# LLNL/Juqbox.jl

Hardware: AMD Instinct MI355X
Metric: traceobjgrad evals/sec (fwd+adjoint), cnot3 Hilbert dim (higher is better)
Workload: dtype f64

## Files before the change

### include/juqbox_hip.h

```cpp
#ifndef JUQBOX_HIP_H
#define JUQBOX_HIP_H

#include <stdint.h>

#ifdef __cplusplus
extern "C" {
#endif

#define JQ_ABI_VERSION 6

#define JQ_MAX_CONTROLS 16
#define JQ_MAX_WRANK 16

#define JQ_OK 0
#define JQ_EINVAL -1
#define JQ_EDIM -2
#define JQ_EUNSUPPORTED -3
#define JQ_EHIP -4
#define JQ_ENOMEM -5

typedef struct jq_handle jq_handle;

typedef struct jq_csc {
    int64_t m, n;
    const int64_t *colptr;
    const int64_t *rowval;
    const double *nzval;
} jq_csc;

typedef struct jq_problem {
    int32_t Ntot;
    int32_t N;
    int32_t Ncoupled;
    int32_t Nfreq;
    int32_t nsteps;
    int32_t neumann_terms;
    int32_t objFuncType;
    int32_t Nunc;
    double T;
    const double *Hconst;
    const double *Hsym_ops;
    const double *Hanti_ops;
    const double *Uinit;
    const double *Utarget_r;
    const double *Utarget_i;
    const double *wmat_real_diag;
    const double *Cfreq;
    const double *Hunc_ops;
    const double *Rfreq;
    const jq_csc *Hconst_csc;
    const jq_csc *Hsym_csc;
    const jq_csc *Hanti_csc;
} jq_problem;

typedef struct jq_timing {
    double ms_total;
    double ms_propagate;
    double ms_generate;
    double ms_forward;
    double ms_backward;
    int64_t n_forward_launches;
    int64_t n_backward_launches;
    int64_t mfma_executed;
    int64_t svts;
    int32_t kernel_family;
    int32_t kernel_size;
    int32_t kernel_band;
    int32_t kernel_variant;
    int64_t mfma_backward;
    double ms_allreduce;
    double ms_shard_min;
    double ms_shard_max;
} jq_timing;

int jq_device_count(void);
int jq_set_device(int device);
int jq_create(const jq_problem *problem, jq_handle **out);
int jq_create_opts(const jq_problem *problem, const char *options, jq_handle **out);
#define JQ_OPTION_DEFAULT INT64_MIN
int jq_set_option(jq_handle *h, const char *name, int64_t value);
int jq_get_option(const jq_handle *h, const char *name, int64_t *value);
void jq_destroy(jq_handle *h);
const char *jq_last_error(const jq_handle *h);

int jq_create_multi(const jq_problem *problem, const int32_t *devices, int32_t ndev, jq_handle **out);
int jq_create_multi_opts(const jq_problem *problem, const int32_t *devices, int32_t ndev, const char *options, jq_handle **out);
int jq_rccl_world_size(const jq_handle *h);
int jq_num_devices(const jq_handle *h);
int jq_num_compute_units(const jq_handle *h);
int jq_handle_device(const jq_handle *h);
int jq_shard_bounds(int32_t nquad, int32_t rank, int32_t world, int32_t *lo, int32_t *hi);

int jq_set_neumann_terms(jq_handle *h, int32_t m);
int jq_set_linear_solver(jq_handle *h, int32_t solver_id, int32_t max_iter, double tol);
int jq_set_integrator(jq_handle *h, int32_t integrator_id, int32_t max_iter, double tol);
int jq_update_target(jq_handle *h, const double *Utarget_r, const double *Utarget_i);
#define JQ_SV_TARGET 1
#define JQ_SV_TERM1 2
#define JQ_SV_TERM2 3
#define JQ_SV_BOTH 4
int jq_update_dvds(jq_handle *h, const double *dVds_r, const double *dVds_i);
int jq_set_sv_type(jq_handle *h, int32_t sv_type);
int jq_get_sv_type(const jq_handle *h);
int jq_update_hconst(jq_handle *h, const double *Hconst);
int jq_update_hconst_csc(jq_handle *h, const jq_csc *Hconst);
int jq_update_wmat_diag(jq_handle *h, const double *wmat_real_diag);
int jq_update_wmat(jq_handle *h, const double *wmat_real, const double *wmat_imag);

int jq_traceobjgrad(jq_handle *h, const double *pcof, int32_t ncoeff, int32_t evaladjoint, double *out4,
                    double *totalgrad, double *infidelgrad, double *leakgrad);

int jq_state_history(jq_handle *h, const double *pcof, int32_t ncoeff, double *ur, double *ui);
int jq_traceobj_verbose(jq_handle *h, const double *pcof, int32_t ncoeff, double *out4, double *ur, double *ui);

int jq_state_populations(jq_handle *h, const double *pcof, int32_t ncoeff, const int32_t *group_of_row, int32_t ngroups,
                         int32_t every, int32_t nout, double *pop, double *maxpop);

int jq_eval_f_g_grad(jq_handle *h, const double *pcof, int32_t ncoeff, const double *nodes, const double *weights,
                     int32_t nquad, const double *shift, int32_t compute_adjoint, double *out2, double *infid_grad,
                     double *leak_grad);

int jq_eval_f_g_grad_dev(jq_handle *h, const double *pcof, int32_t ncoeff, const double *nodes, const double *weights,
                         int32_t nquad, const double *shift, int32_t compute_adjoint, void *d_packed);

int jq_traceobj_sweep(jq_handle *h, const double *pcof, int32_t ncoeff, const double *nodes, int32_t nquad,
                      const double *shift, double *out);

int jq_plan_info(const jq_handle *h, char *buf, int32_t buflen);

int jq_last_timing(const jq_handle *h, jq_timing *t);
const char *jq_version(void);
int jq_abi_version(void);

#ifdef __cplusplus
}
#endif
#endif
```

### juqbox.jl_amd/_lib.py

```python
import ctypes
import os

_HERE = os.path.dirname(os.path.abspath(__file__))
LIB_PATH = os.environ.get("JQ_LIB") or os.path.join(_HERE, "libjuqbox_hip.so")

c_dp = ctypes.POINTER(ctypes.c_double)
c_i32 = ctypes.c_int32

JQ_OK, JQ_EINVAL, JQ_EDIM, JQ_EUNSUPPORTED, JQ_EHIP, JQ_ENOMEM = 0, -1, -2, -3, -4, -5
JQ_SV_TARGET, JQ_SV_TERM1, JQ_SV_TERM2, JQ_SV_BOTH = 1, 2, 3, 4
JQ_OPTION_DEFAULT = -2 ** 63


class jq_csc(ctypes.Structure):
    _fields_ = [("m", ctypes.c_int64), ("n", ctypes.c_int64), ("colptr", ctypes.POINTER(ctypes.c_int64)),
                ("rowval", ctypes.POINTER(ctypes.c_int64)), ("nzval", c_dp)]


class jq_problem(ctypes.Structure):
    _fields_ = [("Ntot", c_i32), ("N", c_i32), ("Ncoupled", c_i32), ("Nfreq", c_i32), ("nsteps", c_i32),
                ("neumann_terms", c_i32), ("objFuncType", c_i32), ("Nunc", c_i32), ("T", ctypes.c_double),
                ("Hconst", c_dp), ("Hsym_ops", c_dp), ("Hanti_ops", c_dp), ("Uinit", c_dp), ("Utarget_r", c_dp),
                ("Utarget_i", c_dp), ("wmat_real_diag", c_dp), ("Cfreq", c_dp), ("Hunc_ops", c_dp), ("Rfreq", c_dp),
                ("Hconst_csc", ctypes.POINTER(jq_csc)), ("Hsym_csc", ctypes.POINTER(jq_csc)), ("Hanti_csc", ctypes.POINTER(jq_csc))]


class jq_timing(ctypes.Structure):
    _fields_ = [("ms_total", ctypes.c_double), ("ms_propagate", ctypes.c_double), ("ms_generate", ctypes.c_double),
                ("ms_forward", ctypes.c_double), ("ms_backward", ctypes.c_double),
                ("n_forward_launches", ctypes.c_int64), ("n_backward_launches", ctypes.c_int64), ("mfma_executed", ctypes.c_int64), ("svts", ctypes.c_int64),
                ("kernel_family", ctypes.c_int32), ("kernel_size", ctypes.c_int32), ("kernel_band", ctypes.c_int32),
                ("kernel_variant", ctypes.c_int32), ("mfma_backward", ctypes.c_int64),
                ("ms_allreduce", ctypes.c_double), ("ms_shard_min", ctypes.c_double), ("ms_shard_max", ctypes.c_double)]


JQ_ABI_VERSION = 6


SYMBOLS = {
    "jq_device_count": (ctypes.c_int, []),
    "jq_set_device": (ctypes.c_int, [ctypes.c_int]),
    "jq_create": (ctypes.c_int, [ctypes.POINTER(jq_problem), ctypes.POINTER(ctypes.c_void_p)]),
    "jq_create_opts": (ctypes.c_int, [ctypes.POINTER(jq_problem), ctypes.c_char_p, ctypes.POINTER(ctypes.c_void_p)]),
    "jq_set_option": (ctypes.c_int, [ctypes.c_void_p, ctypes.c_char_p, ctypes.c_int64]),
    "jq_get_option": (ctypes.c_int, [ctypes.c_void_p, ctypes.c_char_p, ctypes.POINTER(ctypes.c_int64)]),
    "jq_destroy": (None, [ctypes.c_void_p]),
    "jq_last_error": (ctypes.c_char_p, [ctypes.c_void_p]),
    "jq_set_neumann_terms": (ctypes.c_int, [ctypes.c_void_p, c_i32]),
    "jq_set_linear_solver": (ctypes.c_int, [ctypes.c_void_p, c_i32, c_i32, ctypes.c_double]),
    "jq_set_integrator": (ctypes.c_int, [ctypes.c_void_p, c_i32, c_i32, ctypes.c_double]),
    "jq_update_target": (ctypes.c_int, [ctypes.c_void_p, c_dp, c_dp]),
    "jq_update_dvds": (ctypes.c_int, [ctypes.c_void_p, c_dp, c_dp]),
    "jq_set_sv_type": (ctypes.c_int, [ctypes.c_void_p, c_i32]),
    "jq_get_sv_type": (ctypes.c_int, [ctypes.c_void_p]),
    "jq_update_hconst": (ctypes.c_int, [ctypes.c_void_p, c_dp]),
    "jq_update_hconst_csc": (ctypes.c_int, [ctypes.c_void_p, ctypes.POINTER(jq_csc)]),
    "jq_update_wmat_diag": (ctypes.c_int, [ctypes.c_void_p, c_dp]),
    "jq_update_wmat": (ctypes.c_int, [ctypes.c_void_p, c_dp, c_dp]),
    "jq_traceobjgrad": (ctypes.c_int, [ctypes.c_void_p, c_dp, c_i32, c_i32, c_dp, c_dp, c_dp, c_dp]),
    "jq_state_history": (ctypes.c_int, [ctypes.c_void_p, c_dp, c_i32, c_dp, c_dp]),
    "jq_traceobj_verbose": (ctypes.c_int, [ctypes.c_void_p, c_dp, c_i32, c_dp, c_dp, c_dp]),
    "jq_state_populations": (ctypes.c_int, [ctypes.c_void_p, c_dp, c_i32, ctypes.POINTER(ctypes.c_int32), c_i32, c_i32, c_i32,
                                            c_dp, c_dp]),
    "jq_eval_f_g_grad": (ctypes.c_int, [ctypes.c_void_p, c_dp, c_i32, c_dp, c_dp, c_i32, c_dp, c_i32, c_dp, c_dp, c_dp]),
    "jq_eval_f_g_grad_dev": (ctypes.c_int, [ctypes.c_void_p, c_dp, c_i32, c_dp, c_dp, c_i32, c_dp, c_i32, ctypes.c_void_p]),
    "jq_create_multi": (ctypes.c_int, [ctypes.POINTER(jq_problem), ctypes.POINTER(ctypes.c_int32), c_i32,
                                       ctypes.POINTER(ctypes.c_void_p)]),
    "jq_create_multi_opts": (ctypes.c_int, [ctypes.POINTER(jq_problem), ctypes.POINTER(ctypes.c_int32), c_i32, ctypes.c_char_p,
                                            ctypes.POINTER(ctypes.c_void_p)]),
    "jq_rccl_world_size": (ctypes.c_int, [ctypes.c_void_p]),
    "jq_num_devices": (ctypes.c_int, [ctypes.c_void_p]),
    "jq_handle_device": (ctypes.c_int, [ctypes.c_void_p]),
    "jq_num_compute_units": (ctypes.c_int, [ctypes.c_void_p]),
    "jq_shard_bounds": (ctypes.c_int, [c_i32, c_i32, c_i32, ctypes.POINTER(ctypes.c_int32), ctypes.POINTER(ctypes.c_int32)]),
    "jq_traceobj_sweep": (ctypes.c_int, [ctypes.c_void_p, c_dp, c_i32, c_dp, c_i32, c_dp, c_dp]),
    "jq_plan_info": (ctypes.c_int, [ctypes.c_void_p, ctypes.c_char_p, c_i32]),
    "jq_last_timing": (ctypes.c_int, [ctypes.c_void_p, ctypes.POINTER(jq_timing)]),
    "jq_version": (ctypes.c_char_p, []),
    "jq_abi_version": (ctypes.c_int, []),
}

_lib = None


class JuqboxHipError(RuntimeError):
    def __init__(self, code, msg):
        super().__init__("libjuqbox_hip error %d: %s" % (code, msg))
        self.code = code


def load():
    global _lib
    if _lib is None:
        if not os.path.exists(LIB_PATH):
            raise ImportError("libjuqbox_hip.so not built: %s is missing (run `make -C juqbox.jl_amd/csrc`); "
                              "there is no CPU fallback for the hot path" % LIB_PATH)
        L = ctypes.CDLL(LIB_PATH)
        for name, (res, args) in SYMBOLS.items():
            fn = getattr(L, name)
            fn.restype = res
            fn.argtypes = args
        if L.jq_abi_version() != JQ_ABI_VERSION:
            raise ImportError("libjuqbox_hip.so has ABI version %d, this binding is written for %d (rebuild: make -C "
                              "juqbox.jl_amd/csrc)" % (L.jq_abi_version(), JQ_ABI_VERSION))
        _lib = L
    return _lib


def check(rc, handle=None):
    if rc != JQ_OK:
        msg = load().jq_last_error(handle)
        raise JuqboxHipError(rc, msg.decode() if msg else "?")
```

### juqbox.jl_amd/csrc/jq_host_create.h

```cpp
template <typename T>
static int dev_alloc(jq_handle* h, T** p, size_t count)
{
    if (*p) {
        (void)hipFree(*p);
        *p = nullptr;
    }
    if (hipMalloc((void**)p, std::max<size_t>(count, 1) * sizeof(T)) != hipSuccess) {
        *p = nullptr;
        (void)hipGetLastError();
        char buf[160];
        snprintf(buf, sizeof buf, "out of device memory (%zu bytes requested)", std::max<size_t>(count, 1) * sizeof(T));
        return fail(h, JQ_ENOMEM, buf);
    }
    return JQ_OK;
}
template <typename T>
static int dev_grow(jq_handle* h, T** p, size_t* cap, size_t need)
{
    if (need <= *cap && *p) return JQ_OK;
    *cap = 0;
    const int rc = dev_alloc(h, p, need);
    if (rc == JQ_OK) *cap = need;
    return rc;
}

static int upload_operators(jq_handle* h)
{
    const size_t nn = (size_t)h->Ntot * h->Ntot;
    std::vector<double> img((size_t)(1 + 2 * h->Nc) * h->mat_elems, 0.0);
    if (!h->big) {
        tile_image(h->Hconst.data(), h->Ntot, h->NT, h->BW, img.data());
        for (int q = 0; q < h->Nc; ++q) {
            tile_image(h->Hsym.data() + q * nn, h->Ntot, h->NT, h->BW, img.data() + (size_t)(1 + q) * h->mat_elems);
            tile_image(h->Hanti.data() + q * nn, h->Ntot, h->NT, h->BW, img.data() + (size_t)(1 + h->Nc + q) * h->mat_elems);
        }
    }
    HIPCHK(h, hipMemcpy(h->d_himg, img.data(), img.size() * sizeof(double), hipMemcpyHostToDevice));
    auto cslot = [&](int q, bool anti) {
        int g = 0;
        while (ctrl_gstart(h->Nc, g + 1) <= q) ++g;
        const int gs = ctrl_gstart(h->Nc, g), ng = ctrl_gstart(h->Nc, g + 1) - gs;
        return (size_t)(2 * gs + (anti ? ng : 0) + (q - gs));
    };
    std::vector<double> cimg((size_t)(2 * h->Nc) * h->mat_elems, 0.0);
    for (int q = 0; q < h->Nc && !h->big; ++q) {
        const int bwq = (h->BW == JQ_BW_T4) ? JQ_BW_T4 : (h->bw_trace[q] == 0) ? 0 : h->BW;
        const bool sd = (h->BW == JQ_BW_T4) ? false : (h->bw_trace[q] == 2);
        tile_image(h->Hsym.data() + q * nn, h->Ntot, h->NT, bwq, cimg.data() + cslot(q, false) * h->mat_elems, sd);
        tile_image(h->Hanti.data() + q * nn, h->Ntot, h->NT, bwq, cimg.data() + cslot(q, true) * h->mat_elems, sd);
    }
    HIPCHK(h, hipMemcpy(h->d_cimg, cimg.data(), cimg.size() * sizeof(double), hipMemcpyHostToDevice));
    if (h->mat_elems_c > 0) {
        std::vector<double> ic((size_t)(1 + 2 * h->Nc) * h->mat_elems_c, 0.0);
        tile_image_coop(h->Hconst.data(), h->Ntot, h->NT, h->BWc, ic.data());
        for (int q = 0; q < h->Nc; ++q) {
            tile_image_coop(h->Hsym.data() + q * nn, h->Ntot, h->NT, h->BWc, ic.data() + (size_t)(1 + q) * h->mat_elems_c);
            tile_image_coop(h->Hanti.data() + q * nn, h->Ntot, h->NT, h->BWc, ic.data() + (size_t)(1 + h->Nc + q) * h->mat_elems_c);
        }
        HIPCHK(h, hipMemcpy(h->d_himg_c, ic.data(), ic.size() * sizeof(double), hipMemcpyHostToDevice));
        std::vector<double> cc((size_t)2 * h->Nc * h->mat_elems_c);
        for (int q = 0; q < h->Nc; ++q) {
            std::copy_n(ic.data() + (size_t)(1 + q) * h->mat_elems_c, h->mat_elems_c, cc.data() + cslot(q, false) * h->mat_elems_c);
            std::copy_n(ic.data() + (size_t)(1 + h->Nc + q) * h->mat_elems_c, h->mat_elems_c, cc.data() + cslot(q, true) * h->mat_elems_c);
        }
        HIPCHK(h, hipMemcpy(h->d_cimg_c, cc.data(), cc.size() * sizeof(double), hipMemcpyHostToDevice));
    }
    if (h->lane_np > 0) {
        std::vector<double> il((size_t)(1 + 2 * h->Nc) * h->lane_stride, 0.0);
        plain_image(h->Hconst.data(), h->Ntot, h->lane_np, il.data());
        for (int q = 0; q < h->Nc; ++q) {
            plain_image(h->Hsym.data() + q * nn, h->Ntot, h->lane_np, il.data() + (size_t)(1 + q) * h->lane_stride);
            plain_image(h->Hanti.data() + q * nn, h->Ntot, h->lane_np, il.data() + (size_t)(1 + h->Nc + q) * h->lane_stride);
        }
        HIPCHK(h, hipMemcpy(h->d_himg_l, il.data(), il.size() * sizeof(double), hipMemcpyHostToDevice));
        std::vector<double> cl((size_t)2 * h->Nc * h->lane_stride);
        for (int q = 0; q < h->Nc; ++q) {
            std::copy_n(il.data() + (size_t)(1 + q) * h->lane_stride, h->lane_stride, cl.data() + cslot(q, false) * h->lane_stride);
            std::copy_n(il.data() + (size_t)(1 + h->Nc + q) * h->lane_stride, h->lane_stride, cl.data() + cslot(q, true) * h->lane_stride);
        }
        HIPCHK(h, hipMemcpy(h->d_cimg_l, cl.data(), cl.size() * sizeof(double), hipMemcpyHostToDevice));
    }
    if (h->dq_max_quads > 0) {
        std::vector<double> id((size_t)(1 + 2 * h->Nc) * JQ_DQ_ELEMS, 0.0);
        dq_image(h->Hconst.data(), h->Ntot, id.data());
        for (int q = 0; q < h->Nc; ++q) {
            dq_image(h->Hsym.data() + q * nn, h->Ntot, id.data() + (size_t)(1 + q) * JQ_DQ_ELEMS);
            dq_image(h->Hanti.data() + q * nn, h->Ntot, id.data() + (size_t)(1 + h->Nc + q) * JQ_DQ_ELEMS);
        }
        HIPCHK(h, hipMemcpy(h->d_himg_dq, id.data(), id.size() * sizeof(double), hipMemcpyHostToDevice));
        std::vector<double> cd((size_t)2 * h->Nc * JQ_DQ_ELEMS);
        for (int q = 0; q < h->Nc; ++q) {
            std::copy_n(id.data() + (size_t)(1 + q) * JQ_DQ_ELEMS, JQ_DQ_ELEMS, cd.data() + cslot(q, false) * JQ_DQ_ELEMS);
            std::copy_n(id.data() + (size_t)(1 + h->Nc + q) * JQ_DQ_ELEMS, JQ_DQ_ELEMS, cd.data() + cslot(q, true) * JQ_DQ_ELEMS);
        }
        HIPCHK(h, hipMemcpy(h->d_cimg_dq, cd.data(), cd.size() * sizeof(double), hipMemcpyHostToDevice));
    }
    if (h->rl_npj > 0) {
        std::vector<double> ir((size_t)(1 + 2 * h->Nc) * h->rl_stride, 0.0);
        rowlane_image(h->Hconst.data(), h->Ntot, h->rl_npj, ir.data());
        for (int q = 0; q < h->Nc; ++q) {
            rowlane_image(h->Hsym.data() + q * nn, h->Ntot, h->rl_npj, ir.data() + (size_t)(1 + q) * h->rl_stride);
            rowlane_image(h->Hanti.data() + q * nn, h->Ntot, h->rl_npj, ir.data() + (size_t)(1 + h->Nc + q) * h->rl_stride);
        }
        HIPCHK(h, hipMemcpy(h->d_himg_r, ir.data(), ir.size() * sizeof(double), hipMemcpyHostToDevice));
        std::vector<double> cr((size_t)2 * h->Nc * h->rl_stride);
        for (int q = 0; q < h->Nc; ++q) {
            std::copy_n(ir.data() + (size_t)(1 + q) * h->rl_stride, h->rl_stride, cr.data() + cslot(q, false) * h->rl_stride);
            std::copy_n(ir.data() + (size_t)(1 + h->Nc + q) * h->rl_stride, h->rl_stride, cr.data() + cslot(q, true) * h->rl_stride);
        }
        HIPCHK(h, hipMemcpy(h->d_cimg_r, cr.data(), cr.size() * sizeof(double), hipMemcpyHostToDevice));
    }
    return JQ_OK;
}

static int upload_terminal_images(jq_handle* h, const double* re, const double* im, double* d_r, double* d_i, double* d_r_l, double* d_i_l,
                                  double* d_r_r, double* d_i_r)
{
    std::vector<double> img((size_t)h->parts * h->KT * 64);
    slab_image(re, h->Ntot, h->N, h->sps, h->KT, img.data(), h->parts);
    HIPCHK(h, hipMemcpy(d_r, img.data(), img.size() * sizeof(double), hipMemcpyHostToDevice));
    slab_image(im, h->Ntot, h->N, h->sps, h->KT, img.data(), h->parts);
    HIPCHK(h, hipMemcpy(d_i, img.data(), img.size() * sizeof(double), hipMemcpyHostToDevice));
    if (h->lane_np > 0) {
        std::vector<double> cl((size_t)h->N * h->lane_np, 0.0);
        column_image(re, h->Ntot, h->N, h->lane_np, cl.data());
        HIPCHK(h, hipMemcpy(d_r_l, cl.data(), cl.size() * sizeof(double), hipMemcpyHostToDevice));
        std::fill(cl.begin(), cl.end(), 0.0);
        column_image(im, h->Ntot, h->N, h->lane_np, cl.data());
        HIPCHK(h, hipMemcpy(d_i_l, cl.data(), cl.size() * sizeof(double), hipMemcpyHostToDevice));
    }
    if (h->rl_npj > 0) {
        std::vector<double> cl((size_t)h->N * 16, 0.0);
        column_image(re, h->Ntot, h->N, 16, cl.data());
        HIPCHK(h, hipMemcpy(d_r_r, cl.data(), cl.size() * sizeof(double), hipMemcpyHostToDevice));
        std::fill(cl.begin(), cl.end(), 0.0);
        column_image(im, h->Ntot, h->N, 16, cl.data());
        HIPCHK(h, hipMemcpy(d_i_r, cl.data(), cl.size() * sizeof(double), hipMemcpyHostToDevice));
    }
    return JQ_OK;
}

static int upload_targets(jq_handle* h)
{
    return upload_terminal_images(h, h->Utr.data(), h->Uti.data(), h->d_vtr, h->d_vti, h->d_vtr_l, h->d_vti_l, h->d_vtr_r, h->d_vti_r);
}

static int upload_dvds(jq_handle* h)
{
    if (!h->dv_stale) return JQ_OK;
    HIPCHK(h, hipSetDevice(h->device));
    int rc;
    if (!h->dv_alloc) {
        if ((rc = dev_alloc(h, &h->d_dvr, (size_t)h->parts * h->KT * 64))) return rc;
        if ((rc = dev_alloc(h, &h->d_dvi, (size_t)h->parts * h->KT * 64))) return rc;
        if (h->lane_np > 0) {
            if ((rc = dev_alloc(h, &h->d_dvr_l, (size_t)h->N * h->lane_np))) return rc;
            if ((rc = dev_alloc(h, &h->d_dvi_l, (size_t)h->N * h->lane_np))) return rc;
        }
        if (h->rl_npj > 0) {
            if ((rc = dev_alloc(h, &h->d_dvr_r, (size_t)h->N * 16))) return rc;
            if ((rc = dev_alloc(h, &h->d_dvi_r, (size_t)h->N * 16))) return rc;
        }
        h->dv_alloc = true;
    }
    if ((rc = upload_terminal_images(h, h->dVr.data(), h->dVi.data(), h->d_dvr, h->d_dvi, h->d_dvr_l, h->d_dvi_l, h->d_dvr_r, h->d_dvi_r)))
        return rc;
    h->dv_stale = false;
    return JQ_OK;
}

extern "C" int jq_device_count(void)
{
    int n = 0;
    if (hipGetDeviceCount(&n) != hipSuccess) return 0;
    return n;
}

extern "C" int jq_set_device(int device) { return hipSetDevice(device) == hipSuccess ? JQ_OK : JQ_EHIP; }
// ... 70 lines not shown
        const int64_t b = A->colptr[j], e = A->colptr[j + 1];
        for (int64_t k = b - 1; k < e - 1; ++k) {
            const int64_t r = A->rowval[k];
            if (r < 1 || r > Ntot) {
                snprintf(buf, sizeof buf, "%s: rowval out of range (1 .. Ntot)", what);
                return fail(h, JQ_EINVAL, buf);
            }
            out[(r - 1) + (size_t)Ntot * j] += A->nzval[k];
        }
    }
    return JQ_OK;
}

static int create_dense(const jq_problem* p, jq_handle* h);

static int create_impl(const jq_problem* p, jq_handle* h)
{
    if (!p) return fail(h, JQ_EINVAL, "jq_create: problem is NULL");
    const bool sparse = (!p->Hconst && p->Hconst_csc) || (!p->Hsym_ops && p->Hsym_csc) || (!p->Hanti_ops && p->Hanti_csc);
    if (!sparse) return create_dense(p, h);
    if (p->Ntot < 1 || p->Ntot > 16384 || p->Ncoupled < 0 || p->Ncoupled > 4096) return create_dense(p, h);
    const size_t nn = (size_t)p->Ntot * p->Ntot;
    std::vector<double> H0, Hs, Ha;
    jq_problem q = *p;
    q.Hconst_csc = q.Hsym_csc = q.Hanti_csc = nullptr;
    int rc;
    if (!p->Hconst && p->Hconst_csc) {
        H0.resize(nn);
        if ((rc = csc_to_dense(h, p->Hconst_csc, p->Ntot, H0.data(), "jq_create: Hconst_csc"))) return rc;
        q.Hconst = H0.data();
    }
    if (!p->Hsym_ops && p->Hsym_csc) {
        Hs.resize(nn * std::max(p->Ncoupled, 1));
        for (int k = 0; k < p->Ncoupled; ++k)
            if ((rc = csc_to_dense(h, p->Hsym_csc + k, p->Ntot, Hs.data() + nn * k, "jq_create: Hsym_csc"))) return rc;
        q.Hsym_ops = Hs.data();
    }
    if (!p->Hanti_ops && p->Hanti_csc) {
        Ha.resize(nn * std::max(p->Ncoupled, 1));
        for (int k = 0; k < p->Ncoupled; ++k)
            if ((rc = csc_to_dense(h, p->Hanti_csc + k, p->Ntot, Ha.data() + nn * k, "jq_create: Hanti_csc"))) return rc;
        q.Hanti_ops = Ha.data();
    }
    return create_dense(&q, h);
}

static int create_dense(const jq_problem* p, jq_handle* h)
{
    if (!p) return fail(h, JQ_EINVAL, "jq_create: problem is NULL");
    if (p->Ntot < 1 || p->N < 1 || p->N > p->Ntot) return fail(h, JQ_EINVAL, "jq_create: need 1 <= N <= Ntot");
    if (p->nsteps < 1 || !(p->T > 0.0)) return fail(h, JQ_EINVAL, "jq_create: need nsteps >= 1 and T > 0");
    if (p->Nfreq < 1) return fail(h, JQ_EINVAL, "jq_create: need Nfreq >= 1");
    if (p->neumann_terms < 0) return fail(h, JQ_EINVAL, "jq_create: neumann_terms must be >= 0");
    if (p->Nunc < 0) return fail(h, JQ_EINVAL, "jq_create: Nunc must be >= 0");
    if (p->Nunc > 0 && p->Ncoupled != 0)
        return fail(h, JQ_EINVAL, "jq_create: coupled and uncoupled controls cannot be combined (Ncoupled == 0 || Nunc == 0)");
    if (!p->Hconst || !p->Uinit || !p->Utarget_r || !p->Utarget_i || !p->wmat_real_diag || !p->Cfreq ||
        (p->Nunc == 0 && (!p->Hsym_ops || !p->Hanti_ops)) || (p->Nunc > 0 && (!p->Hunc_ops || !p->Rfreq)))
        return fail(h, JQ_EINVAL, "jq_create: NULL array in problem description");
    const int nctrl = p->Nunc > 0 ? p->Nunc : p->Ncoupled;
    if (nctrl < 1) return fail(h, JQ_EUNSUPPORTED, "jq_create: at least one control Hamiltonian is required");
    if (nctrl > 4096) return fail(h, JQ_EINVAL, "jq_create: more than 4096 control Hamiltonians");
    if (p->Ntot > 16384) return fail(h, JQ_EINVAL, "jq_create: Ntot > 16384");
    if (p->objFuncType < 1 || p->objFuncType > 3) return fail(h, JQ_EINVAL, "jq_create: objFuncType must be 1, 2 or 3");

    HIPCHK(h, hipGetDevice(&h->device));
    hipDeviceProp_t prop;
    HIPCHK(h, hipGetDeviceProperties(&prop, h->device));
    if (strncmp(prop.gcnArchName, "gfx950", 6) != 0) {
        char buf[256];
        snprintf(buf, sizeof buf, "jq_create: device arch '%s' is not gfx950 (this library is MI355X-only)", prop.gcnArchName);
        return fail(h, JQ_EUNSUPPORTED, buf);
    }
    HIPCHK(h, hipStreamCreate(&h->stream));

    h->Ntot = p->Ntot; h->N = p->N; h->Nc = nctrl; h->NcK = std::min(nctrl, JQ_MAXNC); h->Nfreq = p->Nfreq; h->nsteps = p->nsteps;
    h->m = p->neumann_terms; h->objFuncType = p->objFuncType; h->T = p->T;
    h->NT = (p->Ntot + 15) / 16;
    h->big = h->NT > 6;
    h->huge = h->NT > 16;
    h->bw_trace.assign(nctrl, 0);
    h->KT = 4 * h->NT;
    h->NP = 16 * h->NT;
    h->parts = p->N > 16 ? (p->N + 15) / 16 : 1;
    h->sps = p->N > 16 ? 1 : 16 / p->N;
    h->state_stride = (long long)(JQ_STATE_ARRAYS * h->KT + JQ_STATE_EXTRA) * 64;
    const size_t nn = (size_t)p->Ntot * p->Ntot, nc = (size_t)p->Ntot * p->N;
    h->Hconst.assign(p->Hconst, p->Hconst + nn);
    if (p->Nunc > 0) {
        h->Hsym.assign(nn * nctrl, 0.0);
        h->Hanti.assign(nn * nctrl, 0.0);
        h->rfreq.assign(p->Rfreq, p->Rfreq + nctrl);
        for (int q = 0; q < nctrl; ++q) {
            const double* M = p->Hunc_ops + nn * q;
            bool sym = true;
            double nrm2 = 0.0;
            for (int c = 0; c < p->Ntot; ++c)
                for (int r = 0; r < p->Ntot; ++r) {
                    const double a = M[r + (size_t)p->Ntot * c], b = M[c + (size_t)p->Ntot * r];
                    if (a != b) sym = false;
                    nrm2 += (a + b) * (a + b);
                }
            if (!sym && !(std::sqrt(nrm2) < 1e-15))
                return fail(h, JQ_EINVAL, "jq_create: Uncoupled Hamiltonian is not symmetric or anti-symmetric. This functionality is "
                                          "not currently supported.");
            std::copy(M, M + nn, (sym ? h->Hsym.begin() : h->Hanti.begin()) + nn * q);
        }
    } else {
        h->Hsym.assign(p->Hsym_ops, p->Hsym_ops + nn * p->Ncoupled);
        h->Hanti.assign(p->Hanti_ops, p->Hanti_ops + nn * p->Ncoupled);
    }
    h->Uinit.assign(p->Uinit, p->Uinit + nc);
    h->Utr.assign(p->Utarget_r, p->Utarget_r + nc);
    h->Uti.assign(p->Utarget_i, p->Utarget_i + nc);
    h->dVr = h->Utr;
    h->dVi = h->Uti;
    h->wd.assign(p->wmat_real_diag, p->wmat_real_diag + p->Ntot);
    h->cfreq.assign(p->Cfreq, p->Cfreq + (size_t)nctrl * p->Nfreq);

    if (h->big && h->NT <= 8 && !h->force_plain) {
        bool t4 = block_band(h->Hconst.data(), h->Ntot) <= 1 && t4_structure(h->Hconst.data(), h->Ntot);
        for (int q = 0; q < h->Nc && t4; ++q)
            t4 = block_band(h->Hsym.data() + q * nn, h->Ntot) <= 1 && block_band(h->Hanti.data() + q * nn, h->Ntot) <= 1 &&
                 t4_structure(h->Hsym.data() + q * nn, h->Ntot) && t4_structure(h->Hanti.data() + q * nn, h->Ntot);
        if (!h->opt.on(O_T4) || !h->opt.on(O_OD) || !h->opt.on(O_T4BIG) || h->opt.on(O_FORCE_DENSE)) t4 = false;
        if (t4) h->big = false;
    }

    {
        int bw = block_band(h->Hconst.data(), h->Ntot);
        for (int q = 0; q < h->Nc; ++q) {
            const int bq = std::max(block_band(h->Hsym.data() + q * nn, h->Ntot), block_band(h->Hanti.data() + q * nn, h->Ntot));
            h->bw_trace[q] = bq;
            bw = std::max(bw, bq);
        }
        if (h->opt.on(O_FORCE_DENSE)) bw = h->NT - 1;
        h->BW = (bw <= 2 && bw < h->NT - 1) ? bw : h->NT - 1;
        if (h->big && h->BW == 0) h->BW = 1;
        if (h->big && h->BW > 2) h->BW = 15;
        if (h->huge) h->BW = 15;
        h->BWc = h->BW;
        bool od = (!h->big && bw == 1 && h->NT >= 2 && offdiag_blocks_diagonal(h->Hconst.data(), h->Ntot));
        for (int q = 0; q < h->Nc && od; ++q)
            od = offdiag_blocks_diagonal(h->Hsym.data() + q * nn, h->Ntot) && offdiag_blocks_diagonal(h->Hanti.data() + q * nn, h->Ntot);
        if (!h->opt.on(O_OD) || h->opt.on(O_FORCE_DENSE)) od = false;
        if (od) h->BW = h->BWc = JQ_BW_OD;
        bool t4 = !h->big && (bw <= 1) && t4_structure(h->Hconst.data(), h->Ntot);
        for (int q = 0; q < h->Nc && t4; ++q)
            t4 = t4_structure(h->Hsym.data() + q * nn, h->Ntot) && t4_structure(h->Hanti.data() + q * nn, h->Ntot);
        if (!h->opt.on(O_T4) || !h->opt.on(O_OD) || h->opt.on(O_FORCE_DENSE) || h->force_plain) t4 = false;
        if (t4) h->BW = JQ_BW_T4;
        for (int q = 0; q < h->Nc && h->BW == JQ_BW_T4; ++q)
            h->bw_trace[q] = t4_mode(h->Hsym.data() + q * nn, h->Ntot) | t4_mode(h->Hanti.data() + q * nn, h->Ntot);
        for (int q = 0; q < h->Nc && h->BW != JQ_BW_T4; ++q) {
            if (h->bw_trace[q] == 0 || h->BW == 0)
                h->bw_trace[q] = (h->BW == 0) ? 1 : 0;
            else
                h->bw_trace[q] = (h->NT > 1 && diag_blocks_zero(h->Hsym.data() + q * nn, h->Ntot) &&
                                  diag_blocks_zero(h->Hanti.data() + q * nn, h->Ntot)) ? 2 : 1;
        }
        h->mat_elems = (((h->BW == JQ_BW_T4 ? (long long)JQ_T4_ELEMS(h->NT)
                                             : 64LL * band_tiles(h->NT, h->BW) + (h->BW == JQ_BW_OD ? JQ_OD_COEFS(h->NT) : 0)) + 127) / 128) * 128;
        const long long slot = h->mat_elems * 8;
        const long long lds_fwd_fixed = (long long)32 * h->NT * 8;
        const long long lds_bwd_fixed = bwd_lds_tail(h->NT, h->NcK, JQ_WAVES, 0);
        const long long park_bytes = (long long)JQ_WAVES * h->KT * 64 * 8;
        if (h->big) {
            h->mat_elems = 128;
            h->BW = -1;
        } else if (2 * slot + lds_fwd_fixed > JQ_LDS_MAX)
            return fail(h, JQ_EUNSUPPORTED, "jq_create: operator images do not fit the LDS double buffer");
        h->nslots = 2;
        h->nslots_bwd = 2;
        h->park_lds = (2 * slot + lds_bwd_fixed + park_bytes <= JQ_LDS_MAX) ? 1 : 0;
        h->mat_elems_c = 0;
        if (h->NT > 6) {
            if (h->BWc == 0) h->BWc = 1;
            if (h->BWc > 2) h->BWc = 15;
        }
        if (h->NT >= 2 || h->N > 4) {
            const long long ec = (((long long)h->NT * coop_row_elems(h->NT, h->BWc) + 127) / 128) * 128;
            const long long lds_c = (coop_hbm(h->NT, h->BWc) ? 0 : 2 * ec * 8) + lds_fwd_fixed + 2LL * h->KT * 64 * 8 + 16LL * h->NT * 8;
            h->mat_elems_c = ec;
            h->coop_ok = lds_c <= JQ_LDS_MAX && (h->NT <= 6 || h->big);
            if (h->huge) h->coop_ok = true;
        }
        h->coop_max_slabs = prop.multiProcessorCount;
        if (h->opt.has(O_COOP_MAX)) h->coop_max_slabs = (int)h->opt.get(O_COOP_MAX);
        if (h->big) h->coop_max_slabs = 1 << 30;
        h->batch = 0;
        {
            const long long budget = (h->NT <= JQ_MINW_MAXNT) ? JQ_LDS_MAX / 2 : JQ_LDS_MAX;
            if (!h->big && (long long)win_lds(h, h->mat_elems) + lds_bwd_fixed + park_bytes <= budget && h->opt.on(O_WINDOW)) {
                h->batch = -1;
                h->park_lds = 1;
            }
        }
        h->quad_max_slabs = (h->BW == JQ_BW_T4 && quad_bwd_lds(h, 1) <= JQ_LDS_MAX && h->opt.on(O_WINDOW)) ? (1 << 30) : 0;
        h->num_cu = prop.multiProcessorCount;
        if (h->opt.has(O_QUAD) && h->quad_max_slabs > 0) h->quad_max_slabs = (int)h->opt.get(O_QUAD);
        h->cq_max_quads = (h->BW == JQ_BW_T4 && h->NT >= 2 && h->NT <= 7 && h->quad_max_slabs > 0 && cq_lds(h, win_lds(h, h->mat_elems)) <= JQ_LDS_MAX) ? 2 * prop.multiProcessorCount : 0;
        if (h->opt.has(O_CQ) && h->cq_max_quads > 0) h->cq_max_quads = (int)h->opt.get(O_CQ);
        h->dq_max_quads = (h->NT == 2 && h->BW != JQ_BW_T4 && !h->big && !h->huge && !h->is_emb && cq_lds(h, win_lds(h, JQ_DQ_ELEMS)) <= JQ_LDS_MAX && h->opt.on(O_DQ)) ? 3 * prop.multiProcessorCount : 0;
        if (h->opt.has(O_BATCH)) {
            const int v = (int)h->opt.get(O_BATCH);
            if (v >= 2 && slot <= 8192) {
                const long long fixed = lds_bwd_fixed + park_bytes + 2LL * h->NcK * slot;
                const long long per_buf = (JQ_LDS_MAX - fixed) / 2;
                long long B = (per_buf / (2 * slot) - 1) / 2;
                if (B > v) B = v;
                if (B >= 2) {
                    h->batch = (int)B;
                    h->park_lds = 1;
                }
            }
        }
    }

    h->lane_np = 0;
    {
        static const int nps[] = {2, 4, 6, 8};
        for (int v : nps)
            if (h->Ntot <= v) {
                h->lane_np = v;
                break;
            }
        if (!h->opt.on(O_LANE)) h->lane_np = 0;
        h->lane_stride = ((long long)h->lane_np * h->lane_np + 15) / 16 * 16;
        h->lane_min_cols = 1;
        h->lane_max_cols = 1 << 30;
        h->rl_npj = h->Ntot <= 8 ? (h->Ntot + 1) / 2 * 2 : (h->Ntot <= 12 ? 12 : (h->Ntot <= 16 ? 16 : 0));
        if (!h->opt.on(O_LANE)) h->rl_npj = 0;
        if (h->is_emb) h->rl_npj = 0, h->lane_np = 0;
        h->rl_stride = 16LL * h->rl_npj;
        h->rl_max_cols = 2 * 4 * 4 * prop.multiProcessorCount;
        if (h->opt.has(O_ROWLANE_MAX)) h->rl_max_cols = (int)h->opt.get(O_ROWLANE_MAX);
        if (h->opt.has(O_LANE_MIN)) h->lane_min_cols = (int)h->opt.get(O_LANE_MIN);
        if (h->opt.has(O_LANE_MAX)) h->lane_max_cols = (int)h->opt.get(O_LANE_MAX);
    }

    const double dt = h->T / h->nsteps;
    h->tf.resize(h->nsteps + 1);
    h->tb.resize(h->nsteps + 1);
    double t = 0.0;
    for (int n = 0; n <= h->nsteps; ++n) {
        h->tf[n] = t;
        t = t + dt;
    }
    t = h->T;
    for (int n = 0; n <= h->nsteps; ++n) {
        h->tb[n] = t;
        t = t + (-dt);
    }

    int rc;
    if ((rc = dev_alloc(h, &h->d_himg, (size_t)(1 + 2 * h->Nc) * h->mat_elems))) return rc;
    if ((rc = dev_alloc(h, &h->d_cimg, (size_t)(2 * h->Nc) * h->mat_elems))) return rc;
    if (h->mat_elems_c > 0) {
        if ((rc = dev_alloc(h, &h->d_himg_c, (size_t)(1 + 2 * h->Nc) * h->mat_elems_c))) return rc;
        if ((rc = dev_alloc(h, &h->d_cimg_c, (size_t)(2 * h->Nc) * h->mat_elems_c))) return rc;
    }
    if (h->lane_np > 0) {
        if ((rc = dev_alloc(h, &h->d_himg_l, (size_t)(1 + 2 * h->Nc) * h->lane_stride))) return rc;
        if ((rc = dev_alloc(h, &h->d_cimg_l, (size_t)(2 * h->Nc) * h->lane_stride))) return rc;
        if ((rc = dev_alloc(h, &h->d_uinit_l, (size_t)h->N * h->lane_np))) return rc;
        if ((rc = dev_alloc(h, &h->d_vtr_l, (size_t)h->N * h->lane_np))) return rc;
        if ((rc = dev_alloc(h, &h->d_vti_l, (size_t)h->N * h->lane_np))) return rc;
        std::vector<double> cl((size_t)h->N * h->lane_np, 0.0);
        column_image(h->Uinit.data(), h->Ntot, h->N, h->lane_np, cl.data());
        HIPCHK(h, hipMemcpy(h->d_uinit_l, cl.data(), cl.size() * sizeof(double), hipMemcpyHostToDevice));
    }
    if (h->dq_max_quads > 0) {
        if ((rc = dev_alloc(h, &h->d_himg_dq, (size_t)(1 + 2 * h->Nc) * JQ_DQ_ELEMS))) return rc;
        if ((rc = dev_alloc(h, &h->d_cimg_dq, (size_t)(2 * h->Nc) * JQ_DQ_ELEMS))) return rc;
    }
    if (h->rl_npj > 0) {
        if ((rc = dev_alloc(h, &h->d_himg_r, (size_t)(1 + 2 * h->Nc) * h->rl_stride))) return rc;
        if ((rc = dev_alloc(h, &h->d_cimg_r, (size_t)(2 * h->Nc) * h->rl_stride))) return rc;
        if ((rc = dev_alloc(h, &h->d_uinit_r, (size_t)h->N * 16))) return rc;
        if ((rc = dev_alloc(h, &h->d_vtr_r, (size_t)h->N * 16))) return rc;
        if ((rc = dev_alloc(h, &h->d_vti_r, (size_t)h->N * 16))) return rc;
        std::vector<double> cl((size_t)h->N * 16, 0.0);
        column_image(h->Uinit.data(), h->Ntot, h->N, 16, cl.data());
        HIPCHK(h, hipMemcpy(h->d_uinit_r, cl.data(), cl.size() * sizeof(double), hipMemcpyHostToDevice));
    }
    if ((rc = dev_alloc(h, &h->d_uimg, (size_t)h->parts * h->KT * 64))) return rc;
    if ((rc = dev_alloc(h, &h->d_vtr, (size_t)h->parts * h->KT * 64))) return rc;
    if ((rc = dev_alloc(h, &h->d_vti, (size_t)h->parts * h->KT * 64))) return rc;
    if ((rc = dev_alloc(h, &h->d_tabs, (size_t)32 * h->NT))) return rc;
    if ((rc = dev_alloc(h, &h->d_tf, (size_t)h->nsteps + 1))) return rc;
    if ((rc = dev_alloc(h, &h->d_tb, (size_t)h->nsteps + 1))) return rc;
    if ((rc = dev_alloc(h, &h->d_cfreq, h->cfreq.size()))) return rc;
    HIPCHK(h, hipMemcpy(h->d_tf, h->tf.data(), h->tf.size() * sizeof(double), hipMemcpyHostToDevice));
    HIPCHK(h, hipMemcpy(h->d_tb, h->tb.data(), h->tb.size() * sizeof(double), hipMemcpyHostToDevice));
    HIPCHK(h, hipMemcpy(h->d_cfreq, h->cfreq.data(), h->cfreq.size() * sizeof(double), hipMemcpyHostToDevice));
    if (!h->rfreq.empty()) {
        if ((rc = dev_alloc(h, &h->d_rfreq, h->rfreq.size()))) return rc;
        HIPCHK(h, hipMemcpy(h->d_rfreq, h->rfreq.data(), h->rfreq.size() * sizeof(double), hipMemcpyHostToDevice));
    }
    if ((rc = upload_operators(h))) return rc;
    if ((rc = upload_targets(h))) return rc;
    {
        std::vector<double> img((size_t)h->parts * h->KT * 64);
        slab_image(h->Uinit.data(), h->Ntot, h->N, h->sps, h->KT, img.data(), h->parts);
        HIPCHK(h, hipMemcpy(h->d_uimg, img.data(), img.size() * sizeof(double), hipMemcpyHostToDevice));
    }
// ... 151 lines not shown
```

### juqbox.jl_amd/csrc/jq_host_info.h

```cpp
extern "C" int jq_set_option(jq_handle* h, const char* name, int64_t value)
{
    if (!h) return JQ_EINVAL;
    if (!name) return fail(h, JQ_EINVAL, "jq_set_option: NULL name");
    const int o = JqOptions::find(name, strlen(name));
    if (o < 0) return fail(h, JQ_EINVAL, (std::string("jq_set_option: unknown option '") + name + "'").c_str());
    const long long v = (value == JQ_OPTION_DEFAULT) ? JQ_OPT_UNSET : (long long)value;
    if (!h->subs.empty()) {
        std::string err;
        if (!h->opt.set(o, v, &err)) return fail(h, JQ_EUNSUPPORTED, ("jq_set_option: " + err).c_str());
        if (o == O_MULTI_SAME_DEVICE) return fail(h, JQ_EINVAL, "jq_set_option: multi_same_device is an option of jq_create_multi_opts");
        return multi_forall(h, [&](jq_handle* sub) { return jq_set_option(sub, name, value); });
    }
    const long long old = h->opt.v[o];
    if (old == v) return JQ_OK;
    std::string err;
    if (!h->opt.set(o, v, &err)) return fail(h, JQ_EUNSUPPORTED, ("jq_set_option: " + err).c_str());
    if (g_jq_opt[o].flags & JQ_OPT_PLAN) {
        HIPCHK(h, hipSetDevice(h->device));
        const std::vector<double> H0 = h->Hconst;
        const int rc = replan(h, H0.data());
        if (rc != JQ_OK) {
            h->opt.v[o] = old;
            return rc;
        }
        h->replanned = false;
        return JQ_OK;
    }
    if (h->emb) h->emb->opt = h->opt;
    return JQ_OK;
}

extern "C" int jq_get_option(const jq_handle* h, const char* name, int64_t* value)
{
    if (!h || !name || !value) return JQ_EINVAL;
    const int o = JqOptions::find(name, strlen(name));
    if (o < 0) return JQ_EINVAL;
    const long long v = h->opt.get(o);
    *value = (v == JQ_OPT_UNSET) ? JQ_OPTION_DEFAULT : (int64_t)v;
    return JQ_OK;
}

extern "C" int jq_rccl_world_size(const jq_handle* h)
{
    if (!h || h->comms.empty() || !h->comms[0] || !g_rccl.CommCount) return 0;
    int n = 0;
    if (g_rccl.CommCount(h->comms[0], &n) != ncclSuccess) return -1;
    return n;
}

extern "C" int jq_plan_info(const jq_handle* hh, char* buf, int32_t buflen)
{
    if (!hh || (!buf && buflen > 0) || buflen < 0) return JQ_EINVAL;
    const jq_handle* h = hh->subs.empty() ? hh : hh->subs[0];
    std::string o = "{";
    auto kv = [&](const char* k, const std::string& v, bool quote = false) {
        if (o.size() > 1) o += ", ";
        o += std::string("\"") + k + "\": " + (quote ? "\"" + v + "\"" : v);
    };
    auto num = [](long long v) { return std::to_string(v); };
    kv("devices", num(hh->subs.empty() ? 1 : (long long)hh->subs.size()));
    kv("Ntot", num(h->Ntot));
    kv("N", num(h->N));
    kv("controls", num(h->Nc));
    kv("control_groups", num(ctrl_ngroups(h->Nc)));
    kv("tile_rows", num(h->NT));
    kv("compute_units", num(h->num_cu));
    const char* structure = h->big ? (h->BWc == 15 ? "dense" : "band") : h->BW == JQ_BW_T4 ? "t4" : h->BW == JQ_BW_OD ? "od" : h->BW == h->NT - 1 ? "dense" : "band";
    kv("structure", structure, true);
    kv("block_band", num(h->big ? h->BWc : h->BW));
    kv("embedded_twin_Ntot", num(h->emb ? h->emb->Ntot : 0));
    kv("integrator", h->integrator == 2 ? "implicit_midpoint" : "stormer_verlet", true);
    kv("linear_solver", h->solver_id == 2 ? "jacobi" : "neumann", true);
    kv("sv_type", num(h->sv_type));
    kv("neumann_terms_or_max_iter", num(h->integrator == 2 ? h->imr_max_iter : h->m));
    kv("chunk_steps", num(h->chunk_steps));
    kv("replanned", h->replanned ? "true" : "false");
    std::string fam = "[";
    auto add = [&](int id, const char* name, const char* unit, long long mx) {
        if (fam.size() > 1) fam += ", ";
        fam += std::string("{\"family\": ") + std::to_string(id) + ", \"name\": \"" + name + "\", \"max_" + unit + "\": " + std::to_string(mx) + "}";
    };
    const jq_handle* t = h->emb ? h->emb : h;
    if (h->rl_npj > 0) add(3, "row-lane (VALU, lane per (row, column); backward sweep on three or four waves, implicit midpoint: two)", "columns", h->rl_max_cols);
    if (h->lane_np > 0) add(2, "lane (VALU, lane per column)", "columns", h->lane_max_cols);
    if (t->cq_max_quads > 0) add(8, "cooperative quad (one 16-row block per wave)", "quads", t->cq_max_quads);
    if (t->dq_max_quads > 0) add(8, "cooperative quad, dense blocks (17 .. 32 levels without the 4 x 4 x n structure; Neumann, Diagonal weights)", "quads", t->dq_max_quads);
    if (t->quad_max_slabs > 0) add(6, "quad layout (four columns per wave; 1 / 2 / 3 slabs per workgroup by round count)", "slabs", t->quad_max_slabs);
    if (t->coop_ok && t->NT >= 2) add(1, "cooperative (tile row per wave)", "slabs", t->coop_max_slabs);
    if (!t->big) add(0, "slab (wave per 16-column slab)", "slabs", 1LL << 30);
    fam += "]";
    kv("families", fam);
    {
        const std::string man(jq_build_manifest);
        std::vector<std::string> tags;
        auto tag = [&](const char* prefix, int a, int b) {
            char buf[32];
            if (b >= 0) snprintf(buf, sizeof buf, "%s_%d_%d", prefix, a, b);
            else snprintf(buf, sizeof buf, "%s_%d", prefix, a);
            tags.push_back(buf);
        };
        for (const jq_handle* x : {h, (const jq_handle*)h->emb}) {
            if (!x) continue;
            if (x->BW == JQ_BW_T4) {
                for (const char* pre : {"k", "s", "p", "u", "w", "q", "v"}) tag(pre, x->NT, JQ_BW_T4Q);
                tag("k", x->NT, JQ_BW_T4);
            } else if (!x->big) {
                tag("k", x->NT, x->BW);
                tag("j", x->NT, x->BW);
            }
            if (x->mat_elems_c > 0) tag("c", x->NT, x->BWc), tag("i", x->NT, x->BWc);
            if (x->rl_npj > 0) tag("r", x->rl_npj, -1), tag("m", x->rl_npj, -1);
            if (x->lane_np > 0) tag("l", x->lane_np, -1);
        }
        std::string objs = "{";
        for (const std::string& t : tags) {
            const std::string key = "\"" + t + "\": {";
            const size_t at = man.find(key);
            if (at == std::string::npos) continue;
            const size_t end = man.find('}', at);
            if (end == std::string::npos) continue;
            if (objs.size() > 1) objs += ", ";
            objs += man.substr(at, end - at + 1);
        }
        objs += "}";
        std::string hipcc = "null";
        {
            const size_t at = man.find("\"hipcc\": {");
            const size_t end = at == std::string::npos ? at : man.find('}', at);
            if (end != std::string::npos) hipcc = man.substr(at + 9, end - at - 8);
        }
        kv("build", std::string("{\"manifest\": ") + (man.size() > 2 ? "true" : "false") + ", \"hipcc\": " + hipcc + ", \"objects\": " + objs + "}");
    }
    kv("full_weight_rank", num(h->wrank));
    kv("options", hh->opt.str(), true);
    kv("rccl_selfchecks", num(hh->rccl_checks));
    {
        const jq_handle* t2 = h->emb ? h->emb : h;
        const std::string d = t2->cq3_last.empty() ? "no batch of the cooperative-quad families yet" : t2->cq3_last;
        kv("latency_split", std::string("{\"last_decision\": \"") + d + "\", \"faults\": " + num(t2->cq3_faults) + ", \"faults_xcd\": " + num(t2->cq3_faults_xcd) + ", \"abandoned_at_rendezvous\": " + num(t2->cq3_busy) + ", \"cooling_down\": " + num(t2->cq3_skip) +
                                ", \"off\": " + (t2->cq3_off ? "true" : "false") + "}");
    }
    o += "}";
    if (buflen > 0) {
        const size_t n = std::min(o.size(), (size_t)buflen - 1);
        memcpy(buf, o.data(), n);
        buf[n] = 0;
    }
    return (int)o.size();
}

extern "C" int jq_last_timing(const jq_handle* h, jq_timing* t)
{
    if (!h || !t) return JQ_EINVAL;
    *t = h->timing;
    return JQ_OK;
}
```

### juqbox.jl_amd/csrc/jq_host_select.h

```cpp
typedef void (*prop_kernel_t)(PropArgs);

#define JQ_FOR_EACH_INST(X)                                                                       \
    X(1, 0) X(2, 0) X(2, 1) X(3, 0) X(3, 1) X(3, 2) X(4, 0) X(4, 1) X(4, 2) X(4, 3) X(5, 0) X(5, 1) \
    X(5, 2) X(5, 4) X(6, 0) X(6, 1) X(6, 2) X(6, 5) X(2, 9) X(3, 9) X(4, 9) X(5, 9) X(6, 9) X(1, 8) X(2, 8) X(3, 8)       \
    X(4, 8) X(5, 8) X(6, 8) X(7, 8) X(8, 8)
#define JQ_MINW_OF(nt) (((nt) <= JQ_MINW_MAXNT) ? 2 : 1)
#define JQ_DECL(nt, bw)                                                                      \
    extern template __global__ void k_forward<nt, bw, JQ_MINW_OF(nt), false>(PropArgs);      \
    extern template __global__ void k_backward<nt, bw, JQ_MINW_OF(nt), false>(PropArgs);     \
    extern template __global__ void k_forward<nt, bw, JQ_MINW_OF(nt), true>(PropArgs);       \
    extern template __global__ void k_backward<nt, bw, JQ_MINW_OF(nt), true>(PropArgs);
JQ_FOR_EACH_INST(JQ_DECL)
#undef JQ_DECL

extern template __global__ void k_forward<1, 0, JQ_MINW_OF(1), false, true>(PropArgs);
extern template __global__ void k_backward<1, 0, JQ_MINW_OF(1), false, true>(PropArgs);
extern template __global__ void k_forward<6, 5, JQ_MINW_OF(6), false, true>(PropArgs);
extern template __global__ void k_backward<6, 5, JQ_MINW_OF(6), false, true>(PropArgs);
extern template __global__ void k_forward<1, 0, JQ_MINW_OF(1), true, true>(PropArgs);
extern template __global__ void k_backward<1, 0, JQ_MINW_OF(1), true, true>(PropArgs);
extern template __global__ void k_forward<6, 5, JQ_MINW_OF(6), true, true>(PropArgs);
extern template __global__ void k_backward<6, 5, JQ_MINW_OF(6), true, true>(PropArgs);

static int select_kernels(jq_handle* h, prop_kernel_t* fwd, prop_kernel_t* bwd)
{
    const bool jac = (h->solver_id == 2);
    if (h->wrank > 0) {
        if (h->NT == 1 && h->BW == 0) {
            *fwd = jac ? k_forward<1, 0, JQ_MINW_OF(1), true, true> : k_forward<1, 0, JQ_MINW_OF(1), false, true>;
            *bwd = jac ? k_backward<1, 0, JQ_MINW_OF(1), true, true> : k_backward<1, 0, JQ_MINW_OF(1), false, true>;
            return JQ_OK;
        }
        if (h->NT == 6 && h->BW == 5) {
            *fwd = jac ? k_forward<6, 5, JQ_MINW_OF(6), true, true> : k_forward<6, 5, JQ_MINW_OF(6), false, true>;
            *bwd = jac ? k_backward<6, 5, JQ_MINW_OF(6), true, true> : k_backward<6, 5, JQ_MINW_OF(6), false, true>;
            return JQ_OK;
        }
        return fail(h, JQ_EUNSUPPORTED, "full leakage weights (jq_update_wmat): no kernels with the low-rank terms for this plan (row-lane kernels "
                                        "disabled, or cooperative kernels that do not fit the LDS)");
    }
#define JQ_PICK(nt, bw)                                                                                  \
    if (h->NT == nt && h->BW == bw) {                                                                    \
        *fwd = jac ? k_forward<nt, bw, JQ_MINW_OF(nt), true> : k_forward<nt, bw, JQ_MINW_OF(nt), false>; \
        *bwd = jac ? k_backward<nt, bw, JQ_MINW_OF(nt), true> : k_backward<nt, bw, JQ_MINW_OF(nt), false>; \
        return JQ_OK;                                                                                    \
    }
    JQ_FOR_EACH_INST(JQ_PICK)
#undef JQ_PICK
    return fail(h, JQ_EUNSUPPORTED, "unsupported Hilbert dimension / band width");
}

#define JQ_DECLQ(nt)                                                            \
    extern template __global__ void k_forward<nt, JQ_BW_T4Q, 1, false>(PropArgs);    \
    extern template __global__ void k_backward<nt, JQ_BW_T4Q, 1, false>(PropArgs);   \
    extern template __global__ void k_forward<nt, JQ_BW_T4Q, 2, false>(PropArgs);    \
    extern template __global__ void k_backward<nt, JQ_BW_T4Q, 2, false>(PropArgs);   \
    extern template __global__ void k_forward<nt, JQ_BW_T4Q, 3, false>(PropArgs);    \
    extern template __global__ void k_backward<nt, JQ_BW_T4Q, 3, false>(PropArgs);   \
    extern template __global__ void k_backward<nt, JQ_BW_T4Q, 3, false, false, true>(PropArgs);   \
    extern template __global__ void k_backward<nt, JQ_BW_T4Q, 3, false, false, true, true>(PropArgs);
JQ_DECLQ(1) JQ_DECLQ(2) JQ_DECLQ(3) JQ_DECLQ(4) JQ_DECLQ(5) JQ_DECLQ(6) JQ_DECLQ(7) JQ_DECLQ(8)
#undef JQ_DECLQ
template <int NT, bool MODD, int NS, bool WLR = false, bool DN = false> __global__ void k_forward_cq(PropArgs);
template <int NT, bool MODD, bool ORD, bool WLR = false, bool DN = false> __global__ void k_backward_cq(PropArgs);
template <int NT, bool MODD, bool ORD, int NR = 3, bool WLR = false, bool DN = false> __global__ void k_backward_cq3(PropArgs);
#define JQ_DECLCQ(nt)                                                      \
    extern template __global__ void k_forward_cq<nt, false, 1>(PropArgs);  \
    extern template __global__ void k_forward_cq<nt, false, 2>(PropArgs);  \
    extern template __global__ void k_backward_cq<nt, false, false>(PropArgs);    \
    extern template __global__ void k_backward_cq<nt, false, true>(PropArgs);     \
    extern template __global__ void k_forward_cq<nt, true, 1>(PropArgs);   \
    extern template __global__ void k_forward_cq<nt, true, 2>(PropArgs);   \
    extern template __global__ void k_backward_cq<nt, true, false>(PropArgs);     \
    extern template __global__ void k_backward_cq<nt, true, true>(PropArgs);      \
    extern template __global__ void k_forward_cq<nt, false, 1, true>(PropArgs);          \
    extern template __global__ void k_forward_cq<nt, true, 1, true>(PropArgs);           \
    extern template __global__ void k_backward_cq<nt, false, false, true>(PropArgs);     \
    extern template __global__ void k_backward_cq<nt, false, true, true>(PropArgs);      \
    extern template __global__ void k_backward_cq<nt, true, false, true>(PropArgs);      \
    extern template __global__ void k_backward_cq<nt, true, true, true>(PropArgs);       \
    extern template __global__ void k_backward_cq3<nt, false, false, 3, true>(PropArgs);   \
    extern template __global__ void k_backward_cq3<nt, false, true, 3, true>(PropArgs);    \
    extern template __global__ void k_backward_cq3<nt, true, false, 3, true>(PropArgs);    \
    extern template __global__ void k_backward_cq3<nt, true, true, 3, true>(PropArgs);     \
    extern template __global__ void k_backward_cq3<nt, false, false, 2, true>(PropArgs);   \
    extern template __global__ void k_backward_cq3<nt, false, true, 2, true>(PropArgs);    \
    extern template __global__ void k_backward_cq3<nt, true, false, 2, true>(PropArgs);    \
    extern template __global__ void k_backward_cq3<nt, true, true, 2, true>(PropArgs);     \
    extern template __global__ void k_backward_cq3<nt, false, false>(PropArgs);   \
    extern template __global__ void k_backward_cq3<nt, false, true>(PropArgs);    \
    extern template __global__ void k_backward_cq3<nt, true, false>(PropArgs);    \
    extern template __global__ void k_backward_cq3<nt, true, true>(PropArgs);     \
    extern template __global__ void k_backward_cq3<nt, false, false, 2>(PropArgs);   \
    extern template __global__ void k_backward_cq3<nt, false, true, 2>(PropArgs);    \
    extern template __global__ void k_backward_cq3<nt, true, false, 2>(PropArgs);    \
    extern template __global__ void k_backward_cq3<nt, true, true, 2>(PropArgs);
JQ_DECLCQ(1) JQ_DECLCQ(2) JQ_DECLCQ(3) JQ_DECLCQ(4) JQ_DECLCQ(5) JQ_DECLCQ(6) JQ_DECLCQ(7)
#undef JQ_DECLCQ
extern template __global__ void k_forward_cq<2, false, 1, false, true>(PropArgs);
extern template __global__ void k_forward_cq<2, true, 1, false, true>(PropArgs);
extern template __global__ void k_backward_cq<2, false, false, false, true>(PropArgs);
extern template __global__ void k_backward_cq<2, true, false, false, true>(PropArgs);
extern template __global__ void k_backward_cq3<2, false, false, 3, false, true>(PropArgs);
extern template __global__ void k_backward_cq3<2, true, false, 3, false, true>(PropArgs);
extern template __global__ void k_backward_cq3<2, false, false, 2, false, true>(PropArgs);
extern template __global__ void k_backward_cq3<2, true, false, 2, false, true>(PropArgs);
static bool ctrl_per_subsystem(const jq_handle* h)
{
    for (int q = 0; q < h->Nc; ++q)
        if (h->bw_trace[q] != (1 << q)) return false;
    return true;
}
static int select_cq_kernels(jq_handle* h, bool fwd2, int bwd_nr, bool wlr, bool dense, prop_kernel_t* fwd, prop_kernel_t* bwd)
{
    const bool bwd3 = bwd_nr == 3, bwd2 = bwd_nr == 2;
    const bool modd = (h->m > 0 ? h->m : 0) & 1;
    if (dense) {
        if (h->NT != 2 || wlr || fwd2) return fail(h, JQ_EHIP, "internal error: dense cooperative-quad kernels selected for a plan they do not exist for");
        *fwd = modd ? k_forward_cq<2, true, 1, false, true> : k_forward_cq<2, false, 1, false, true>;
        *bwd = bwd3 ? (modd ? k_backward_cq3<2, true, false, 3, false, true> : k_backward_cq3<2, false, false, 3, false, true>)
             : bwd2 ? (modd ? k_backward_cq3<2, true, false, 2, false, true> : k_backward_cq3<2, false, false, 2, false, true>)
                    : (modd ? k_backward_cq<2, true, false, false, true> : k_backward_cq<2, false, false, false, true>);
        return JQ_OK;
    }
    const bool ord = h->Nc <= 3 && !h->opt.on(O_CQ_GENERIC_TRACES) && ctrl_per_subsystem(h);
#define JQ_PICKCQ(nt)                                                              \
    if (h->NT == nt && wlr) {                                                      \
        *fwd = modd ? k_forward_cq<nt, true, 1, true> : k_forward_cq<nt, false, 1, true>;                        \
        *bwd = bwd3 ? (modd ? (ord ? k_backward_cq3<nt, true, true, 3, true> : k_backward_cq3<nt, true, false, 3, true>)          \
                            : (ord ? k_backward_cq3<nt, false, true, 3, true> : k_backward_cq3<nt, false, false, 3, true>))       \
             : bwd2 ? (modd ? (ord ? k_backward_cq3<nt, true, true, 2, true> : k_backward_cq3<nt, true, false, 2, true>)          \
                            : (ord ? k_backward_cq3<nt, false, true, 2, true> : k_backward_cq3<nt, false, false, 2, true>))       \
                    : modd ? (ord ? k_backward_cq<nt, true, true, true> : k_backward_cq<nt, true, false, true>)         \
                           : (ord ? k_backward_cq<nt, false, true, true> : k_backward_cq<nt, false, false, true>);      \
        return JQ_OK;                                                              \
    }                                                                              \
    if (h->NT == nt) {                                                             \
        *fwd = fwd2 ? (modd ? k_forward_cq<nt, true, 2> : k_forward_cq<nt, false, 2>) : (modd ? k_forward_cq<nt, true, 1> : k_forward_cq<nt, false, 1>);            \
        *bwd = bwd3 ? (modd ? (ord ? k_backward_cq3<nt, true, true> : k_backward_cq3<nt, true, false>)          \
                            : (ord ? k_backward_cq3<nt, false, true> : k_backward_cq3<nt, false, false>))       \
             : bwd2 ? (modd ? (ord ? k_backward_cq3<nt, true, true, 2> : k_backward_cq3<nt, true, false, 2>)    \
                            : (ord ? k_backward_cq3<nt, false, true, 2> : k_backward_cq3<nt, false, false, 2>)) \
                    : modd ? (ord ? k_backward_cq<nt, true, true> : k_backward_cq<nt, true, false>)          \
                           : (ord ? k_backward_cq<nt, false, true> : k_backward_cq<nt, false, false>);       \
        return JQ_OK;                                                              \
    }
    JQ_PICKCQ(1) JQ_PICKCQ(2) JQ_PICKCQ(3) JQ_PICKCQ(4) JQ_PICKCQ(5) JQ_PICKCQ(6) JQ_PICKCQ(7)
#undef JQ_PICKCQ
    return fail(h, JQ_EUNSUPPORTED, "unsupported Hilbert dimension");
}
template <int NT, int SPW> __global__ void k_forward_quad_imr(PropArgs);
template <int NT, int SPW> __global__ void k_backward_quad_imr(PropArgs);
#define JQ_DECLQI(nt)                                                         \
    extern template __global__ void k_forward_quad_imr<nt, 1>(PropArgs);      \
    extern template __global__ void k_backward_quad_imr<nt, 1>(PropArgs);
JQ_DECLQI(1) JQ_DECLQI(2) JQ_DECLQI(3) JQ_DECLQI(4) JQ_DECLQI(5) JQ_DECLQI(6) JQ_DECLQI(7) JQ_DECLQI(8)
#undef JQ_DECLQI
static int select_quad_imr_kernels(jq_handle* h, prop_kernel_t* fwd, prop_kernel_t* bwd)
{
#define JQ_PICKQI(nt)                                 \
    if (h->NT == nt) {                                \
        *fwd = k_forward_quad_imr<nt, 1>;             \
        *bwd = k_backward_quad_imr<nt, 1>;            \
        return JQ_OK;                                 \
    }
    JQ_PICKQI(1) JQ_PICKQI(2) JQ_PICKQI(3) JQ_PICKQI(4) JQ_PICKQI(5) JQ_PICKQI(6) JQ_PICKQI(7) JQ_PICKQI(8)
#undef JQ_PICKQI
    return fail(h, JQ_EUNSUPPORTED, "unsupported Hilbert dimension");
}
template <int NT, bool DN = false> __global__ void k_forward_cq_imr(PropArgs);
template <int NT, bool DN = false> __global__ void k_backward_cq_imr(PropArgs);
template <int NT> __global__ void k_backward_cq_imr2(PropArgs);
#define JQ_DECLCI(nt)                                                    \
    extern template __global__ void k_forward_cq_imr<nt>(PropArgs);      \
    extern template __global__ void k_backward_cq_imr<nt>(PropArgs);
JQ_DECLCI(1) JQ_DECLCI(2) JQ_DECLCI(3) JQ_DECLCI(4) JQ_DECLCI(5) JQ_DECLCI(6) JQ_DECLCI(7)
#undef JQ_DECLCI
template <int NT, bool DN = false> __global__ void k_backward_cq_imr3(PropArgs);
#define JQ_DECLCI(nt) extern template __global__ void k_backward_cq_imr3<nt>(PropArgs);
JQ_DECLCI(1) JQ_DECLCI(2) JQ_DECLCI(3) JQ_DECLCI(4) JQ_DECLCI(5) JQ_DECLCI(6) JQ_DECLCI(7)
#undef JQ_DECLCI
#define JQ_DECLCI(nt) extern template __global__ void k_backward_cq_imr2<nt>(PropArgs);
JQ_DECLCI(1) JQ_DECLCI(2) JQ_DECLCI(3) JQ_DECLCI(4) JQ_DECLCI(5) JQ_DECLCI(6)
#undef JQ_DECLCI
extern template __global__ void k_forward_cq_imr<2, true>(PropArgs);
extern template __global__ void k_backward_cq_imr<2, true>(PropArgs);
extern template __global__ void k_backward_cq_imr3<2, true>(PropArgs);
static int select_cq_imr_kernels(jq_handle* h, bool two, bool three, bool dense, prop_kernel_t* fwd, prop_kernel_t* bwd)
{
    if (dense) {
        if (h->NT != 2 || two) return fail(h, JQ_EHIP, "internal error: dense implicit-midpoint cooperative-quad kernels selected for a plan they do not exist for");
        *fwd = k_forward_cq_imr<2, true>;
        *bwd = three ? k_backward_cq_imr3<2, true> : k_backward_cq_imr<2, true>;
        return JQ_OK;
    }
#define JQ_PICKCI(nt)                            \
    if (h->NT == nt && three) {                  \
        *fwd = k_forward_cq_imr<nt>;             \
        *bwd = k_backward_cq_imr3<nt>;           \
        return JQ_OK;                            \
    }
    JQ_PICKCI(1) JQ_PICKCI(2) JQ_PICKCI(3) JQ_PICKCI(4) JQ_PICKCI(5) JQ_PICKCI(6) JQ_PICKCI(7)
#undef JQ_PICKCI
#define JQ_PICKCI(nt)                            \
    if (h->NT == nt && two) {                    \
        *fwd = k_forward_cq_imr<nt>;             \
        *bwd = k_backward_cq_imr2<nt>;           \
        return JQ_OK;                            \
    }
    JQ_PICKCI(1) JQ_PICKCI(2) JQ_PICKCI(3) JQ_PICKCI(4) JQ_PICKCI(5) JQ_PICKCI(6)
#undef JQ_PICKCI
#define JQ_PICKCI(nt)                            \
    if (h->NT == nt) {                           \
        *fwd = k_forward_cq_imr<nt>;             \
        *bwd = k_backward_cq_imr<nt>;            \
        return JQ_OK;                            \
    }
    JQ_PICKCI(1) JQ_PICKCI(2) JQ_PICKCI(3) JQ_PICKCI(4) JQ_PICKCI(5) JQ_PICKCI(6) JQ_PICKCI(7)
#undef JQ_PICKCI
    return fail(h, JQ_EUNSUPPORTED, "unsupported Hilbert dimension");
}
static int select_quad_kernels(jq_handle* h, int spw, prop_kernel_t* fwd, prop_kernel_t* bwd)
{
    const bool uni = (h->N % 4 == 0 || h->parts > 1) && !h->opt.on(O_NO_UNI);
    const bool ord = uni && h->Nc >= 2 && h->Nc <= 3 && !h->opt.on(O_NO_ORD) && ctrl_per_subsystem(h);
#define JQ_PICKQ(nt)                                                                                                                             \
    if (h->NT == nt) {                                                                                                                           \
        *fwd = spw == 3 ? k_forward<nt, JQ_BW_T4Q, 3, false> : spw == 2 ? k_forward<nt, JQ_BW_T4Q, 2, false> : k_forward<nt, JQ_BW_T4Q, 1, false>;     \
        *bwd = spw == 3 ? (ord ? k_backward<nt, JQ_BW_T4Q, 3, false, false, true, true>                                                       \
                                : uni ? k_backward<nt, JQ_BW_T4Q, 3, false, false, true> : k_backward<nt, JQ_BW_T4Q, 3, false>)                 \
                        : spw == 2 ? k_backward<nt, JQ_BW_T4Q, 2, false> : k_backward<nt, JQ_BW_T4Q, 1, false>;  \
        return JQ_OK;                                                                                                                            \
    }
    JQ_PICKQ(1) JQ_PICKQ(2) JQ_PICKQ(3) JQ_PICKQ(4) JQ_PICKQ(5) JQ_PICKQ(6) JQ_PICKQ(7) JQ_PICKQ(8)
#undef JQ_PICKQ
    return fail(h, JQ_EUNSUPPORTED, "unsupported Hilbert dimension");
}

template <int NT, bool ORD, int QW, bool RIDE = false> __global__ void k_backward_qsplit(PropArgs);
#define JQ_DECLQS(nt)                                                            \
    extern template __global__ void k_backward_qsplit<nt, false, 4>(PropArgs);   \
    extern template __global__ void k_backward_qsplit<nt, true, 4>(PropArgs);    \
    extern template __global__ void k_backward_qsplit<nt, false, 2>(PropArgs);   \
    extern template __global__ void k_backward_qsplit<nt, true, 2>(PropArgs);    \
    extern template __global__ void k_backward_qsplit<nt, true, 4, true>(PropArgs);    \
    extern template __global__ void k_backward_qsplit<nt, true, 2, true>(PropArgs);
JQ_DECLQS(1) JQ_DECLQS(2) JQ_DECLQS(3) JQ_DECLQS(4) JQ_DECLQS(5) JQ_DECLQS(6)
#undef JQ_DECLQS
static int select_qsplit_kernel(jq_handle* h, int qw, prop_kernel_t* bwd)
{
    const bool ord = h->Nc >= 2 && h->Nc <= 3 && !h->opt.on(O_NO_ORD) && ctrl_per_subsystem(h);
    const bool ride_set = h->opt.has(O_QS_RIDE);
    const long long ride_v = h->opt.get(O_QS_RIDE);
    const bool ride = ord && h->Nc == 3 && !(ride_set && ride_v == 0) && (qw == 2 || (ride_set && ride_v == 1));
#define JQ_PICKQS(nt)                                                                                         \
    if (h->NT == nt) {                                                                                        \
        *bwd = qw == 4 ? (ride ? k_backward_qsplit<nt, true, 4, true> : ord ? k_backward_qsplit<nt, true, 4> : k_backward_qsplit<nt, false, 4>)             \
                       : (ride ? k_backward_qsplit<nt, true, 2, true> : ord ? k_backward_qsplit<nt, true, 2> : k_backward_qsplit<nt, false, 2>);            \
        return JQ_OK;                                                                                         \
    }
    JQ_PICKQS(1) JQ_PICKQS(2) JQ_PICKQS(3) JQ_PICKQS(4) JQ_PICKQS(5) JQ_PICKQS(6)
#undef JQ_PICKQS
    return fail(h, JQ_EUNSUPPORTED, "unsupported Hilbert dimension");
}

#define JQ_DECLQW(nt)                                                                  \
    extern template __global__ void k_forward<nt, JQ_BW_T4Q, 1, false, true>(PropArgs);    \
    extern template __global__ void k_backward<nt, JQ_BW_T4Q, 1, false, true>(PropArgs);
JQ_DECLQW(1) JQ_DECLQW(2) JQ_DECLQW(3) JQ_DECLQW(4) JQ_DECLQW(5) JQ_DECLQW(6) JQ_DECLQW(7) JQ_DECLQW(8)
#undef JQ_DECLQW
static int select_quad_w_kernels(jq_handle* h, prop_kernel_t* fwd, prop_kernel_t* bwd)
{
#define JQ_PICKQW(nt)                                          \
    if (h->NT == nt) {                                         \
        *fwd = k_forward<nt, JQ_BW_T4Q, 1, false, true>;       \
        *bwd = k_backward<nt, JQ_BW_T4Q, 1, false, true>;      \
        return JQ_OK;                                          \
    }
    JQ_PICKQW(1) JQ_PICKQW(2) JQ_PICKQW(3) JQ_PICKQW(4) JQ_PICKQW(5) JQ_PICKQW(6) JQ_PICKQW(7) JQ_PICKQW(8)
#undef JQ_PICKQW
    return fail(h, JQ_EUNSUPPORTED, "unsupported Hilbert dimension");
}

#define JQ_DECLC(nt, bw)                                                   \
    extern template __global__ void k_forward_coop<nt, bw>(PropArgs);       \
    extern template __global__ void k_backward_coop<nt, bw>(PropArgs);
#define JQ_FOR_EACH_COOP(X)                                                                               \
    X(2, 0) X(2, 1) X(3, 0) X(3, 1) X(3, 2) X(4, 0) X(4, 1) X(4, 2) X(4, 3) X(5, 0) X(5, 1) X(5, 2) X(5, 4) \
    X(6, 0) X(6, 1) X(6, 2) X(6, 5) X(2, 9) X(3, 9) X(4, 9) X(5, 9) X(6, 9)
JQ_FOR_EACH_COOP(JQ_DECLC)
#define JQ_FOR_EACH_BIG(X)                                                                                   \
    X(7, 1) X(7, 2) X(7, 15) X(8, 1) X(8, 2) X(8, 15) X(9, 1) X(9, 2) X(9, 15) X(10, 1) X(10, 2) X(10, 15)  \
    X(11, 1) X(11, 2) X(11, 15) X(12, 1) X(12, 2) X(12, 15) X(13, 1) X(13, 2) X(13, 15) X(14, 1) X(14, 2)   \
    X(14, 15) X(15, 1) X(15, 2) X(15, 15) X(16, 1) X(16, 2) X(16, 15)
JQ_FOR_EACH_BIG(JQ_DECLC)
#undef JQ_DECLC

static int select_coop_kernels(jq_handle* h, prop_kernel_t* fwd, prop_kernel_t* bwd)
{
    if (h->huge) {
        *fwd = k_forward_huge, *bwd = k_backward_huge;
        return JQ_OK;
    }
#define JQ_PICKC(nt, bw)                      \
    if (h->NT == nt && h->BWc == bw) {        \
        *fwd = k_forward_coop<nt, bw>;        \
        *bwd = k_backward_coop<nt, bw>;       \
        return JQ_OK;                         \
    }
    JQ_FOR_EACH_COOP(JQ_PICKC)
    JQ_FOR_EACH_BIG(JQ_PICKC)
#undef JQ_PICKC
    return fail(h, JQ_EUNSUPPORTED, "no cooperative kernel for this Hilbert dimension / band width");
}

typedef void (*lane_init_t)(double*, long long, const double*, int, long long);
typedef void (*lane_term_t)(double*, long long, const double*, const double*, int, int, double, double*, const double*, const double*, int);
#define JQ_FOR_EACH_LANE(X) X(2) X(4) X(6) X(8)
#define JQ_DECLL(np)                                                                                  \
    extern template __global__ void k_forward_lane<np>(PropArgs);                                     \
    extern template __global__ void k_backward_lane<np>(PropArgs);                                    \
    extern template __global__ void k_init_state_lane<np>(double*, long long, const double*, int, long long); \
    extern template __global__ void k_terminal_lane<np>(double*, long long, const double*, const double*, int, int, double, double*, const double*, const double*, int);
JQ_FOR_EACH_LANE(JQ_DECLL)
#undef JQ_DECLL

static int select_lane_kernels(jq_handle* h, prop_kernel_t* fwd, prop_kernel_t* bwd, lane_init_t* init, lane_term_t* term)
{
#define JQ_PICKL(np)                     \
    if (h->lane_np == np) {              \
        *fwd = k_forward_lane<np>;       \
        *bwd = k_backward_lane<np>;      \
        *init = k_init_state_lane<np>;   \
        *term = k_terminal_lane<np>;     \
        return JQ_OK;                    \
    }
    JQ_FOR_EACH_LANE(JQ_PICKL)
#undef JQ_PICKL
    return fail(h, JQ_EUNSUPPORTED, "no lane kernel for this Hilbert dimension");
}

#define JQ_FOR_EACH_ROWLANE(X) X(2) X(4) X(6) X(8) X(12) X(16)
#define JQ_DECLR(npj)                                                     \
    extern template __global__ void k_forward_rowlane<npj>(PropArgs);     \
    extern template __global__ void k_backward_rowlane<npj>(PropArgs);    \
    extern template __global__ void k_forward_rowlane<npj, false, true>(PropArgs);     \
    extern template __global__ void k_forward_rowlane<npj, true, true>(PropArgs);     \
    extern template __global__ void k_backward_rowlane<npj, true>(PropArgs);    \
    extern template __global__ void k_backward_rowlane2<npj>(PropArgs);   \
    extern template __global__ void k_backward_rowlane3<npj>(PropArgs);
JQ_FOR_EACH_ROWLANE(JQ_DECLR)
#undef JQ_DECLR

static int select_rowlane_kernels(jq_handle* h, int split, bool hist, prop_kernel_t* fwd, prop_kernel_t* bwd)
{
#define JQ_PICKR(npj)                                                          \
    if (h->rl_npj == npj) {                                                    \
        *fwd = h->wrank > 0 ? k_forward_rowlane<npj, true, true> : hist ? k_forward_rowlane<npj, false, true> : k_forward_rowlane<npj>;     \
        *bwd = h->wrank > 0 ? k_backward_rowlane<npj, true> : split == 3 ? k_backward_rowlane3<npj> : split == 2 ? k_backward_rowlane2<npj> : k_backward_rowlane<npj>;     \
        return JQ_OK;                                                          \
    }
    JQ_FOR_EACH_ROWLANE(JQ_PICKR)
#undef JQ_PICKR
    return fail(h, JQ_EUNSUPPORTED, "no row-lane kernel for this Hilbert dimension");
}

#define JQ_DECLM(npj)                                                        \
    extern template __global__ void k_forward_rowlane_imr<npj>(PropArgs);    \
    extern template __global__ void k_backward_rowlane_imr<npj>(PropArgs);   \
    extern template __global__ void k_backward_rowlane_imr2<npj>(PropArgs);
JQ_FOR_EACH_ROWLANE(JQ_DECLM)
#undef JQ_DECLM

static int select_rowlane_imr_kernels(jq_handle* h, bool split, prop_kernel_t* fwd, prop_kernel_t* bwd)
{
#define JQ_PICKM(npj)                                                                  \
    if (h->rl_npj == npj) {                                                            \
        *fwd = k_forward_rowlane_imr<npj>;                                             \
        *bwd = split ? k_backward_rowlane_imr2<npj> : k_backward_rowlane_imr<npj>;     \
        return JQ_OK;                                                                  \
    }
    JQ_FOR_EACH_ROWLANE(JQ_PICKM)
// ... 66 lines not shown
```

### juqbox.jl_amd/csrc/jq_kernel_inst.hip

```cpp
#if !defined(JQ_NT) || !defined(JQ_BW) || !defined(JQ_VARIANT)
#error "compile with -DJQ_NT=<tiles> -DJQ_BW=<band> -DJQ_VARIANT=<0..12>"
#endif
#if JQ_VARIANT == 9
#include "jq_cq_split_kernels.h"
template __global__ void k_forward_cq<JQ_NT, false>(PropArgs);
template __global__ void k_backward_cq<JQ_NT, false, false>(PropArgs);
template __global__ void k_backward_cq<JQ_NT, false, true>(PropArgs);
template __global__ void k_forward_cq<JQ_NT, true>(PropArgs);
template __global__ void k_forward_cq<JQ_NT, false, 2>(PropArgs);
template __global__ void k_forward_cq<JQ_NT, true, 2>(PropArgs);
template __global__ void k_backward_cq<JQ_NT, true, false>(PropArgs);
template __global__ void k_backward_cq<JQ_NT, true, true>(PropArgs);
template __global__ void k_forward_cq<JQ_NT, false, 1, true>(PropArgs);
template __global__ void k_forward_cq<JQ_NT, true, 1, true>(PropArgs);
template __global__ void k_backward_cq<JQ_NT, false, false, true>(PropArgs);
template __global__ void k_backward_cq<JQ_NT, false, true, true>(PropArgs);
template __global__ void k_backward_cq<JQ_NT, true, false, true>(PropArgs);
template __global__ void k_backward_cq<JQ_NT, true, true, true>(PropArgs);
template __global__ void k_backward_cq3<JQ_NT, false, false>(PropArgs);
template __global__ void k_backward_cq3<JQ_NT, false, true>(PropArgs);
template __global__ void k_backward_cq3<JQ_NT, true, false>(PropArgs);
template __global__ void k_backward_cq3<JQ_NT, true, true>(PropArgs);
template __global__ void k_backward_cq3<JQ_NT, false, false, 2>(PropArgs);
template __global__ void k_backward_cq3<JQ_NT, false, true, 2>(PropArgs);
template __global__ void k_backward_cq3<JQ_NT, true, false, 2>(PropArgs);
template __global__ void k_backward_cq3<JQ_NT, true, true, 2>(PropArgs);
template __global__ void k_backward_cq3<JQ_NT, false, false, 3, true>(PropArgs);
template __global__ void k_backward_cq3<JQ_NT, false, true, 3, true>(PropArgs);
template __global__ void k_backward_cq3<JQ_NT, true, false, 3, true>(PropArgs);
template __global__ void k_backward_cq3<JQ_NT, true, true, 3, true>(PropArgs);
template __global__ void k_backward_cq3<JQ_NT, false, false, 2, true>(PropArgs);
template __global__ void k_backward_cq3<JQ_NT, false, true, 2, true>(PropArgs);
template __global__ void k_backward_cq3<JQ_NT, true, false, 2, true>(PropArgs);
template __global__ void k_backward_cq3<JQ_NT, true, true, 2, true>(PropArgs);
#if JQ_NT == 2
template __global__ void k_forward_cq<2, false, 1, false, true>(PropArgs);
template __global__ void k_forward_cq<2, true, 1, false, true>(PropArgs);
template __global__ void k_backward_cq<2, false, false, false, true>(PropArgs);
template __global__ void k_backward_cq<2, true, false, false, true>(PropArgs);
template __global__ void k_backward_cq3<2, false, false, 3, false, true>(PropArgs);
template __global__ void k_backward_cq3<2, true, false, 3, false, true>(PropArgs);
template __global__ void k_backward_cq3<2, false, false, 2, false, true>(PropArgs);
template __global__ void k_backward_cq3<2, true, false, 2, false, true>(PropArgs);
#endif
#elif JQ_VARIANT == 12
#include "jq_quad_split_kernels.h"
template __global__ void k_backward_qsplit<JQ_NT, false, 4>(PropArgs);
template __global__ void k_backward_qsplit<JQ_NT, true, 4>(PropArgs);
template __global__ void k_backward_qsplit<JQ_NT, false, 2>(PropArgs);
template __global__ void k_backward_qsplit<JQ_NT, true, 2>(PropArgs);
template __global__ void k_backward_qsplit<JQ_NT, true, 4, true>(PropArgs);
template __global__ void k_backward_qsplit<JQ_NT, true, 2, true>(PropArgs);
#elif JQ_VARIANT == 10
#include "jq_cq_imr_kernels.h"
template __global__ void k_forward_cq_imr<JQ_NT>(PropArgs);
template __global__ void k_backward_cq_imr<JQ_NT>(PropArgs);
template __global__ void k_backward_cq_imr3<JQ_NT>(PropArgs);
#if JQ_NT <= 6
template __global__ void k_backward_cq_imr2<JQ_NT>(PropArgs);
#endif
#if JQ_NT == 2
template __global__ void k_forward_cq_imr<2, true>(PropArgs);
template __global__ void k_backward_cq_imr<2, true>(PropArgs);
template __global__ void k_backward_cq_imr3<2, true>(PropArgs);
#endif
#elif JQ_VARIANT == 7
#include "jq_quad_imr_kernels.h"
template __global__ void k_forward_quad_imr<JQ_NT, 1>(PropArgs);
template __global__ void k_backward_quad_imr<JQ_NT, 1>(PropArgs);
#elif JQ_VARIANT == 6
#include "jq_coop_imr_kernels.h"
template __global__ void k_forward_coop_imr<JQ_NT, JQ_BW, (JQ_NT > 6)>(PropArgs);
template __global__ void k_backward_coop_imr<JQ_NT, JQ_BW, (JQ_NT > 6)>(PropArgs);
#if JQ_NT >= 2
template __global__ void k_forward_coop_imr_parts<JQ_NT, JQ_BW, (JQ_NT > 6)>(PropArgs);
template __global__ void k_backward_coop_imr_parts<JQ_NT, JQ_BW, (JQ_NT > 6)>(PropArgs);
#endif
#if JQ_NT == 6 && JQ_BW == 5
template __global__ void k_forward_coop_imr<6, 5, true>(PropArgs);
template __global__ void k_backward_coop_imr<6, 5, true>(PropArgs);
template __global__ void k_forward_coop_imr_parts<6, 5, true>(PropArgs);
template __global__ void k_backward_coop_imr_parts<6, 5, true>(PropArgs);
#endif
#elif JQ_VARIANT == 5
#include "jq_rowlane_imr_kernels.h"
template __global__ void k_forward_rowlane_imr<JQ_NT>(PropArgs);
template __global__ void k_backward_rowlane_imr<JQ_NT>(PropArgs);
template __global__ void k_backward_rowlane_imr2<JQ_NT>(PropArgs);
#elif JQ_VARIANT == 4
#include "jq_rowlane_kernels.h"
template __global__ void k_forward_rowlane<JQ_NT>(PropArgs);
template __global__ void k_forward_rowlane<JQ_NT, false, true>(PropArgs);
template __global__ void k_backward_rowlane<JQ_NT>(PropArgs);
template __global__ void k_backward_rowlane2<JQ_NT>(PropArgs);
template __global__ void k_backward_rowlane3<JQ_NT>(PropArgs);
template __global__ void k_forward_rowlane<JQ_NT, true, true>(PropArgs);
template __global__ void k_backward_rowlane<JQ_NT, true>(PropArgs);
#elif JQ_VARIANT == 3
#include "jq_lane_kernels.h"
template __global__ void k_forward_lane<JQ_NT>(PropArgs);
template __global__ void k_backward_lane<JQ_NT>(PropArgs);
template __global__ void k_init_state_lane<JQ_NT>(double*, long long, const double*, int, long long);
template __global__ void k_terminal_lane<JQ_NT>(double*, long long, const double*, const double*, int, int, double, double*, const double*, const double*, int);
#elif JQ_VARIANT == 2
#include "jq_coop_kernels.h"
template __global__ void k_forward_coop<JQ_NT, JQ_BW>(PropArgs);
template __global__ void k_backward_coop<JQ_NT, JQ_BW>(PropArgs);
#else
#include "jq_kernels.h"
#ifndef JQ_MINW_MAXNT
#define JQ_MINW_MAXNT 2
#endif
#define JQ_MINW ((JQ_NT <= JQ_MINW_MAXNT) ? 2 : 1)
#if JQ_BW == 7 && JQ_VARIANT == 11
template __global__ void k_forward<JQ_NT, JQ_BW, 1, false, true>(PropArgs);
template __global__ void k_backward<JQ_NT, JQ_BW, 1, false, true>(PropArgs);
#elif JQ_VARIANT == 11
template __global__ void k_forward<JQ_NT, JQ_BW, JQ_MINW, false, true>(PropArgs);
template __global__ void k_backward<JQ_NT, JQ_BW, JQ_MINW, false, true>(PropArgs);
#elif JQ_VARIANT == 13
template __global__ void k_forward<JQ_NT, JQ_BW, JQ_MINW, true, true>(PropArgs);
template __global__ void k_backward<JQ_NT, JQ_BW, JQ_MINW, true, true>(PropArgs);
#elif JQ_BW == 7 && JQ_VARIANT == 8
template __global__ void k_forward<JQ_NT, JQ_BW, 1, false>(PropArgs);
template __global__ void k_backward<JQ_NT, JQ_BW, 1, false>(PropArgs);
template __global__ void k_forward<JQ_NT, JQ_BW, 2, false>(PropArgs);
template __global__ void k_backward<JQ_NT, JQ_BW, 2, false>(PropArgs);
#elif JQ_BW == 7
template __global__ void k_forward<JQ_NT, JQ_BW, 3, false>(PropArgs);
template __global__ void k_backward<JQ_NT, JQ_BW, 3, false>(PropArgs);
template __global__ void k_backward<JQ_NT, JQ_BW, 3, false, false, true>(PropArgs);
template __global__ void k_backward<JQ_NT, JQ_BW, 3, false, false, true, true>(PropArgs);
#else
template __global__ void k_forward<JQ_NT, JQ_BW, JQ_MINW, (JQ_VARIANT == 1)>(PropArgs);
template __global__ void k_backward<JQ_NT, JQ_BW, JQ_MINW, (JQ_VARIANT == 1)>(PropArgs);
#endif
#endif
```

### juqbox.jl_amd/csrc/jq_kernels.h

```cpp
#pragma once
#include <hip/hip_runtime.h>
#include <stdint.h>
#include <type_traits>

typedef double d4 __attribute__((ext_vector_type(4)));

#define JQ_WAVES 4
#define JQ_MAXNC 4
#define JQ_NTR 5
#define JQ_STATE_ARRAYS 4
#define JQ_STATE_EXTRA 8
#define JQ_MAXSLOTS 2
#define JQ_MAXSCHED 30

#define JQ_BW_OD 9
#define JQ_OD_COEFS(NT) (32 * (NT))

#define JQ_BW_T4 8
#define JQ_BW_T4Q 7
#define JQ_T4_AIDX(rho, k, i) (((rho) >> 2) * 64 + 16 * (k) + 4 * ((rho) & 3) + (i))
#define JQ_T4_TILE 16
#define JQ_T4_COEFS(NT) (64 * (NT))
#define JQ_T4_CIDX(g, r, t) ((g) * 16 + (r) * 4 + (t))
#define JQ_T4_CPOS(r, t) (4 * (r) + (t))
// ... 281 lines not shown
    constexpr auto cnt = [on](int r) constexpr { return on(r, 0) + on(r, 1) + on(r, 2) + on(r, 3); };
    constexpr auto act = [on](int r, int k) constexpr {
        for (int t = 0; t < 4; ++t)
            if (on(r, t) && k-- == 0) return t;
        return 0;
    };
    constexpr int NA = cnt(R), NB = cnt(R + 1);
    static_assert((NA == 0) == (NB == 0), "");
    if constexpr (NA > 0) {
#define JQ_XA(k) (k < NA ? xa[act(R, k)] : c)
#define JQ_XB(k) (k < NB ? xb[act(R + 1, k)] : c)
        fma_rowbcast_pair<G, NA, NB, JQ_T4_CPOS(R, act(R, 0)), JQ_T4_CPOS(R, act(R, 1)), JQ_T4_CPOS(R, act(R, 2)), JQ_T4_CPOS(R, act(R, 3)),
                          JQ_T4_CPOS(R + 1, act(R + 1, 0)), JQ_T4_CPOS(R + 1, act(R + 1, 1)), JQ_T4_CPOS(R + 1, act(R + 1, 2)),
                          JQ_T4_CPOS(R + 1, act(R + 1, 3))>(
            accA, accB, c, JQ_XA(0), JQ_XA(1), JQ_XA(2), JQ_XA(3), JQ_XB(0), JQ_XB(1), JQ_XB(2), JQ_XB(3));
#undef JQ_XA
#undef JQ_XB
    }
}
template <int R, bool RT, bool MTM, int G>
__device__ __forceinline__ void t4_couple_pair(double& accA, double& accB, double c, const double (&xa)[4], const double (&xb)[4], bool lo,
                                               bool hi)
{
    if (lo && hi) t4_couple_pair<R, RT, MTM, true, true, G>(accA, accB, c, xa, xb);
    else if (lo) t4_couple_pair<R, RT, MTM, true, false, G>(accA, accB, c, xa, xb);
    else if (hi) t4_couple_pair<R, RT, MTM, false, true, G>(accA, accB, c, xa, xb);
    else t4_couple_pair<R, RT, MTM, false, false, G>(accA, accB, c, xa, xb);
}

template <int NT, bool ZEROC, int MODE>
__device__ __forceinline__ void mm_t4(Arr<NT>& D, const Arr<NT>& C, const double* mat, const Arr<NT>& x)
{
    constexpr int NR = 4 * NT;
    constexpr bool diag = MODE & JQ_T4_DIAG, rt = MODE & JQ_T4_RTERMS, mtm = MODE & JQ_T4_MTERMS;
    const int lane = threadIdx.x & 63;
    const double* cf = mat + NR * JQ_T4_TILE;
    const double* ma = mat - lane + ((lane >> 4) * 16 + (lane & 3));
    double f[JQ_PF];
    double cq[2];
    if constexpr (diag) {
#pragma unroll
        for (int i = 0; i < JQ_PF; ++i)
            if (i < NR) f[i] = ma[JQ_T4_AIDX(i, 0, 0)];
    }
    if constexpr (rt || mtm) {
        cq[0] = cf[0];
        if (NT > 1) cq[1] = cf[64];
    }
    double xo[4] = {0.0, 0.0, 0.0, 0.0};
    double pend[2];
#pragma unroll
    for (int i = 0; i < 2; ++i) {
        pend[i] = ZEROC ? 0.0 : C.t[0][i];
        if constexpr (diag) {
            pend[i] = __builtin_amdgcn_mfma_f64_4x4x4f64(f[i % JQ_PF], x.t[0][i], pend[i], 0, 0, 0);
            if (i + JQ_PF < NR) f[i % JQ_PF] = ma[JQ_T4_AIDX(i + JQ_PF, 0, 0)];
        }
    }
    __builtin_amdgcn_sched_barrier(0);
#pragma unroll
    for (int mt = 0; mt < NT; ++mt) {
        double c = 0.0;
        if constexpr (rt || mtm) {
            c = cq[mt & 1];
            if (mt + 2 < NT) cq[mt & 1] = cf[(mt + 2) * 64];
        }
#pragma unroll
        for (int pr = 0; pr < 2; ++pr) {
            const int r = 2 * pr, rho = 4 * mt + r;
            double curA = pend[0], curB = pend[1];
#pragma unroll
            for (int i = 0; i < 2; ++i) {
                const int nx = rho + 2 + i;
                if (nx < NR) {
                    double nxt = ZEROC ? 0.0 : C.t[nx >> 2][nx & 3];
                    if constexpr (diag) {
                        nxt = __builtin_amdgcn_mfma_f64_4x4x4f64(f[nx % JQ_PF], x.t[nx >> 2][nx & 3], nxt, 0, 0, 0);
                        if (nx + JQ_PF < NR) f[nx % JQ_PF] = ma[JQ_T4_AIDX(nx + JQ_PF, 0, 0)];
                    }
                    pend[i] = nxt;
                }
            }
            __builtin_amdgcn_sched_barrier(0);
            const double xA = x.t[mt][r], xB = x.t[mt][r + 1];
            if constexpr (rt || mtm) {
                const bool hi = mt + 1 < NT;
                const int mu = hi ? mt + 1 : mt;
                const double xa[4] = {xo[(rho + 3) & 3], xB, xo[rho & 3], hi ? x.t[mu][r] : 0.0};
                const double xb[4] = {xA, r + 2 < 4 ? x.t[mt][(r + 2) & 3] : 0.0, xo[(rho + 1) & 3], hi ? x.t[mu][r + 1] : 0.0};
                constexpr int G = diag ? 6 : 2;
                if (rho == 0)
                    t4_couple_pair<0, rt, mtm, G>(curA, curB, c, xa, xb, false, hi);
                else if (pr == 0)
                    t4_couple_pair<0, rt, mtm, 2>(curA, curB, c, xa, xb, mt > 0, hi);
                else
                    t4_couple_pair<2, rt, mtm, 2>(curA, curB, c, xa, xb, mt > 0, hi);
            }
            D.t[mt][r] = curA;
            D.t[mt][r + 1] = curB;
            xo[rho & 3] = xA;
            xo[(rho + 1) & 3] = xB;
            __builtin_amdgcn_sched_barrier(0);
        }
    }
}

template <int CTRL>
__device__ __forceinline__ double row_shift4(double x)
{
    union {
        double d;
        int i[2];
    } a, b;
    a.d = x;
#ifdef JQ_EXP_NOSHIFT
    return x;
#endif
#ifdef JQ_EXP_BPERM
    if (CTRL == 0x114) {
        const int addr = (((int)(threadIdx.x & 63) - 4) & 63) * 4;
        b.i[0] = __builtin_amdgcn_ds_bpermute(addr, a.i[0]);
        b.i[1] = __builtin_amdgcn_ds_bpermute(addr, a.i[1]);
        return b.d;
    }
#endif
#ifdef JQ_EXP_BPERM2
    {
        const int addr = (((int)(threadIdx.x & 63) + (CTRL == 0x114 ? -4 : 4)) & 63) * 4;
        b.i[0] = __builtin_amdgcn_ds_bpermute(addr, a.i[0]);
        b.i[1] = __builtin_amdgcn_ds_bpermute(addr, a.i[1]);
        return b.d;
    }
#endif
    b.i[0] = __builtin_amdgcn_update_dpp(0, a.i[0], CTRL, 0xf, 0xf, true);
    b.i[1] = __builtin_amdgcn_update_dpp(0, a.i[1], CTRL, 0xf, 0xf, true);
    return b.d;
}
typedef double d2 __attribute__((ext_vector_type(2)));
template <int NT>
struct OpQ {
    double a[NT];
    d4 c[NT];
};
__device__ __forceinline__ const double* t4q_a(const double* mat, int lane)
{
    return mat;
}
template <int NT>
__device__ __forceinline__ const d4* t4q_c(const double* mat, int lane)
{
    return (const d4*)(mat - lane + 4 * NT * JQ_T4_TILE + JQ_T4_CIDX(lane >> 4, (lane >> 2) & 3, 0));
}
__device__ __forceinline__ d4 t4q_cload(const d4* cf, int mt) { return cf[mt * 16]; }
template <int NT, bool ZEROC, int MODE>
__device__ __forceinline__ void t4q_block(Arr<NT>& D, const Arr<NT>& C, const Arr<NT>& x, int mt, double a, const d4& c, double& xold)
{
    constexpr bool diag = MODE & JQ_T4_DIAG, rt = MODE & JQ_T4_RTERMS, mtm = MODE & JQ_T4_MTERMS;
    const double xc = x.t[mt][0];
    double acc = ZEROC ? 0.0 : C.t[mt][0];
#ifdef JQ_EXP_MFMA_LAST
    const double xnext = x.t[mt + 1 < NT ? mt + 1 : mt][0];
    if constexpr (rt) {
        acc = fma(c[0], row_shift4<0x114>(xc), acc);
        acc = fma(c[1], row_shift4<0x104>(xc), acc);
    }
    if constexpr (mtm) {
        if (mt > 0) acc = fma(c[2], xold, acc);
        if (mt + 1 < NT) acc = fma(c[3], xnext, acc);
    }
    if constexpr (diag) acc = __builtin_amdgcn_mfma_f64_4x4x4f64(a, xc, acc, 0, 0, 0);
#else
    if constexpr (diag) acc = __builtin_amdgcn_mfma_f64_4x4x4f64(a, xc, acc, 0, 0, 0);
    if constexpr (rt) {
        acc = fma(c[0], row_shift4<0x114>(xc), acc);
        acc = fma(c[1], row_shift4<0x104>(xc), acc);
    }
    if constexpr (mtm) {
        if (mt > 0) acc = fma(c[2], xold, acc);
        if (mt + 1 < NT) acc = fma(c[3], x.t[mt + 1 < NT ? mt + 1 : mt][0], acc);
    }
#endif
    xold = xc;
    D.t[mt][0] = acc;
}
template <int NT, bool ZEROC, int MODE, bool SH = false>
__device__ __forceinline__ void mm_t4q(Arr<NT>& D, const Arr<NT>& C, const double* mat, const Arr<NT>& x, double shd = 0.0,
                                       const double* wsr = nullptr)
{
    constexpr bool diag = MODE & JQ_T4_DIAG, coef = (MODE & (JQ_T4_RTERMS | JQ_T4_MTERMS)) != 0;
    const int lane = threadIdx.x & 63;
    const double* ma = t4q_a(mat, lane);
    const d4* cf = t4q_c<NT>(mat, lane);
    double a_cur = 0.0;
    d4 c_cur = {0.0, 0.0, 0.0, 0.0};
    if constexpr (diag) a_cur = ma[0];
    if constexpr (diag && SH) a_cur = fma(shd, wsr[0], a_cur);
    if constexpr (coef) c_cur = t4q_cload(cf, 0);
    double xold = 0.0;
#ifdef JQ_EXP_NOPF
#pragma unroll
    for (int mt = 0; mt < NT; ++mt) {
        double a = 0.0;
        d4 c = {0.0, 0.0, 0.0, 0.0};
        if constexpr (diag) a = ma[mt * 64];
        if constexpr (coef) c = t4q_cload(cf, mt);
        t4q_block<NT, ZEROC, MODE>(D, C, x, mt, a, c, xold);
        __builtin_amdgcn_sched_barrier(0);
    }
    return;
#endif
#pragma unroll
    for (int mt = 0; mt < NT; ++mt) {
        const double a = a_cur;
        const d4 c = c_cur;
        if (mt + 1 < NT) {
            if constexpr (diag) a_cur = ma[(mt + 1) * 64];
            if constexpr (diag && SH) a_cur = fma(shd, wsr[16 * (mt + 1)], a_cur);
            if constexpr (coef) c_cur = t4q_cload(cf, mt + 1);
        }
        t4q_block<NT, ZEROC, MODE>(D, C, x, mt, a, c, xold);
    }
}
struct T4qNoHook {
    __device__ __forceinline__ void operator()(int, double, double) const {}
};
template <int NT, int NP, bool Z0, bool Z1, bool Z2, int SH = 0, typename HOOK = T4qNoHook>
__device__ __forceinline__ void mm_t4q_multi(Arr<NT>& D0, const Arr<NT>& C0, const double* m0, Arr<NT>& D1, const Arr<NT>& C1,
                                             const double* m1, Arr<NT>& D2, const Arr<NT>& C2, const double* m2, const Arr<NT>& x,
                                             double sh0 = 0.0, double sh1 = 0.0, double sh2 = 0.0, const double* wsr = nullptr,
                                             HOOK hook = HOOK())
{
    const int lane = threadIdx.x & 63;
    const double* ma[3] = {t4q_a(m0, lane), t4q_a(m1, lane), t4q_a(NP > 2 ? m2 : m1, lane)};
    const d4* cf[3] = {t4q_c<NT>(m0, lane), t4q_c<NT>(m1, lane), t4q_c<NT>(NP > 2 ? m2 : m1, lane)};
    double xold = 0.0;
#pragma unroll
    for (int mt = 0; mt < NT; ++mt) {
        double a[3];
        d4 c[3];
#pragma unroll
        for (int k = 0; k < NP; ++k) {
            a[k] = ma[k][mt * 64];
            c[k] = t4q_cload(cf[k], mt);
        }
        if constexpr (SH != 0) {
            const double w = wsr[16 * mt];
            if constexpr (SH & 1) a[0] = fma(sh0, w, a[0]);
            if constexpr (NP > 1 && (SH & 2)) a[1] = fma(sh1, w, a[1]);
            if constexpr (NP > 2 && (SH & 4)) a[2] = fma(sh2, w, a[2]);
        }
        const double xc = x.t[mt][0], xn = x.t[mt + 1 < NT ? mt + 1 : mt][0];
        const double su = row_shift4<0x114>(xc), sd = row_shift4<0x104>(xc);
        hook(mt, su, sd);
        double acc[3] = {Z0 ? 0.0 : C0.t[mt][0], (NP > 1 && !Z1) ? C1.t[mt][0] : 0.0, (NP > 2 && !Z2) ? C2.t[mt][0] : 0.0};
#ifndef JQ_EXP_MFMA_LAST
#pragma unroll
        for (int k = 0; k < NP; ++k) acc[k] = __builtin_amdgcn_mfma_f64_4x4x4f64(a[k], xc, acc[k], 0, 0, 0);
#endif
#pragma unroll
        for (int k = 0; k < NP; ++k) acc[k] = fma(c[k][0], su, acc[k]);
#pragma unroll
        for (int k = 0; k < NP; ++k) acc[k] = fma(c[k][1], sd, acc[k]);
        if (mt > 0) {
#pragma unroll
            for (int k = 0; k < NP; ++k) acc[k] = fma(c[k][2], xold, acc[k]);
        }
        if (mt + 1 < NT) {
#pragma unroll
            for (int k = 0; k < NP; ++k) acc[k] = fma(c[k][3], xn, acc[k]);
        }
#ifdef JQ_EXP_MFMA_LAST
#pragma unroll
        for (int k = 0; k < NP; ++k) acc[k] = __builtin_amdgcn_mfma_f64_4x4x4f64(a[k], xc, acc[k], 0, 0, 0);
#endif
        xold = xc;
        D0.t[mt][0] = acc[0];
        if constexpr (NP > 1) D1.t[mt][0] = acc[1];
        if constexpr (NP > 2) D2.t[mt][0] = acc[2];
        __builtin_amdgcn_sched_barrier(0);
    }
}
template <int NT, bool Z0, bool Z1, int SH = 0>
__device__ __forceinline__ void mm_t4q2(Arr<NT>& D0, const Arr<NT>& C0, const double* m0, Arr<NT>& D1, const Arr<NT>& C1,
                                        const double* m1, const Arr<NT>& x, double sh0 = 0.0, double sh1 = 0.0, const double* wsr = nullptr)
{
    mm_t4q_multi<NT, 2, Z0, Z1, true, SH>(D0, C0, m0, D1, C1, m1, D1, C1, m1, x, sh0, sh1, 0.0, wsr);
}
template <int NT, bool Z0, bool Z1, bool Z2, int SH = 0>
__device__ __forceinline__ void mm_t4q3(Arr<NT>& D0, const Arr<NT>& C0, const double* m0, Arr<NT>& D1, const Arr<NT>& C1,
                                        const double* m1, Arr<NT>& D2, const Arr<NT>& C2, const double* m2, const Arr<NT>& x,
                                        double sh0 = 0.0, double sh1 = 0.0, double sh2 = 0.0, const double* wsr = nullptr)
{
    mm_t4q_multi<NT, 3, Z0, Z1, Z2, SH>(D0, C0, m0, D1, C1, m1, D2, C2, m2, x, sh0, sh1, sh2, wsr);
}
template <int NT>
__device__ __forceinline__ void t4q_load(OpQ<NT>& op, const double* mat)
{
    const int lane = threadIdx.x & 63;
    const double* ma = t4q_a(mat, lane);
    const d4* cf = t4q_c<NT>(mat, lane);
#pragma unroll
    for (int mt = 0; mt < NT; ++mt) {
        op.a[mt] = ma[mt * 64];
#ifdef JQ_EXP_OPQ_EDGE
        const double* cd = (const double*)(cf + mt * 16);
        op.c[mt][0] = cd[0], op.c[mt][1] = cd[1];
        op.c[mt][2] = mt > 0 ? cd[2] : 0.0;
        op.c[mt][3] = mt + 1 < NT ? cd[3] : 0.0;
#else
        op.c[mt] = t4q_cload(cf, mt);
#endif
    }
}
template <int NT>
__device__ __forceinline__ void mm_t4q_regs(Arr<NT>& D, const Arr<NT>& C, const OpQ<NT>& op, const Arr<NT>& x)
{
    double xold = 0.0;
#pragma unroll
    for (int mt = 0; mt < NT; ++mt) t4q_block<NT, false, JQ_T4_DIAG | JQ_T4_RTERMS | JQ_T4_MTERMS>(D, C, x, mt, op.a[mt], op.c[mt], xold);
}

template <int NT, int BW, bool ZEROC, bool SD = false>
__device__ __forceinline__ void mm_band(Arr<NT>& D, const Arr<NT>& C, const double* mat, const Arr<NT>& x);
template <int NT, int BW, bool ZEROC, bool SD = false>
__device__ __forceinline__ void mm_any(Arr<NT>& D, const Arr<NT>& C, const double* mat, const Arr<NT>& x)
{
    if constexpr (BW == JQ_BW_T4)
        mm_t4<NT, ZEROC, JQ_T4_DIAG | JQ_T4_RTERMS | JQ_T4_MTERMS>(D, C, mat, x);
    else if constexpr (BW == JQ_BW_T4Q)
        mm_t4q<NT, ZEROC, JQ_T4_DIAG | JQ_T4_RTERMS | JQ_T4_MTERMS>(D, C, mat, x);
    else if constexpr (BW == JQ_BW_OD)
        mm_od<NT, ZEROC, SD>(D, C, mat, x);
    else
        mm_band<NT, BW, ZEROC, SD>(D, C, mat, x);
}
template <int NT, int BW, bool ZEROC, bool SD>
__device__ __forceinline__ void mm_band(Arr<NT>& D, const Arr<NT>& C, const double* mat, const Arr<NT>& x)
{
    constexpr int NTILES = band_tiles(NT, BW, SD);
    double f[JQ_PF];
#pragma unroll
    for (int i = 0; i < JQ_PF; ++i)
        if (i < NTILES) f[i] = mat[i * 64];
    int idx = 0;
#pragma unroll
    for (int kk = 0; kk < 4 * NT; ++kk) {
#pragma unroll
        for (int mt = 0; mt < NT; ++mt) {
            if (block_on(BW, SD, mt, kk >> 2)) {
                const double a = f[idx % JQ_PF];
                if (idx + JQ_PF < NTILES) f[idx % JQ_PF] = mat[(idx + JQ_PF) * 64];
                const bool first = (kk == 4 * first_kb(NT, BW, SD, mt));
                const d4 zero = {0.0, 0.0, 0.0, 0.0};
                const d4 cin = first ? (ZEROC ? zero : C.t[mt]) : D.t[mt];
                D.t[mt] = __builtin_amdgcn_mfma_f64_16x16x4f64(a, x.t[kk >> 2][kk & 3], cin, 0, 0, 0);
                __builtin_amdgcn_sched_barrier(0);
                ++idx;
            }
        }
    }
    if (ZEROC) {
#pragma unroll
        for (int mt = 0; mt < NT; ++mt)
            if (first_kb(NT, BW, SD, mt) >= NT) D.t[mt] = (d4){0.0, 0.0, 0.0, 0.0};
    }
}
template <int NT, int BW>
__device__ __forceinline__ void mm_c(Arr<NT>& D, const Arr<NT>& C, const double* mat, const Arr<NT>& x)
{
    mm_any<NT, BW, false>(D, C, mat, x);
}
template <int NT, int BW>
__device__ __forceinline__ void mm_z(Arr<NT>& D, const double* mat, const Arr<NT>& x)
{
    mm_any<NT, BW, true>(D, D, mat, x);
}
template <int NT, int BW>
__device__ __forceinline__ void mm_z_bw(Arr<NT>& D, const double* mat, const Arr<NT>& x, int mode)
{
    if constexpr (BW == JQ_BW_T4) {
        switch (mode) {
        case JQ_T4_DIAG: mm_t4<NT, true, JQ_T4_DIAG>(D, D, mat, x); break;
        case JQ_T4_RTERMS: mm_t4<NT, true, JQ_T4_RTERMS>(D, D, mat, x); break;
        case JQ_T4_MTERMS: mm_t4<NT, true, JQ_T4_MTERMS>(D, D, mat, x); break;
        default: mm_t4<NT, true, JQ_T4_DIAG | JQ_T4_RTERMS | JQ_T4_MTERMS>(D, D, mat, x); break;
        }
    } else if constexpr (BW == JQ_BW_T4Q) {
        switch (mode) {
        case JQ_T4_DIAG: mm_t4q<NT, true, JQ_T4_DIAG>(D, D, mat, x); break;
        case JQ_T4_RTERMS: mm_t4q<NT, true, JQ_T4_RTERMS>(D, D, mat, x); break;
        case JQ_T4_MTERMS: mm_t4q<NT, true, JQ_T4_MTERMS>(D, D, mat, x); break;
        default: mm_t4q<NT, true, JQ_T4_DIAG | JQ_T4_RTERMS | JQ_T4_MTERMS>(D, D, mat, x); break;
        }
    } else {
        if (BW > 0 && mode == 0)
            mm_any<NT, 0, true>(D, D, mat, x);
        else if (BW > 0 && NT > 1 && mode == 2)
            mm_any<NT, BW, true, true>(D, D, mat, x);
        else
            mm_any<NT, BW, true>(D, D, mat, x);
    }
}

template <int N>
__device__ __forceinline__ double row_ror_add(double x)
{
    union {
        double d;
        int i[2];
    } a, b;
    a.d = x;
    b.i[0] = __builtin_amdgcn_update_dpp(0, a.i[0], 0x120 + N, 0xf, 0xf, false);
    b.i[1] = __builtin_amdgcn_update_dpp(0, a.i[1], 0x120 + N, 0xf, 0xf, false);
    return x + b.d;
}
__device__ __forceinline__ double lane_bcast(double x, int l)
{
    union {
        double d;
        int i[2];
    } a, b;
    a.d = x;
    b.i[0] = __builtin_amdgcn_readlane(a.i[0], l);
    b.i[1] = __builtin_amdgcn_readlane(a.i[1], l);
    return b.d;
}
__device__ __forceinline__ double wave_sum(double x)
{
    x = row_ror_add<8>(x);
    x = row_ror_add<4>(x);
    x = row_ror_add<2>(x);
    x = row_ror_add<1>(x);
    return (lane_bcast(x, 0) + lane_bcast(x, 16)) + (lane_bcast(x, 32) + lane_bcast(x, 48));
}

__device__ __forceinline__ double wave_sum_hi(double x)
{
    x = row_ror_add<8>(x);
    x = row_ror_add<4>(x);
    x = row_ror_add<2>(x);
    x = row_ror_add<1>(x);
    union {
        double d;
        int i[2];
    } a, b;
    a.d = x;
    b.i[0] = __builtin_amdgcn_update_dpp(0, a.i[0], 0x142, 0xa, 0xf, false);
    b.i[1] = __builtin_amdgcn_update_dpp(0, a.i[1], 0x142, 0xa, 0xf, false);
    x += b.d;
    a.d = x;
    b.i[0] = __builtin_amdgcn_update_dpp(0, a.i[0], 0x143, 0xc, 0xf, false);
    b.i[1] = __builtin_amdgcn_update_dpp(0, a.i[1], 0x143, 0xc, 0xf, false);
    return x + b.d;
}

typedef unsigned jq_u2 __attribute__((ext_vector_type(2)));
__device__ __forceinline__ void row_swap32(double& a, double& b)
{
    union { double d; unsigned u[2]; } x, y;
    x.d = a, y.d = b;
    const jq_u2 lo = __builtin_amdgcn_permlane32_swap(x.u[0], y.u[0], false, false);
    const jq_u2 hi = __builtin_amdgcn_permlane32_swap(x.u[1], y.u[1], false, false);
    x.u[0] = lo[0], y.u[0] = lo[1], x.u[1] = hi[0], y.u[1] = hi[1];
    a = x.d, b = y.d;
}
__device__ __forceinline__ void row_swap16(double& a, double& b)
{
    union { double d; unsigned u[2]; } x, y;
    x.d = a, y.d = b;
    const jq_u2 lo = __builtin_amdgcn_permlane16_swap(x.u[0], y.u[0], false, false);
    const jq_u2 hi = __builtin_amdgcn_permlane16_swap(x.u[1], y.u[1], false, false);
    x.u[0] = lo[0], y.u[0] = lo[1], x.u[1] = hi[0], y.u[1] = hi[1];
// ... 393 lines not shown
                if (sl >= TPS) sl -= TPS;
                off = sl * (unsigned)slot_bytes + kind * stride_b;
            }
            qword >>= 6;
            if (Q >= npro) {
                ++iq;
                if (iq == 10) qword = sb1;
                if (iq == 20) qword = sb2;
                if (iq == period) {
                    iq = 0;
                    qword = sb0;
                }
            } else if (Q + 1 == npro) {
                qword = sb0;
            }
            ++Q;
            return (const double*)(smem + off) + lane;
        }
        if (batch > 0) {
            int kind, tp;
            entry_at(Q, ip, kind, tp);
            const int n = (Q < npro) ? 0 : np;
            if (kind == 2) {
                M = (const double*)(smem + 2 * (size_t)slot_bytes) + (size_t)tp * stride;
            } else {
                const int b = n / batch, nl = n - b * batch;
                M = (const double*)(smem + (size_t)(b & 1) * slot_bytes) + (size_t)(2 * (2 * nl + tp) + kind) * stride;
            }
            advance(Q, np, ip);
            return M + lane;
        }
        if (!(debug & 8)) {
            asm volatile("s_waitcnt vmcnt(0) lgkmcnt(0)" ::: "memory");
            __builtin_amdgcn_s_barrier();
            asm volatile("" ::: "memory");
            issue_prefetch<KPER>();
        }
        M = (const double*)(smem + (size_t)(Q & 1) * slot_bytes) + lane;
        ++Q;
        return M;
    }
    template <int KIND, int TP>
    __device__ __forceinline__ const double* next_ks()
    {
        if constexpr (WIN) __builtin_amdgcn_sched_barrier(0);
        if (WIN || batch < 0) return (const double*)(smem + ((TP == 0 ? wb0 : TP == 1 ? wb1 : wb2) + KIND * stride_b)) + lane;
        return next();
    }
    __device__ __forceinline__ const double* next_c(int idx)
    {
        if constexpr (WIN) __builtin_amdgcn_sched_barrier(0);
        if (WIN || batch < 0) return (const double*)(smem + ((unsigned)(TPS * slot_bytes) + (unsigned)idx * stride_b)) + lane;
        return next();
    }
    __device__ __forceinline__ void drain()
    {
        asm volatile("s_waitcnt vmcnt(0) lgkmcnt(0)" ::: "memory");
        __builtin_amdgcn_s_barrier();
        asm volatile("" ::: "memory");
    }
};
typedef RingT<false> Ring;


template <int NT>
__device__ __forceinline__ double a_diff2(const Arr<NT>& x, const Arr<NT>& y)
{
    double s = 0.0;
#pragma unroll
    for (int i = 0; i < NT; ++i) {
        const auto d = x.t[i] - y.t[i];
        s += row_sum(d * d);
    }
    return s;
}

__device__ __forceinline__ double sample_sum(double x, int N)
{
    x += __shfl_xor(x, 16);
    x += __shfl_xor(x, 32);
    const int lane = threadIdx.x & 63, col = lane & 15;
    const int n = N < 16 ? N : 16, c0 = col - col % n;
    double s = 0.0;
    for (int k = 0; k < n; ++k) {
        const double v = __shfl(x, (lane & 48) | ((c0 + k) & 15));
        s += (c0 + k < 16) ? v : 0.0;
    }
    return s;
}

__device__ __forceinline__ double jacobi_wg_sum(double r, int jac_wg, int it)
{
    extern __shared__ __attribute__((aligned(16))) char jq_smem_[];
    double* ex = (double*)(jq_smem_ + jac_wg) + (it & 1) * JQ_WAVES;
    const int wave = threadIdx.x >> 6, nw = blockDim.x >> 6;
    if ((threadIdx.x & 63) == 0) ex[wave] = r;
    asm volatile("s_waitcnt lgkmcnt(0)" ::: "memory");
    __builtin_amdgcn_s_barrier();
    asm volatile("" ::: "memory");
    double s = 0.0;
    for (int w = 0; w < nw; ++w) s += ex[w];
    return s;
}
template <int NT, int BW>
__device__ __forceinline__ void jacobi_add(Arr<NT>& out, const Arr<NT>& bpa, const Arr<NT>& A, const double* S, int max_iter,
                                           double tol2, Arr<NT>& Ya, Arr<NT>& Yb, int ncol, int jac_wg = -1)
{
    if (max_iter <= 0) {
        out = bpa;
        return;
    }
    if (jac_wg >= 0) {
        __builtin_amdgcn_s_barrier();
        mm_c<NT, BW>(Ya, A, S, A);
        bool in_a = true;
        bool done = jacobi_wg_sum(sample_sum(a_diff2(Ya, A), ncol), jac_wg, 1) < tol2;
        for (int j = 2; j <= max_iter && !done; ++j) {
            if (in_a) {
                mm_c<NT, BW>(Yb, A, S, Ya);
                done = jacobi_wg_sum(sample_sum(a_diff2(Yb, Ya), ncol), jac_wg, j) < tol2;
            } else {
                mm_c<NT, BW>(Ya, A, S, Yb);
                done = jacobi_wg_sum(sample_sum(a_diff2(Ya, Yb), ncol), jac_wg, j) < tol2;
            }
            in_a = !in_a;
        }
#pragma unroll
        for (int i = 0; i < NT; ++i) out.t[i] = (bpa.t[i] - A.t[i]) + (in_a ? Ya.t[i] : Yb.t[i]);
        return;
    }
    mm_c<NT, BW>(Ya, A, S, A);
    bool in_a = true;
    bool done = sample_sum(a_diff2(Ya, A), ncol) < tol2;
    for (int j = 2; j <= max_iter && !__all(done); ++j) {
        if (in_a) {
            mm_c<NT, BW>(Yb, A, S, Ya);
            const bool conv = sample_sum(a_diff2(Yb, Ya), ncol) < tol2;
#pragma unroll
            for (int i = 0; i < NT; ++i) Yb.t[i] = done ? Ya.t[i] : Yb.t[i];
            done = done || conv;
        } else {
            mm_c<NT, BW>(Ya, A, S, Yb);
            const bool conv = sample_sum(a_diff2(Ya, Yb), ncol) < tol2;
#pragma unroll
            for (int i = 0; i < NT; ++i) Ya.t[i] = done ? Yb.t[i] : Ya.t[i];
            done = done || conv;
        }
        in_a = !in_a;
    }
#pragma unroll
    for (int i = 0; i < NT; ++i) out.t[i] = (bpa.t[i] - A.t[i]) + (in_a ? Ya.t[i] : Yb.t[i]);
}

template <int NT, int BW, bool JAC, bool REGOP = true>
__device__ __forceinline__ void horner_add(Arr<NT>& out, const Arr<NT>& bpa, const Arr<NT>& A, const double* S, int m,
                                           Arr<NT>& Ya, Arr<NT>& Yb, double jacobi_tol2, int ncol, int jac_wg = -1)
{
    if (JAC) {
        jacobi_add<NT, BW>(out, bpa, A, S, m, jacobi_tol2, Ya, Yb, ncol, jac_wg);
        return;
    }
    if (m <= 0) {
        out = bpa;
        return;
    }
    int rem = m - 1;
    if (rem == 0) {
        mm_c<NT, BW>(out, bpa, S, A);
        return;
    }
#ifdef JQ_EXP_NOOPQ
    if constexpr (false) {
#else
    if constexpr (BW == JQ_BW_T4Q && REGOP) {
#endif
        OpQ<NT> op;
        t4q_load(op, S);
        mm_t4q_regs(Ya, A, op, A);
        for (--rem; rem >= 2; rem -= 2) {
            mm_t4q_regs(Ya, A, op, Ya);
            mm_t4q_regs(Ya, A, op, Ya);
        }
        if (rem > 0) mm_t4q_regs(Ya, A, op, Ya);
        mm_t4q_regs(out, bpa, op, Ya);
        return;
    }
    mm_c<NT, BW>(Ya, A, S, A);
    --rem;
    if constexpr (BW == JQ_BW_OD || BW == JQ_BW_T4 || BW == JQ_BW_T4Q) {
        for (; rem > 0; --rem) mm_c<NT, BW>(Ya, A, S, Ya);
        mm_c<NT, BW>(out, bpa, S, Ya);
        return;
    }
    while (rem >= 2) {
        mm_c<NT, BW>(Yb, A, S, Ya);
        mm_c<NT, BW>(Ya, A, S, Yb);
        rem -= 2;
    }
    if (rem == 1) {
        mm_c<NT, BW>(Yb, A, S, Ya);
        mm_c<NT, BW>(out, bpa, S, Yb);
    } else {
        mm_c<NT, BW>(out, bpa, S, Ya);
    }
}

#ifndef JQ_BWD_TERMS
#define JQ_BWD_TERMS 1
#endif
constexpr bool jq_bwd_terms(int NT, int BW, bool JAC) { return JQ_BWD_TERMS && !JAC && NT >= 6 && BW != JQ_BW_OD && BW != JQ_BW_T4 && BW != JQ_BW_T4Q; }
template <int NT, int BW>
__device__ __forceinline__ void neumann_terms_add(Arr<NT>& out, Arr<NT>& A, const double* S, int m, Arr<NT>& Ya)
{
    for (int j = 0; j < m; j += 2) {
        mm_z<NT, BW>(Ya, S, A);
        a_add(out, Ya);
        if (j + 1 < m) {
            mm_z<NT, BW>(A, S, Ya);
            a_add(out, A);
        }
    }
}

template <int NT>
__device__ __forceinline__ void a_park(const Arr<NT>& a, __attribute__((address_space(3))) double* park)
{
#pragma unroll
    for (int i = 0; i < NT; ++i)
#pragma unroll
        for (int r = 0; r < JQ_RL; ++r) park[(JQ_RL * i + r) * 64] = a.t[i][r];
}
template <int NT>
__device__ __forceinline__ void a_unpark(Arr<NT>& a, const __attribute__((address_space(3))) double* park)
{
#pragma unroll
    for (int i = 0; i < NT; ++i)
#pragma unroll
        for (int r = 0; r < JQ_RL; ++r) a.t[i][r] = park[(JQ_RL * i + r) * 64];
}
template <int NT>
__device__ __forceinline__ void a_park(const Arr<NT>& a, double* park)
{
#pragma unroll
    for (int i = 0; i < NT; ++i)
#pragma unroll
        for (int r = 0; r < JQ_RL; ++r) park[(JQ_RL * i + r) * 64] = a.t[i][r];
}
template <int NT>
__device__ __forceinline__ void a_unpark(Arr<NT>& a, const double* park)
{
#pragma unroll
    for (int i = 0; i < NT; ++i)
#pragma unroll
        for (int r = 0; r < JQ_RL; ++r) a.t[i][r] = park[(JQ_RL * i + r) * 64];
}

#ifndef JQ_FWD_FUSE
#define JQ_FWD_FUSE 3
#endif
#ifndef JQ_BWD_FUSE
#define JQ_BWD_FUSE 3
#endif
#ifndef JQ_BWD_FUSE3
#define JQ_BWD_FUSE3 0
#endif
#ifndef JQ_BWD_ADJ_FUSE
#define JQ_BWD_ADJ_FUSE 1
#endif
#ifndef JQ_BWD3_NOOPQ
#define JQ_BWD3_NOOPQ 0
#endif
#ifndef JQ_BWD3_NOOPQ_STATE
#define JQ_BWD3_NOOPQ_STATE 0
#endif
template <int NT, int BW, bool JAC, int FUSE = 0, bool FOLD = false, bool REGOP = true, bool TERMS = false, typename RING = RingT<BW == JQ_BW_T4Q>>
__device__ __forceinline__ void sv_state(RING& p, const PropArgs& a, bool active, double ceps, const double* ws, int g,
                                         const Arr<NT>& u, Arr<NT>& v, Arr<NT>& unew, Arr<NT>& vN, Arr<NT>& A, Arr<NT>& Ya,
                                         Arr<NT>& Yb)
{
    if constexpr (BW == JQ_BW_T4Q && !JAC && FUSE != 0) {
        const double* M0 = p.template next_ks<0, 1>();
        const double* M1 = p.template next_ks<1, 0>();
        if (active) {
            if constexpr (FOLD) {
                static_assert(!FOLD || (FUSE & 3) == 3 || FUSE == 0, "FOLD: fused or generic path");
                mm_t4q2<NT, true, false, 1>(A, A, M0, unew, u, M1, u, ceps, 0.0, ws + g);
            } else {
            if constexpr (FUSE & 1) {
                mm_t4q2<NT, true, false>(A, A, M0, unew, u, M1, u);
            } else {
                mm_z<NT, BW>(A, M0, u);
                mm_c<NT, BW>(unew, u, M1, u);
            }
            if (a.use_shift) a_axpy_rows(A, ceps, ws, g, u);
            }
        }
        M0 = p.template next_ks<1, 1>();
        if (active) {
            mm_c<NT, BW>(A, A, M0, v);
            a_add(v, A);
            horner_add<NT, BW, JAC, REGOP>(v, v, A, M0, a.m, Ya, Yb, a.jacobi_tol2, a.N, a.jac_wg_lds);
        }
        M1 = p.template next_ks<0, 0>();
        const double* M2 = p.template next_ks<0, 2>();
        if (active) {
            if constexpr (FOLD) {
                mm_t4q3<NT, false, false, true, 6>(vN, v, M0, unew, unew, M1, A, A, M2, v, 0.0, -ceps, -ceps, ws + g);
            } else {
            if constexpr (FUSE & 2) {
                mm_t4q3<NT, false, false, true>(vN, v, M0, unew, unew, M1, A, A, M2, v);
            } else {
                mm_c<NT, BW>(vN, v, M0, v);
                mm_c<NT, BW>(unew, unew, M1, v);
                mm_z<NT, BW>(A, M2, v);
            }
            if (a.use_shift) {
                a_axpy_rows(unew, -ceps, ws, g, v);
                a_axpy_rows(A, -ceps, ws, g, v);
            }
            }
        }
        M0 = p.template next_ks<1, 2>();
        if (active) {
            mm_c<NT, BW>(A, A, M0, unew);
            a_add(unew, A);
            horner_add<NT, BW, JAC, REGOP>(unew, unew, A, M0, a.m, Ya, Yb, a.jacobi_tol2, a.N, a.jac_wg_lds);
        }
        return;
    }
    constexpr int FULLQ = JQ_T4_DIAG | JQ_T4_RTERMS | JQ_T4_MTERMS;
    const double* M = p.template next_ks<0, 1>();
    if (active) {
        if constexpr (FOLD) {
            mm_t4q<NT, true, FULLQ, true>(A, A, M, u, ceps, ws + g);
        } else {
            mm_z<NT, BW>(A, M, u);
            if (a.use_shift) a_axpy_rows(A, ceps, ws, g, u);
        }
    }
    M = p.template next_ks<1, 1>();
    if (active) {
        mm_c<NT, BW>(A, A, M, v);
        a_add(v, A);
        if constexpr (TERMS) neumann_terms_add<NT, BW>(v, A, M, a.m, Ya);
        else horner_add<NT, BW, JAC, REGOP>(v, v, A, M, a.m, Ya, Yb, a.jacobi_tol2, a.N, a.jac_wg_lds);
        mm_c<NT, BW>(vN, v, M, v);
    }
    M = p.template next_ks<0, 0>();
    if (active) {
        if constexpr (FOLD) {
            mm_t4q<NT, false, FULLQ, true>(unew, u, M, v, -ceps, ws + g);
        } else {
            mm_c<NT, BW>(unew, u, M, v);
            if (a.use_shift) a_axpy_rows(unew, -ceps, ws, g, v);
        }
    }
    M = p.template next_ks<1, 0>();
    if (active) mm_c<NT, BW>(unew, unew, M, u);
    M = p.template next_ks<0, 2>();
    if (active) {
        if constexpr (FOLD) {
            mm_t4q<NT, true, FULLQ, true>(A, A, M, v, -ceps, ws + g);
        } else {
            mm_z<NT, BW>(A, M, v);
            if (a.use_shift) a_axpy_rows(A, -ceps, ws, g, v);
        }
    }
    M = p.template next_ks<1, 2>();
    if (active) {
        mm_c<NT, BW>(A, A, M, unew);
        a_add(unew, A);
        if constexpr (TERMS) neumann_terms_add<NT, BW>(unew, A, M, a.m, Ya);
        else horner_add<NT, BW, JAC, REGOP>(unew, unew, A, M, a.m, Ya, Yb, a.jacobi_tol2, a.N, a.jac_wg_lds);
    }
}

template <int BW, bool JAC, bool WLRT>
constexpr bool jq_wlr_on() { return WLRT; }
template <int NT, int BW, int MINW, bool JAC, bool WLRT = false, bool UNI = false>
__global__ __launch_bounds__((BW == JQ_BW_T4Q) ? 256 * MINW : 256, (BW == JQ_BW_T4Q) ? 1 : MINW) void k_forward(PropArgs a)
{
    extern __shared__ __attribute__((aligned(16))) char smem[];
    constexpr int KT = 4 * NT;
    const int lane_ = threadIdx.x & 63;
    const int wave = __builtin_amdgcn_readfirstlane(threadIdx.x >> 6);
    constexpr bool QUAD = (BW == JQ_BW_T4Q);
    constexpr int NWAVES = QUAD ? JQ_WAVES * MINW : JQ_WAVES;
    const int col = QUAD ? 4 * (wave & 3) + (lane_ & 3) : (lane_ & 15);
    const int lane = QUAD ? ((lane_ >> 2) & 3) * 64 + 16 * (lane_ >> 4) + col : lane_;
    const int g = QUAD ? 4 * (lane_ >> 4) + ((lane_ >> 2) & 3) : lane_ >> 4;
    const int wpw = (JAC && !QUAD) ? (int)(blockDim.x >> 6) : JQ_WAVES;
    const int slab = QUAD ? (int)blockIdx.x * (NWAVES / 4) + (wave >> 2) : blockIdx.x * wpw + wave;
    const bool active = slab < a.nslabs;

    double* tab = (double*)(smem + a.lds_tab_off);
    const double* wd = tab;
    const double* ws = tab + 16 * NT;
    for (int i = threadIdx.x; i < 32 * NT; i += blockDim.x) tab[(i & ~15) + 4 * (i & 3) + ((i >> 2) & 3)] = a.tabs[i];

    Arr<NT> ua, va, ub, vb, A, Ya, Yb;
    double leak = 0.0, ceps = 0.0;
    double* st = a.state + (size_t)(active ? slab : 0) * a.state_stride;
    if (active) {
        a_load(ua, st, lane);
        a_load(va, st + KT * 64, lane);
        leak = (!QUAD || ((lane_ >> 2) & 3) == 0) ? st[(JQ_STATE_ARRAYS * KT + JQ_MAXNC) * 64 + (QUAD ? 16 * (lane_ >> 4) + col : lane)] : 0.0;
        ceps = 0.5 * a.h * a.colinfo[(size_t)slab * 32 + col];
        if constexpr (UNI) ceps = (a.use_shift && (lane_ >> 4) == (lane_ & 3)) ? lane_bcast(ceps, 0) : 0.0;
    } else {
        a_zero(ua);
        a_zero(va);
    }
    RingT<QUAD> p;
    p.init(smem, a, wave, lane_, QUAD ? NWAVES : wpw);
    constexpr bool WLR = jq_wlr_on<BW, JAC, WLRT>();
    WLow<NT, QUAD> wl;
    if constexpr (WLR) wl.init(a, lane_, smem);

#define JQ_FWD_STEP(U, V, UN, VN, NSTEP)                                                                         \
    {                                                                                                            \
        p.begin_step(NSTEP);                                                                                     \
        if (active) leak += a_wsq(wd, g, U);                   \
        sv_state<NT, BW, JAC, JQ_FWD_FUSE, UNI>(p, a, active, ceps, ws, g, U, V, UN, VN, A, Ya, Yb);                  \
                                                \
        const double* M6 = p.template next_ks<0, 1>();                                                                             \
        if (active) {                                                                                            \
            if constexpr (UNI) {                                                                                 \
                mm_t4q<NT, false, JQ_T4_DIAG | JQ_T4_RTERMS | JQ_T4_MTERMS, true>(VN, VN, M6, UN, ceps, ws + g);   \
            } else {                                                                                             \
                mm_c<NT, BW>(VN, VN, M6, UN);                                                                    \
                if (a.use_shift) a_axpy_rows(VN, ceps, ws, g, UN);                                               \
            }                                                                                                    \
                   \
            leak += a_wsq(wd, g, UN) + 2.0 * a_wsq(wd, g, V);                                                    \
            if constexpr (WLR)                                                                                   \
                if (wl.r > 0) {    \
                    double lk = 0.0;                                                                             \
                    for (int k = 0; k < wl.r; ++k) {                                                             \
                        double p0, q0, p1, q1, rr, ss;                                                           \
                        if (wl.has_sc) p0 = wl.get(k, 0), q0 = wl.get(k, 1);       \
                        else wl.dots(k, U, p0, q0);                                                              \
                        wl.dots(k, UN, p1, q1);                                                                  \
                        if (wl.has_sc) wl.put(k, 0, p1), wl.put(k, 1, q1);                                       \
                        wl.dots(k, V, rr, ss);                                                                   \
                        lk += wl.lam(k) * ((p0 * p0 + q0 * q0) + (p1 * p1 + q1 * q1) + 2.0 * (rr * rr + ss * ss) - 2.0 * (ss * p0 - rr * q0)); \
                    }                                                                                            \
                    if (wl.lead) leak += lk;                                                                     \
                }                                                                                                \
            if (a.hist_r) hist_store<NT>(a, slab, col, QUAD ? 4 * ((lane_ >> 2) & 3) + (lane_ >> 4) : g, NSTEP, UN, VN); \
        }                                                                                                        \
    }
    if constexpr (WLR)
        if (wl.has_sc && active)
            for (int k = 0; k < wl.r; ++k) {
                double p0, q0;
                wl.dots(k, ua, p0, q0);
                wl.put(k, 0, p0), wl.put(k, 1, q0);
            }
    int n = 0;
    for (; n + 1 < a.nsteps_chunk; n += 2) {
        JQ_FWD_STEP(ua, va, ub, vb, n)
        JQ_FWD_STEP(ub, vb, ua, va, n + 1)
    }
    if (n < a.nsteps_chunk) {
        JQ_FWD_STEP(ua, va, ub, vb, n)
        if (active) {
            ua = ub;
            va = vb;
        }
    }
#undef JQ_FWD_STEP
    p.drain();
    if (active) {
        a_store(ua, st, lane);
        a_store(va, st + KT * 64, lane);
        if constexpr (QUAD) {
            leak = row_ror_add<8>(row_ror_add<4>(leak));
            if (((lane_ >> 2) & 3) == 0) st[(JQ_STATE_ARRAYS * KT + JQ_MAXNC) * 64 + 16 * (lane_ >> 4) + col] = leak;
        } else {
            st[(JQ_STATE_ARRAYS * KT + JQ_MAXNC) * 64 + lane] = leak;
        }
    }
}

template <int NT, int BW, int MINW, bool JAC, bool WLRT = false, bool UNI = false, bool ORD = false>
__global__ __launch_bounds__((BW == JQ_BW_T4Q) ? 256 * MINW : 256, (BW == JQ_BW_T4Q) ? 1 : MINW) void k_backward(PropArgs a)
{
    static_assert(!ORD || (UNI && BW == JQ_BW_T4Q && !JAC), "ORD: a variant of the UNI quad-layout kernel");
    extern __shared__ __attribute__((aligned(16))) char smem[];
    constexpr int KT = 4 * NT;
    const int lane_ = threadIdx.x & 63;
    const int wave = __builtin_amdgcn_readfirstlane(threadIdx.x >> 6);
    constexpr bool QUAD = (BW == JQ_BW_T4Q);
    constexpr int NWAVES = QUAD ? JQ_WAVES * MINW : JQ_WAVES;
    constexpr int NTHREADS = 64 * NWAVES;
    const int col = QUAD ? 4 * (wave & 3) + (lane_ & 3) : (lane_ & 15);
    const int lane = QUAD ? ((lane_ >> 2) & 3) * 64 + 16 * (lane_ >> 4) + col : lane_;
    const int g = QUAD ? 4 * (lane_ >> 4) + ((lane_ >> 2) & 3) : lane_ >> 4;
    const int wpw = (JAC && !QUAD) ? (int)(blockDim.x >> 6) : JQ_WAVES;
    const int slab = QUAD ? (int)blockIdx.x * (NWAVES / 4) + (wave >> 2) : blockIdx.x * wpw + wave;
    const bool active = slab < a.nslabs;
    const int Nc = a.Ncoupled;
    const bool cslot = !QUAD || ((lane_ >> 2) & 3) == 0;
    const int clane = QUAD ? 16 * (lane_ >> 4) + col : lane_;

    double* tab = (double*)(smem + a.lds_tab_off);
    const double* wd = tab;
    const double* ws = tab + 16 * NT;
    double* carry = tab + 32 * NT;
    const double cfw = a.forced ? 0.5 * a.h * a.tinv : 0.0;
    for (int i = threadIdx.x; i < 32 * NT; i += blockDim.x)
        tab[(i & ~15) + 4 * (i & 3) + ((i >> 2) & 3)] = (i < 16 * NT) ? cfw * a.tabs[i] : a.tabs[i];
    double* st = a.state + (size_t)(active ? slab : 0) * a.state_stride;
    typedef __attribute__((address_space(3))) double lds_double;
    typedef typename std::conditional<QUAD, lds_double*, double*>::type park_ptr;
    park_ptr P0;
    if constexpr (QUAD)
        P0 = (lds_double*)(carry + Nc * NTHREADS + (size_t)wave * (JQ_RL * NT) * 64 + lane_);
    else
        P0 = a.park_lds ? (carry + Nc * NTHREADS + (size_t)wave * (JQ_RL * NT) * 64 + lane_)
                        : (a.park + (size_t)(active ? slab : 0) * KT * 64 + lane);
    const int ntr = Nc * JQ_NTR;
    double* rec = carry + Nc * NTHREADS + (a.park_lds ? (size_t)NWAVES * (JQ_RL * NT) * 64 : 0);
    const int rslots = 8 * Nc;
    for (int i = threadIdx.x; i < 2 * NWAVES * rslots; i += blockDim.x) rec[i] = 0.0;
    auto flush_traces = [&](int k) {
        if (!QUAD && a.batch > 0) {
            asm volatile("s_waitcnt lgkmcnt(0)" ::: "memory");
            __builtin_amdgcn_s_barrier();
            asm volatile("" ::: "memory");
        }
        if (wave == 0 && lane_ < ntr) {
            const int q = lane_ / JQ_NTR, kk = lane_ - q * JQ_NTR;
            const int slot = (kk == 0 ? 0 : kk == 2 ? 2 : 4 * Nc + (kk == 1 ? 0 : kk == 3 ? 2 : 1)) + 4 * q;
            const double* r = rec + (size_t)(k & 1) * NWAVES * rslots + slot;
            double s = r[0];
#pragma unroll
            for (int w = 1; w < NWAVES; ++w) s += r[w * rslots];
            a.traces[((size_t)blockIdx.x * a.nsteps_chunk + k) * ntr + lane_] = s;
        }
    };

    Arr<NT> u, v, mu, nb, un, vN, L, Ya, Yb;
    double ceps = 0.0, wgt = 0.0;
    if (active) {
        a_load(u, st, lane);
        a_load(v, st + KT * 64, lane);
        a_load(mu, st + 2 * KT * 64, lane);
        a_load(nb, st + 3 * KT * 64, lane);
        ceps = 0.5 * a.h * a.colinfo[(size_t)slab * 32 + col];
        wgt = a.colinfo[(size_t)slab * 32 + 16 + col];
        if constexpr (UNI) {
            wgt = lane_bcast(wgt, 0);
            ceps = (a.use_shift && (lane_ >> 4) == (lane_ & 3)) ? lane_bcast(ceps, 0) : 0.0;
        }
        for (int q = 0; q < Nc; ++q) carry[q * NTHREADS + threadIdx.x] = cslot ? st[(JQ_STATE_ARRAYS * KT + q) * 64 + clane] : 0.0;
    } else {
        a_zero(u);
        a_zero(v);
        a_zero(mu);
        a_zero(nb);
    }
    RingT<QUAD> p;
    p.init(smem, a, wave, lane_, QUAD ? NWAVES : wpw);
    constexpr bool WLR = jq_wlr_on<BW, JAC, WLRT>();
    WLow<NT, QUAD> wl;
    if constexpr (WLR) wl.init(a, lane_, smem);
    const bool wforce = WLR && a.wrank > 0 && a.forced;
    constexpr bool BREG = !(QUAD && MINW >= 3 && JQ_BWD3_NOOPQ);

    if (a.first_chunk) {
        for (int q = 0; q < Nc; ++q) {
            const double* M = p.next_c(q);
            if (active) {
                mm_z_bw<NT, BW>(Ya, M, nb, a.bw_trace[q]);
                carry[q * NTHREADS + threadIdx.x] = -a_dot(u, Ya);
            }
        }
    }

    if constexpr (WLR)
        if (wforce && wl.has_sc && active)
            for (int k = 0; k < wl.r; ++k) {
                double pu, qu;
                wl.dots(k, u, pu, qu);
                wl.put(k, 0, pu), wl.put(k, 1, qu);
            }
    for (int n = 0; n < a.nsteps_chunk; ++n) {
        p.begin_step(n);
        if (active) a_park(mu, P0);
        sv_state<NT, BW, JAC, (MINW >= 3 ? (UNI ? 3 : JQ_BWD_FUSE3) : JQ_BWD_FUSE), UNI, !(QUAD && MINW >= 3 && JQ_BWD3_NOOPQ_STATE), jq_bwd_terms(NT, BW, JAC)>(p, a, active, ceps, ws, g, u, v, un, vN, mu, Ya, Yb);
        if (n > 0) flush_traces(n - 1);
        const double* M = p.template next_ks<0, 1>();
        if (active) {
            if constexpr (UNI) {
                constexpr int FULLQ = JQ_T4_DIAG | JQ_T4_RTERMS | JQ_T4_MTERMS;
                mm_t4q<NT, false, FULLQ, true>(vN, vN, M, un, ceps, ws + g);
                mm_t4q<NT, true, FULLQ, true>(L, L, M, nb, ceps, ws + g);
            } else {
                mm_c<NT, BW>(vN, vN, M, un);
                if (a.use_shift) a_axpy_rows(vN, ceps, ws, g, un);
                mm_z<NT, BW>(L, M, nb);
                if (a.use_shift) a_axpy_rows(L, ceps, ws, g, nb);
            }
            a_unpark(mu, P0);
            a_park(vN, P0);
        }
        M = p.template next_ks<1, 0>();
        if (active) {
            mm_c<NT, BW>(L, L, M, mu);
            a_axpy_rows1<NT, false>(L, wd, g, u);
            if constexpr (WLR)
                if (wforce)
                    for (int k = 0; k < wl.r; ++k) {
                        double pu, qu;
                        if (wl.has_sc) pu = wl.get(k, 0), qu = wl.get(k, 1);
                        else wl.dots(k, u, pu, qu);
                        const double cl = cfw * wl.lam(k);
                        wl.axpy2(k, L, cl * pu, cl * qu);
                    }
            a_add(mu, L);
            if constexpr (jq_bwd_terms(NT, BW, JAC)) neumann_terms_add<NT, BW>(mu, L, M, a.m, Ya);
            else horner_add<NT, BW, JAC, BREG>(mu, mu, L, M, a.m, Ya, Yb, a.jacobi_tol2, a.N, a.jac_wg_lds);
        }
        double o_p4 = 0.0;
        for (int q = 0; q < Nc; ++q) {
            M = p.next_c(Nc + q);
            if (active) {
                if constexpr (ORD) {
                    if (q == 0) mm_t4q<NT, true, JQ_T4_DIAG>(Ya, Ya, M, mu);
                    else if (q == 1) mm_t4q<NT, true, JQ_T4_RTERMS>(Ya, Ya, M, mu);
                    else mm_t4q<NT, true, JQ_T4_MTERMS>(Ya, Ya, M, mu);
                } else {
                    mm_z_bw<NT, BW>(Ya, M, mu, a.bw_trace[q]);
                }
                const double ts = UNI ? wave_sum4(a_dot(u, Ya), a_dot(un, Ya), 0.0, 0.0) * wgt
                                      : wave_sum4(a_dot(u, Ya) * wgt, a_dot(un, Ya) * wgt, 0.0, 0.0);
                if ((lane_ & 15) == 0) rec[((size_t)(n & 1) * NWAVES + wave) * rslots + 4 * q + (lane_ >> 4)] = ts;
            }
        }
        if constexpr (QUAD && !JAC && (JQ_BWD_ADJ_FUSE & 1)) {
            M = p.template next_ks<0, 0>();
            const double* M9 = p.template next_ks<0, 2>();
            if (active) {
                if constexpr (UNI) {
                    mm_t4q2<NT, true, true, 3>(L, L, M, vN, vN, M9, mu, -ceps, -ceps, ws + g);
                } else {
                    mm_t4q2<NT, true, true>(L, L, M, vN, vN, M9, mu);
                    if (a.use_shift) {
                        a_axpy_rows(L, -ceps, ws, g, mu);
                        a_axpy_rows(vN, -ceps, ws, g, mu);
                    }
                }
            }
        } else {
        M = p.template next_ks<0, 0>();
        if (active) {
            mm_z<NT, BW>(L, M, mu);
            if (a.use_shift) a_axpy_rows(L, -ceps, ws, g, mu);
        }
        M = p.template next_ks<0, 2>();
        if (active) {
            mm_z<NT, BW>(vN, M, mu);
            if (a.use_shift) a_axpy_rows(vN, -ceps, ws, g, mu);
        }
        }
        M = p.template next_ks<1, 1>();
        if (active) {
            mm_z<NT, BW>(Ya, M, nb);
            a_axpy_rows1<NT, true>(Ya, wd, g, v);
            if constexpr (WLR)
                if (wforce)
                    for (int k = 0; k < wl.r; ++k) {
                        double pn, qn, rr, ss;
                        wl.dots(k, un, pn, qn);
                        wl.dots(k, v, rr, ss);
                        if (wl.has_sc) wl.put(k, 2, pn), wl.put(k, 3, qn), wl.put(k, 4, rr), wl.put(k, 5, ss);
                        const double cl = cfw * wl.lam(k);
                        wl.axpy2(k, Ya, -cl * rr, -cl * ss);
                        wl.axpy2(k, vN, -cl * qn, cl * pn);
                    }
            a_add(L, Ya);
            a_add(vN, Ya);
            mm_c<NT, BW>(vN, vN, M, L);
            a_add(L, nb);
            a_add(L, vN);
            if constexpr (jq_bwd_terms(NT, BW, JAC)) neumann_terms_add<NT, BW>(L, vN, M, a.m, Ya);
            else horner_add<NT, BW, JAC, BREG>(L, L, vN, M, a.m, Ya, Yb, a.jacobi_tol2, a.N, a.jac_wg_lds);
            a_add(nb, L);
        }
        M = p.template next_ks<0, 1>();
        if (active) {
            if constexpr (ORD) {
                const d4* cfs = t4q_c<NT>(p.next_c(1), lane_);
                mm_t4q_multi<NT, 1, false, true, true, 1>(vN, mu, M, vN, mu, M, vN, mu, M, L, ceps, 0.0, 0.0, ws + g,
                                                          [&](int mt, double su, double sd) {
                                                              const d4 cs = t4q_cload(cfs, mt);
                                                              o_p4 = fma(-un.t[mt][0], fma(cs[1], sd, cs[0] * su), o_p4);
                                                          });
            } else if constexpr (UNI) {
                mm_t4q<NT, false, JQ_T4_DIAG | JQ_T4_RTERMS | JQ_T4_MTERMS, true>(vN, mu, M, L, ceps, ws + g);
            } else {
                mm_c<NT, BW>(vN, mu, M, L);
                if (a.use_shift) a_axpy_rows(vN, ceps, ws, g, L);
            }
        }
        M = p.template next_ks<1, 2>();
        if (active) {
            mm_c<NT, BW>(vN, vN, M, mu);
            a_axpy_rows1<NT, false>(vN, wd, g, un);
            if constexpr (WLR)
                if (wforce)
                    for (int k = 0; k < wl.r; ++k) {
                        double pn, qn, rr, ss;
                        if (wl.has_sc) {
                            pn = wl.get(k, 2), qn = wl.get(k, 3), rr = wl.get(k, 4), ss = wl.get(k, 5);
                            wl.put(k, 0, pn), wl.put(k, 1, qn);
                        } else {
                            wl.dots(k, un, pn, qn);
                            wl.dots(k, v, rr, ss);
                        }
                        const double cl = cfw * wl.lam(k);
                        wl.axpy2(k, vN, cl * (pn - ss), cl * (qn + rr));
                    }
        }
        for (int q = 0; q < Nc; ++q) {
            double t2 = 0, t4 = 0, t5 = 0;
            const int bwq = a.bw_trace[q];
            M = p.next_c(Nc + q);
            if (active) {
                if constexpr (ORD) {
                    if (q == 0) mm_t4q<NT, true, JQ_T4_DIAG>(Ya, Ya, M, nb);
                    else if (q == 1) mm_t4q<NT, true, JQ_T4_RTERMS>(Ya, Ya, M, nb);
                    else mm_t4q<NT, true, JQ_T4_MTERMS>(Ya, Ya, M, nb);
                } else {
                    mm_z_bw<NT, BW>(Ya, M, nb, bwq);
                }
                t5 = -a_dot(v, Ya);
            }
            M = p.next_c(q);
            if (active) {
                double p4;
                if constexpr (ORD) {
                    if (q == 1) {
                        mm_t4q<NT, true, JQ_T4_RTERMS>(Ya, Ya, M, mu);
                        t2 = a_dot(v, Ya);
                        p4 = o_p4;
                    } else {
                        if (q == 0) mm_t4q<NT, true, JQ_T4_DIAG>(Ya, Ya, M, mu);
                        else mm_t4q<NT, true, JQ_T4_MTERMS>(Ya, Ya, M, mu);
                        t2 = a_dot(v, Ya);
                        if (q == 0) mm_t4q<NT, true, JQ_T4_DIAG>(Ya, Ya, M, L);
                        else mm_t4q<NT, true, JQ_T4_MTERMS>(Ya, Ya, M, L);
                        p4 = -a_dot(un, Ya);
                    }
                } else {
                    mm_z_bw<NT, BW>(Ya, M, mu, bwq);
                    t2 = a_dot(v, Ya);
                    mm_z_bw<NT, BW>(Ya, M, L, bwq);
                    p4 = -a_dot(un, Ya);
                }
                t4 = p4 + carry[q * NTHREADS + threadIdx.x];
                carry[q * NTHREADS + threadIdx.x] = p4;
                const double ts = UNI ? wave_sum4(t2, t4, t5, 0.0) * wgt : wave_sum4(t2 * wgt, t4 * wgt, t5 * wgt, 0.0);
                if ((lane_ & 15) == 0) rec[((size_t)(n & 1) * NWAVES + wave) * rslots + 4 * (Nc + q) + (lane_ >> 4)] = ts;
            }
        }
        if (active) {
            u = un;
            mu = vN;
            nb = L;
            a_unpark(v, P0);
        }
    }
    p.drain();
    flush_traces(a.nsteps_chunk - 1);
    if (active) {
        a_store(u, st, lane);
        a_store(v, st + KT * 64, lane);
        a_store(mu, st + 2 * KT * 64, lane);
        a_store(nb, st + 3 * KT * 64, lane);
        for (int q = 0; q < Nc; ++q) {
            double cv = carry[q * NTHREADS + threadIdx.x];
            if constexpr (QUAD) cv = row_ror_add<8>(row_ror_add<4>(cv));
            if (cslot) st[(JQ_STATE_ARRAYS * KT + q) * 64 + clane] = cv;
        }
    }
}
```

### juqbox.jl_amd/csrc/jq_options.h

```cpp
#pragma once
#include <climits>
#include <cstdlib>
#include <cstring>
#include <string>

enum JqOpt {
    O_T4, O_OD, O_T4BIG, O_FORCE_DENSE, O_WINDOW, O_LANE, O_LANE_MIN, O_LANE_MAX, O_ROWLANE_MAX, O_COOP_MAX, O_QUAD, O_CQ, O_EMBED,
    O_STREAM_BYTES, O_CHUNK_STEPS, O_BATCH,
    O_DQ, O_NOSPLIT, O_QUAD8, O_CQ_W, O_IMR_CQ, O_IMR_CQ2, O_CQ_FWD2, O_CQ3, O_QSPLIT, O_RL_SPLIT, O_JAC_WG, O_TRACE_BYTES, O_NO_UNI, O_NO_ORD,
    O_QS_RIDE, O_CQ_GENERIC_TRACES, O_WLR_SC, O_RCCL_SELFCHECK, O_MULTI_SAME_DEVICE, O_CQ3_RDV_US, O_CQ3_WAIT_MS,
    O_DEBUG, O_CQ3_FAULT,
    O_COUNT
};

#define JQ_OPT_UNSET LLONG_MIN
#define JQ_OPT_PLAN 1u
#define JQ_OPT_HOOK 2u
#define JQ_OPT_EXP 4u

struct JqOptDesc {
    const char* name;
    long long dflt;
    unsigned flags;
    const char* doc;
};

static const JqOptDesc g_jq_opt[O_COUNT] = {
    {"t4", 1, JQ_OPT_PLAN, "0: no 4 x 4 x n variant (4x4 diagonal blocks on v_mfma_f64_4x4x4); falls back to diagonal off-diagonal blocks"},
    {"od", 1, JQ_OPT_PLAN, "0: no diagonal-off-diagonal-block and no 4 x 4 x n variant (plain block-band tiles)"},
    {"t4big", 1, JQ_OPT_PLAN, "0: 4 x 4 x 7 / 4 x 4 x 8 structures (Ntot 97 .. 128) on the general Ntot > 96 cooperative kernels"},
    {"force_dense", 0, JQ_OPT_PLAN, "1: no structure exploitation at all (all 16x16 tiles)"},
    {"window", 1, JQ_OPT_PLAN, "0: per-operator LDS ring instead of the window staging"},
    {"lane", 1, JQ_OPT_PLAN, "0: no lane / row-lane kernels (Ntot <= 16 on the MFMA kernels)"},
    {"lane_min", JQ_OPT_UNSET, JQ_OPT_PLAN, "smallest column count routed to the lane kernels"},
    {"lane_max", JQ_OPT_UNSET, JQ_OPT_PLAN, "largest column count routed to the lane kernels"},
    {"rowlane_max", JQ_OPT_UNSET, JQ_OPT_PLAN, "largest column count routed to the row-lane kernels (0: never)"},
    {"coop_max", JQ_OPT_UNSET, JQ_OPT_PLAN, "cooperative kernels for batches of at most n slabs (default #CU; 0: never)"},
    {"quad", JQ_OPT_UNSET, JQ_OPT_PLAN, "quad-layout kernels for batches of at most n slabs (0: never; default: whenever the round count favours them)"},
    {"cq", JQ_OPT_UNSET, JQ_OPT_PLAN, "cooperative-quad (latency) kernels for batches of at most n column quads (0: never; default 2 #CU)"},
    {"embed", 1, JQ_OPT_PLAN, "structure embedding (d1 x d2 x d3 zero-padded to 4 x 4 x n): 0 off, 1 for batches of the MFMA families, 2 for every batch"},
    {"stream_bytes", JQ_OPT_UNSET, JQ_OPT_PLAN, "bytes of the operator tile stream of one chunk (default 1 GiB)"},
    {"chunk_steps", JQ_OPT_UNSET, JQ_OPT_PLAN, "time steps per chunk (default: what the tile stream holds)"},
    {"batch", JQ_OPT_UNSET, JQ_OPT_PLAN | JQ_OPT_EXP, "batched staging of B time steps per DMA burst (measured: no gain)"},
    {"dq", 1, JQ_OPT_PLAN, "0: no dense cooperative-quad kernels (17 .. 32 levels without the 4 x 4 x n structure: small batches on the cooperative kernels)"},
    {"nosplit", 0, 0, "1: evaluate an ensemble as ONE batch even when full rounds + a remainder on other kernels would be faster"},
    {"quad8", JQ_OPT_UNSET, 0, "force 1 / 2 / 3 slabs per quad-layout workgroup (value 0 / 1 / 2)"},
    {"cq_w", 1, 0, "0: full leakage weights that fit four slots on the quad-layout kernels instead of the cooperative-quad ones"},
    {"imr_cq", 1, 0, "0: implicit midpoint, N = 4, on the quad-layout kernels instead of the cooperative-quad ones"},
    {"imr_cq2", 1, 0, "0: implicit midpoint, cooperative quad: the one-set backward kernel (bit-identical)"},
    {"cq_fwd2", JQ_OPT_UNSET, 0, "cooperative-quad forward sweep with one (0) / two (1) column quads per workgroup (default: two beyond #CU quads; bit-identical)"},
    {"cq3", JQ_OPT_UNSET, 0, "cooperative-quad backward sweep: 0 the one-workgroup kernel, 3 three workgroups per quad or none (default: three / two / one by batch size; bit-identical)"},
    {"qsplit", JQ_OPT_UNSET, 0, "quad-layout backward sweep on two waves per quad: 0 off (one-wave kernel, bit-identical), 2 two quads per workgroup for every batch of the cooperative-quad plan"},
    {"rl_split", 1, 0, "row-lane backward sweep: 0 = one wave, 1 = the library's rule (Stormer-Verlet: three or four waves -- state | adjoint | traces; implicit midpoint: two while idle SIMDs remain), 2 / 3 = two / three at every batch size (all bit-identical)"},
    {"jac_wg", 1, 0, "0: Jacobi solver, N > 16: convergence per 16-column part instead of per sample"},
    {"trace_bytes", JQ_OPT_UNSET, 0, "bytes of the per-step trace records of one backward chunk (default 4 GiB): smaller = more, shorter chunks"},
    {"no_uni", 0, 0, "1: three-slab quad-layout backward sweep on the generic kernel (tests compare)"},
    {"no_ord", 0, 0, "1: no single-subsystem-control specialisation of the quad-layout backward kernels (tests compare)"},
    {"qs_ride", JQ_OPT_UNSET, 0, "split quad-layout backward kernel: trace products as separate passes (0) / riding along also at four quads per workgroup (1)"},
    {"cq_generic_traces", 0, 0, "1: cooperative-quad backward sweep with full trace products even when every control acts on one subsystem"},
    {"wlr_sc", 0, JQ_OPT_EXP, "1: full weights, quad layout: carry the column dots of a step in LDS (measured slower)"},
    {"rccl_selfcheck", 1, 0, "multi-device handles: 0 never, 1 on the first all-reduce, 2 on every all-reduce compare RCCL's result with the host-order sum (3: test mode)"},
    {"multi_same_device", 0, 0, "TEST MODE of jq_create_multi: 1 = up to 16 sub-handles may share physical GPUs, host-side sum in place of the all-reduce"},
    {"cq3_rdv_us", JQ_OPT_UNSET, 0, "two- / three-workgroup latency kernels: microseconds the workgroups of a launch wait for each other at its start before the launch is abandoned and the evaluation repeated on one workgroup per quad (default: one launch duration, 2 .. 100 ms)"},
    {"cq3_wait_ms", JQ_OPT_UNSET, 0, "two- / three-workgroup latency kernels: milliseconds a wait between roles may take after a passed rendezvous before the launch is declared dead (default: 10 x the launch's expected duration, at least 50 ms)"},
    {"debug", 0, JQ_OPT_HOOK, "bit 16 / 32: the consumer roles / the state role of the split latency kernels start ~ 5 ms late (results unchanged); bits 1, 2, 4, 8: profiling experiments with WRONG results (experiment builds only)"},
    {"cq3_fault", 0, JQ_OPT_HOOK, "1: the split latency kernels report a dead wait, 3: a failed start-up rendezvous (exercises fall-back and cool-down)"},
};

struct JqOptions {
    long long v[O_COUNT];
    JqOptions()
    {
        for (int i = 0; i < O_COUNT; ++i) v[i] = JQ_OPT_UNSET;
    }
    bool has(int o) const { return v[o] != JQ_OPT_UNSET; }
    long long get(int o) const { return v[o] != JQ_OPT_UNSET ? v[o] : g_jq_opt[o].dflt; }
    bool on(int o) const { return get(o) != 0; }
    static int find(const char* name, size_t len)
    {
        for (int i = 0; i < O_COUNT; ++i)
            if (strlen(g_jq_opt[i].name) == len && strncmp(g_jq_opt[i].name, name, len) == 0) return i;
        return -1;
    }
    bool set(int o, long long value, std::string* err)
    {
#ifndef JQ_EXPERIMENTS
        if ((g_jq_opt[o].flags & JQ_OPT_EXP) && value != JQ_OPT_UNSET && value != g_jq_opt[o].dflt) {
            *err = std::string("option '") + g_jq_opt[o].name + "' exists in experiment builds only (-DJQ_EXPERIMENTS)";
            return false;
        }
        if (o == O_DEBUG && value != JQ_OPT_UNSET && (value & ~48LL)) {
            *err = "option 'debug': only the test hooks 16 / 32 exist in release builds (the other bits change results)";
            return false;
        }
#endif
        v[o] = value;
        return true;
    }
    bool parse(const char* s, std::string* err)
    {
        if (!s) return true;
        while (*s) {
            while (*s == ',' || *s == ';' || *s == ' ' || *s == '\t' || *s == '\n') ++s;
            if (!*s) break;
            const char* e = s;
            while (*e && *e != '=' && *e != ',' && *e != ';' && *e != ' ') ++e;
            if (*e != '=') {
                *err = std::string("options: '") + std::string(s, e - s) + "' is not of the form name=value";
                return false;
            }
            const int o = find(s, (size_t)(e - s));
            if (o < 0) {
                *err = std::string("options: unknown option '") + std::string(s, e - s) + "'";
                return false;
            }
            char* end = nullptr;
            const long long val = strtoll(e + 1, &end, 0);
            if (end == e + 1) {
                *err = std::string("options: '") + g_jq_opt[o].name + "' needs an integer value";
                return false;
            }
            if (!set(o, val, err)) return false;
            s = end;
        }
        return true;
    }
    std::string str() const
    {
        std::string r;
        for (int i = 0; i < O_COUNT; ++i)
            if (has(i)) r += (r.empty() ? "" : ",") + std::string(g_jq_opt[i].name) + "=" + std::to_string(v[i]);
        return r;
    }
};
```

### juqbox.jl_amd/csrc/juqbox_hip.hip

```cpp
#include "../../include/juqbox_hip.h"
#include "jq_aux_kernels.h"
#include "jq_coop_kernels.h"
#include "jq_kernels.h"
#include "jq_lane_kernels.h"
#include "jq_rowlane_kernels.h"
#include "jq_rowlane_imr_kernels.h"
#include "jq_coop_imr_kernels.h"
#include "jq_huge_kernels.h"
#include "jq_options.h"

#include <rccl/rccl.h>

#include <dlfcn.h>

#include <algorithm>
#include <chrono>
#include <cmath>
#include <cstdio>
#include <cstdlib>
#include <cstring>
#include <condition_variable>
#include <mutex>
#include <string>
#include <thread>
#include <vector>

#ifndef JQ_SRC_HASH
#define JQ_SRC_HASH "unknown"
#endif
#ifndef JQ_CODE_HASH
#define JQ_CODE_HASH "unknown"
#endif
#define JQ_VERSION "gfx950 juqbox_hip 0.4.0 src:" JQ_SRC_HASH " code:" JQ_CODE_HASH
#ifndef JQ_MINW_MAXNT
#define JQ_MINW_MAXNT 2
#endif

static thread_local std::string g_create_error;
static bool debug_timing()
{
    static const bool on = getenv("JQ_DEBUG_TIMING") != nullptr;
    return on;
}

extern "C" const char jq_build_manifest[];

struct jq_handle {
    int device = 0;
    JqOptions opt;
    hipStream_t stream = nullptr;
    int Ntot = 0, N = 0, Nc = 0, Nfreq = 0, nsteps = 0, m = 0, objFuncType = 1;
    int integrator = 1;
    int imr_max_iter = 100;
    double imr_tol = 1e-12;
    int solver_id = 1;
    double solver_tol = 0.0;
    double T = 0.0;
    int NT = 0, KT = 0, NP = 0, sps = 0;
    int parts = 1;
    int BW = 0;
    int BWc = 0;
    int NcK = 0;
    std::vector<int> bw_trace;
    long long mat_elems = 0;
    long long mat_elems_c = 0;
    bool coop_ok = false;
    int coop_max_slabs = 256;
    long long state_stride = 0;
    int nslots = 2;
    int nslots_bwd = 2;
    int park_lds = 0;
    int batch = 0;
    bool big = false;
    bool huge = false;
    bool force_plain = false;
    bool replanned = false;
    bool in_split = false;
    double* d_pk2 = nullptr;
    size_t cap_pk2 = 0;
    int dq_max_quads = 0;
    double *d_himg_dq = nullptr, *d_cimg_dq = nullptr;
    int cq_max_quads = 0;
    int quad_max_slabs = 0;
    int num_cu = 256;
    int lane_np = 0;
    long long lane_stride = 0;
    int lane_min_cols = 0, lane_max_cols = 0;
    int rl_npj = 0;
    long long rl_stride = 0;
    int rl_max_cols = 0;
    std::vector<double> Hconst, Hsym, Hanti, Uinit, Utr, Uti, wd, cfreq;
    int sv_type = 1;
    std::vector<double> dVr, dVi;
    bool dv_stale = true, dv_alloc = false;
    double *d_dvr = nullptr, *d_dvi = nullptr, *d_dvr_l = nullptr, *d_dvi_l = nullptr, *d_dvr_r = nullptr, *d_dvi_r = nullptr;
    std::vector<double> rfreq;
    double* d_rfreq = nullptr;
    int wrank = 0;
    int wlam = JQ_MAX_WRANK;
    std::vector<double> Wr, Wi, wlr;
    double* d_wlr = nullptr;
    bool wlr_real = false;
    std::vector<double> tf, tb;
    double *d_cimg = nullptr, *d_park = nullptr;
    double* d_cq3 = nullptr;
    size_t cap_cq3 = 0;
    bool cq3_off = false;
    int cq3_faults = 0;
    int cq3_faults_xcd = 0;
    int cq3_busy = 0;
    int cq3_busy_streak = 0;
    double cq3_us_per_step = 0.0;
    int cq3_skip = 0;
    std::string cq3_last;
    double* d_qsplit = nullptr;
    size_t cap_qsplit = 0;
    double *d_himg_c = nullptr, *d_cimg_c = nullptr;
    double *d_himg_l = nullptr, *d_uinit_l = nullptr, *d_vtr_l = nullptr, *d_vti_l = nullptr;
    double *d_himg_r = nullptr, *d_uinit_r = nullptr, *d_vtr_r = nullptr, *d_vti_r = nullptr;
    double *d_cimg_l = nullptr, *d_cimg_r = nullptr;
    double *d_himg = nullptr, *d_uimg = nullptr, *d_vtr = nullptr, *d_vti = nullptr, *d_tabs = nullptr;
    double *d_tf = nullptr, *d_tb = nullptr, *d_cfreq = nullptr, *d_pcof = nullptr;
    double *d_stream = nullptr, *d_pq = nullptr;
    double *d_state = nullptr, *d_state_save = nullptr, *d_colinfo = nullptr, *d_traces = nullptr, *d_R = nullptr;
    double *d_grad = nullptr, *d_res = nullptr;
    double *d_wq = nullptr, *d_pack = nullptr;
    size_t cap_pcof = 0, cap_slabs = 0, cap_traces = 0, cap_grad = 0, cap_res = 0, cap_state = 0, cap_colinfo = 0, cap_wq = 0, cap_pack = 0;
    int chunk_steps = 0;
    jq_handle* emb = nullptr;
    std::vector<int> emb_row;
    int emb_mode = 1;
    bool is_emb = false;
    std::vector<jq_handle*> subs;
    std::vector<ncclComm_t> comms;
    bool host_reduce = false;
    bool comm_broken = false;
    int rccl_checks = 0;
    std::vector<hipEvent_t> ev;
    std::string err;
    jq_timing timing = {};
};

#define HIPCHK(h, call)                                                                              \
    do {                                                                                             \
        hipError_t e_ = (call);                                                                      \
        if (e_ != hipSuccess) {                                                                      \
            char buf_[512];                                                                          \
            snprintf(buf_, sizeof buf_, "HIP error '%s' at %s:%d (%s)", hipGetErrorString(e_), __FILE__, __LINE__, #call); \
            (h)->err = buf_;                                                                         \
            return JQ_EHIP;                                                                          \
        }                                                                                            \
    } while (0)

static int fail(jq_handle* h, int code, const char* msg)
{
    h->err = msg;
    return code;
}

static int ctrl_ngroups(int Nc) { return (Nc + JQ_MAXNC - 1) / JQ_MAXNC; }
static int ctrl_gstart(int Nc, int g)
{
    const int ng = ctrl_ngroups(Nc), base = Nc / ng, rem = Nc % ng;
    return g * base + std::min(g, rem);
}

struct DeviceGuard {
    int prev = -1;
    DeviceGuard() { if (hipGetDevice(&prev) != hipSuccess) prev = -1; }
    ~DeviceGuard() { if (prev >= 0) (void)hipSetDevice(prev); }
};

#include "jq_host_images.h"
#include "jq_host_create.h"
#include "jq_host_update.h"
#include "jq_host_select.h"
#include "jq_host_plan.h"
#include "jq_host_eval.h"
extern "C" int jq_traceobjgrad(jq_handle* h, const double* pcof, int32_t ncoeff, int32_t evaladjoint, double* out4,
                               double* totalgrad, double* infidelgrad, double* leakgrad)
{
    if (!h) return JQ_EINVAL;
    if (!pcof || !out4) return fail(h, JQ_EINVAL, "jq_traceobjgrad: NULL pointer");
    if (evaladjoint && (!totalgrad || !infidelgrad || !leakgrad))
        return fail(h, JQ_EINVAL, "jq_traceobjgrad: gradient outputs are required when evaladjoint != 0");
    JQ_ON_FIRST(h, jq_traceobjgrad(s0_, pcof, ncoeff, evaladjoint, out4, totalgrad, infidelgrad, leakgrad))
    EvalOut o;
    int rc = run_eval(h, pcof, ncoeff, 1, nullptr, nullptr, nullptr, evaladjoint != 0, nullptr, nullptr, &o);
    if (rc) return rc;
    const double primary = o.res[0], secondary = o.res[1];
    out4[0] = primary + secondary;
    out4[1] = primary;
    out4[2] = secondary;
    out4[3] = primary;
    if (evaladjoint) {
        for (int i = 0; i < ncoeff; ++i) totalgrad[i] = o.grad0[i];
        if (h->objFuncType != 1) {
            for (int i = 0; i < ncoeff; ++i) {
                infidelgrad[i] = o.grad1[i];
                leakgrad[i] = o.grad0[i] - o.grad1[i];
            }
        } else {
            for (int i = 0; i < ncoeff; ++i) {
                infidelgrad[i] = o.grad0[i];
                leakgrad[i] = 0.0;
            }
        }
    }
    return JQ_OK;
}

extern "C" int jq_state_history(jq_handle* h, const double* pcof, int32_t ncoeff, double* ur, double* ui)
{
    return jq_traceobj_verbose(h, pcof, ncoeff, nullptr, ur, ui);
}

// ... 184 lines not shown
```

Before: 2959.

## Use compact uniform S-operand loads in three-slab quad-layout kernels

At plan time the code checks whether the tiled antisymmetric operator images are the same across block rows (s_uniform). When they are, new kernel variants load the diagonal scalar and the first coefficient pair once and read only the varying coefficient pair per block. This cuts per-block memory loads and lets Horner iterations keep the operator in registers. The cost is extra template instantiations, register pressure from holding the operator, and a result that depends on the uniformity check being correct.

```diff
diff --git a/include/juqbox_hip.h b/include/juqbox_hip.h
--- a/include/juqbox_hip.h
+++ b/include/juqbox_hip.h
@@ -128,6 +128,8 @@
 
 int jq_plan_info(const jq_handle *h, char *buf, int32_t buflen);
 
+int jq_s_uniform(const double *Hanti_ops, int32_t Ntot, int32_t Ncoupled);
+
 int jq_last_timing(const jq_handle *h, jq_timing *t);
 const char *jq_version(void);
 int jq_abi_version(void);
diff --git a/juqbox.jl_amd/_lib.py b/juqbox.jl_amd/_lib.py
--- a/juqbox.jl_amd/_lib.py
+++ b/juqbox.jl_amd/_lib.py
@@ -75,6 +75,7 @@
     "jq_shard_bounds": (ctypes.c_int, [c_i32, c_i32, c_i32, ctypes.POINTER(ctypes.c_int32), ctypes.POINTER(ctypes.c_int32)]),
     "jq_traceobj_sweep": (ctypes.c_int, [ctypes.c_void_p, c_dp, c_i32, c_dp, c_i32, c_dp, c_dp]),
     "jq_plan_info": (ctypes.c_int, [ctypes.c_void_p, ctypes.c_char_p, c_i32]),
+    "jq_s_uniform": (ctypes.c_int, [c_dp, c_i32, c_i32]),
     "jq_last_timing": (ctypes.c_int, [ctypes.c_void_p, ctypes.POINTER(jq_timing)]),
     "jq_version": (ctypes.c_char_p, []),
     "jq_abi_version": (ctypes.c_int, []),
diff --git a/juqbox.jl_amd/csrc/jq_host_create.h b/juqbox.jl_amd/csrc/jq_host_create.h
--- a/juqbox.jl_amd/csrc/jq_host_create.h
+++ b/juqbox.jl_amd/csrc/jq_host_create.h
@@ -24,6 +24,7 @@
     return rc;
 }
 
+static bool hanti_s_uniform(const double* Hanti, int Ntot, int NT, int Nc);
 static int upload_operators(jq_handle* h)
 {
     const size_t nn = (size_t)h->Ntot * h->Ntot;
@@ -400,6 +401,7 @@
         if (t4) h->BW = JQ_BW_T4;
         for (int q = 0; q < h->Nc && h->BW == JQ_BW_T4; ++q)
             h->bw_trace[q] = t4_mode(h->Hsym.data() + q * nn, h->Ntot) | t4_mode(h->Hanti.data() + q * nn, h->Ntot);
+        h->s_uniform = h->BW == JQ_BW_T4 && hanti_s_uniform(h->Hanti.data(), h->Ntot, h->NT, h->Nc);
         for (int q = 0; q < h->Nc && h->BW != JQ_BW_T4; ++q) {
             if (h->bw_trace[q] == 0 || h->BW == 0)
                 h->bw_trace[q] = (h->BW == 0) ? 1 : 0;
diff --git a/juqbox.jl_amd/csrc/jq_host_info.h b/juqbox.jl_amd/csrc/jq_host_info.h
--- a/juqbox.jl_amd/csrc/jq_host_info.h
+++ b/juqbox.jl_amd/csrc/jq_host_info.h
@@ -75,6 +75,8 @@
     kv("neumann_terms_or_max_iter", num(h->integrator == 2 ? h->imr_max_iter : h->m));
     kv("chunk_steps", num(h->chunk_steps));
     kv("replanned", h->replanned ? "true" : "false");
+    kv("s_uniform", (h->emb ? h->emb : h)->s_uniform ? "true" : "false");
+    kv("s_compact", num(hh->opt.get(O_S_COMPACT)));
     std::string fam = "[";
     auto add = [&](int id, const char* name, const char* unit, long long mx) {
         if (fam.size() > 1) fam += ", ";
@@ -149,6 +151,15 @@
     return (int)o.size();
 }
 
+extern "C" int jq_s_uniform(const double* Hanti_ops, int32_t Ntot, int32_t Ncoupled)
+{
+    if (!Hanti_ops || Ntot < 1 || Ntot > 128 || Ntot % 16 != 0 || Ncoupled < 1) return JQ_EINVAL;
+    const size_t nn = (size_t)Ntot * Ntot;
+    for (int q = 0; q < Ncoupled; ++q)
+        if (block_band(Hanti_ops + q * nn, Ntot) > 1 || !t4_structure(Hanti_ops + q * nn, Ntot)) return 0;
+    return hanti_s_uniform(Hanti_ops, Ntot, Ntot / 16, Ncoupled) ? 1 : 0;
+}
+
 extern "C" int jq_last_timing(const jq_handle* h, jq_timing* t)
 {
     if (!h || !t) return JQ_EINVAL;
diff --git a/juqbox.jl_amd/csrc/jq_host_select.h b/juqbox.jl_amd/csrc/jq_host_select.h
--- a/juqbox.jl_amd/csrc/jq_host_select.h
+++ b/juqbox.jl_amd/csrc/jq_host_select.h
@@ -58,7 +58,9 @@
     extern template __global__ void k_forward<nt, JQ_BW_T4Q, 3, false>(PropArgs);    \
     extern template __global__ void k_backward<nt, JQ_BW_T4Q, 3, false>(PropArgs);   \
     extern template __global__ void k_backward<nt, JQ_BW_T4Q, 3, false, false, true>(PropArgs);   \
-    extern template __global__ void k_backward<nt, JQ_BW_T4Q, 3, false, false, true, true>(PropArgs);
+    extern template __global__ void k_backward<nt, JQ_BW_T4Q, 3, false, false, true, true>(PropArgs);   \
+    extern template __global__ void k_forward<nt, JQ_BW_T4Q, 3, false, false, false, true>(PropArgs);   \
+    extern template __global__ void k_backward<nt, JQ_BW_T4Q, 3, false, false, true, true, true>(PropArgs);
 JQ_DECLQ(1) JQ_DECLQ(2) JQ_DECLQ(3) JQ_DECLQ(4) JQ_DECLQ(5) JQ_DECLQ(6) JQ_DECLQ(7) JQ_DECLQ(8)
 #undef JQ_DECLQ
 template <int NT, bool MODD, int NS, bool WLR = false, bool DN = false> __global__ void k_forward_cq(PropArgs);
@@ -111,6 +113,32 @@
         if (h->bw_trace[q] != (1 << q)) return false;
     return true;
 }
+static bool s_image_uniform(const double* img, int NT)
+{
+    auto same = [](double x, double y) { return memcmp(&x, &y, sizeof x) == 0; };
+    const double* cf = img + (size_t)4 * NT * JQ_T4_TILE;
+    for (int mt = 0; mt < NT; ++mt) {
+        for (int e = 0; e < 64; ++e)
+            if (!same(img[mt * 64 + e], img[e])) return false;
+        for (int g = 0; g < 4; ++g)
+            for (int r = 0; r < 4; ++r) {
+                const double* rec = cf + mt * 64 + JQ_T4_CIDX(g, r, 0);
+                if (!same(rec[0], cf[JQ_T4_CIDX(g, r, 0)]) || !same(rec[1], cf[JQ_T4_CIDX(g, r, 1)])) return false;
+                if (mt > 0 && !same(rec[2], cf[mt * 64 + 2])) return false;
+                if (mt + 1 < NT && !same(rec[3], cf[mt * 64 + 3])) return false;
+            }
+    }
+    return true;
+}
+static bool hanti_s_uniform(const double* Hanti, int Ntot, int NT, int Nc)
+{
+    std::vector<double> img((size_t)JQ_T4_ELEMS(NT));
+    for (int q = 0; q < Nc; ++q) {
+        tile_image(Hanti + (size_t)q * Ntot * Ntot, Ntot, NT, JQ_BW_T4, img.data());
+        if (!s_image_uniform(img.data(), NT)) return false;
+    }
+    return true;
+}
 static int select_cq_kernels(jq_handle* h, bool fwd2, int bwd_nr, bool wlr, bool dense, prop_kernel_t* fwd, prop_kernel_t* bwd)
 {
     const bool bwd3 = bwd_nr == 3, bwd2 = bwd_nr == 2;
@@ -224,10 +252,11 @@
 {
     const bool uni = (h->N % 4 == 0 || h->parts > 1) && !h->opt.on(O_NO_UNI);
     const bool ord = uni && h->Nc >= 2 && h->Nc <= 3 && !h->opt.on(O_NO_ORD) && ctrl_per_subsystem(h);
+    const bool sc = spw == 3 && h->s_uniform && h->opt.on(O_S_COMPACT);
 #define JQ_PICKQ(nt)                                                                                                                             \
     if (h->NT == nt) {                                                                                                                           \
-        *fwd = spw == 3 ? k_forward<nt, JQ_BW_T4Q, 3, false> : spw == 2 ? k_forward<nt, JQ_BW_T4Q, 2, false> : k_forward<nt, JQ_BW_T4Q, 1, false>;     \
-        *bwd = spw == 3 ? (ord ? k_backward<nt, JQ_BW_T4Q, 3, false, false, true, true>                                                       \
+        *fwd = spw == 3 ? (sc ? k_forward<nt, JQ_BW_T4Q, 3, false, false, false, true> : k_forward<nt, JQ_BW_T4Q, 3, false>) : spw == 2 ? k_forward<nt, JQ_BW_T4Q, 2, false> : k_forward<nt, JQ_BW_T4Q, 1, false>;     \
+        *bwd = spw == 3 ? (ord ? (sc ? k_backward<nt, JQ_BW_T4Q, 3, false, false, true, true, true> : k_backward<nt, JQ_BW_T4Q, 3, false, false, true, true>) \
                                 : uni ? k_backward<nt, JQ_BW_T4Q, 3, false, false, true> : k_backward<nt, JQ_BW_T4Q, 3, false>)                 \
                         : spw == 2 ? k_backward<nt, JQ_BW_T4Q, 2, false> : k_backward<nt, JQ_BW_T4Q, 1, false>;  \
         return JQ_OK;                                                                                                                            \
diff --git a/juqbox.jl_amd/csrc/jq_kernel_inst.hip b/juqbox.jl_amd/csrc/jq_kernel_inst.hip
--- a/juqbox.jl_amd/csrc/jq_kernel_inst.hip
+++ b/juqbox.jl_amd/csrc/jq_kernel_inst.hip
@@ -131,6 +131,8 @@
 template __global__ void k_backward<JQ_NT, JQ_BW, 3, false>(PropArgs);
 template __global__ void k_backward<JQ_NT, JQ_BW, 3, false, false, true>(PropArgs);
 template __global__ void k_backward<JQ_NT, JQ_BW, 3, false, false, true, true>(PropArgs);
+template __global__ void k_forward<JQ_NT, JQ_BW, 3, false, false, false, true>(PropArgs);
+template __global__ void k_backward<JQ_NT, JQ_BW, 3, false, false, true, true, true>(PropArgs);
 #else
 template __global__ void k_forward<JQ_NT, JQ_BW, JQ_MINW, (JQ_VARIANT == 1)>(PropArgs);
 template __global__ void k_backward<JQ_NT, JQ_BW, JQ_MINW, (JQ_VARIANT == 1)>(PropArgs);
diff --git a/juqbox.jl_amd/csrc/jq_kernels.h b/juqbox.jl_amd/csrc/jq_kernels.h
--- a/juqbox.jl_amd/csrc/jq_kernels.h
+++ b/juqbox.jl_amd/csrc/jq_kernels.h
@@ -457,6 +457,9 @@
     return (const d4*)(mat - lane + 4 * NT * JQ_T4_TILE + JQ_T4_CIDX(lane >> 4, (lane >> 2) & 3, 0));
 }
 __device__ __forceinline__ d4 t4q_cload(const d4* cf, int mt) { return cf[mt * 16]; }
+__device__ __forceinline__ d2 t4s_c01(const d4* cf) { return ((const d2*)cf)[0]; }
+__device__ __forceinline__ d2 t4s_c23(const d4* cf, int mt) { return ((const d2*)(cf + mt * 16))[1]; }
+__device__ __forceinline__ d4 t4s_c(const d2& c01, const d2& c23) { return (d4){c01[0], c01[1], c23[0], c23[1]}; }
 template <int NT, bool ZEROC, int MODE>
 __device__ __forceinline__ void t4q_block(Arr<NT>& D, const Arr<NT>& C, const Arr<NT>& x, int mt, double a, const d4& c, double& xold)
 {
@@ -529,7 +532,7 @@
 struct T4qNoHook {
     __device__ __forceinline__ void operator()(int, double, double) const {}
 };
-template <int NT, int NP, bool Z0, bool Z1, bool Z2, int SH = 0, typename HOOK = T4qNoHook>
+template <int NT, int NP, bool Z0, bool Z1, bool Z2, int SH = 0, typename HOOK = T4qNoHook, int SCM = 0>
 __device__ __forceinline__ void mm_t4q_multi(Arr<NT>& D0, const Arr<NT>& C0, const double* m0, Arr<NT>& D1, const Arr<NT>& C1,
                                              const double* m1, Arr<NT>& D2, const Arr<NT>& C2, const double* m2, const Arr<NT>& x,
                                              double sh0 = 0.0, double sh1 = 0.0, double sh2 = 0.0, const double* wsr = nullptr,
@@ -539,14 +542,27 @@
     const double* ma[3] = {t4q_a(m0, lane), t4q_a(m1, lane), t4q_a(NP > 2 ? m2 : m1, lane)};
     const d4* cf[3] = {t4q_c<NT>(m0, lane), t4q_c<NT>(m1, lane), t4q_c<NT>(NP > 2 ? m2 : m1, lane)};
     double xold = 0.0;
+    double as[3];
+    d2 cs[3];
+#pragma unroll
+    for (int k = 0; k < NP; ++k)
+        if ((SCM >> k) & 1) {
+            as[k] = ma[k][0];
+            cs[k] = t4s_c01(cf[k]);
+        }
 #pragma unroll
     for (int mt = 0; mt < NT; ++mt) {
         double a[3];
         d4 c[3];
 #pragma unroll
         for (int k = 0; k < NP; ++k) {
-            a[k] = ma[k][mt * 64];
-            c[k] = t4q_cload(cf[k], mt);
+            if ((SCM >> k) & 1) {
+                a[k] = as[k];
+                c[k] = t4s_c(cs[k], t4s_c23(cf[k], mt));
+            } else {
+                a[k] = ma[k][mt * 64];
+                c[k] = t4q_cload(cf[k], mt);
+            }
         }
         if constexpr (SH != 0) {
             const double w = wsr[16 * mt];
@@ -585,18 +601,18 @@
         __builtin_amdgcn_sched_barrier(0);
     }
 }
-template <int NT, bool Z0, bool Z1, int SH = 0>
+template <int NT, bool Z0, bool Z1, int SH = 0, int SCM = 0>
 __device__ __forceinline__ void mm_t4q2(Arr<NT>& D0, const Arr<NT>& C0, const double* m0, Arr<NT>& D1, const Arr<NT>& C1,
                                         const double* m1, const Arr<NT>& x, double sh0 = 0.0, double sh1 = 0.0, const double* wsr = nullptr)
 {
-    mm_t4q_multi<NT, 2, Z0, Z1, true, SH>(D0, C0, m0, D1, C1, m1, D1, C1, m1, x, sh0, sh1, 0.0, wsr);
-}
-template <int NT, bool Z0, bool Z1, bool Z2, int SH = 0>
+    mm_t4q_multi<NT, 2, Z0, Z1, true, SH, T4qNoHook, SCM>(D0, C0, m0, D1, C1, m1, D1, C1, m1, x, sh0, sh1, 0.0, wsr);
+}
+template <int NT, bool Z0, bool Z1, bool Z2, int SH = 0, int SCM = 0>
 __device__ __forceinline__ void mm_t4q3(Arr<NT>& D0, const Arr<NT>& C0, const double* m0, Arr<NT>& D1, const Arr<NT>& C1,
                                         const double* m1, Arr<NT>& D2, const Arr<NT>& C2, const double* m2, const Arr<NT>& x,
                                         double sh0 = 0.0, double sh1 = 0.0, double sh2 = 0.0, const double* wsr = nullptr)
 {
-    mm_t4q_multi<NT, 3, Z0, Z1, Z2, SH>(D0, C0, m0, D1, C1, m1, D2, C2, m2, x, sh0, sh1, sh2, wsr);
+    mm_t4q_multi<NT, 3, Z0, Z1, Z2, SH, T4qNoHook, SCM>(D0, C0, m0, D1, C1, m1, D2, C2, m2, x, sh0, sh1, sh2, wsr);
 }
 template <int NT>
 __device__ __forceinline__ void t4q_load(OpQ<NT>& op, const double* mat)
@@ -623,6 +639,47 @@
     double xold = 0.0;
 #pragma unroll
     for (int mt = 0; mt < NT; ++mt) t4q_block<NT, false, JQ_T4_DIAG | JQ_T4_RTERMS | JQ_T4_MTERMS>(D, C, x, mt, op.a[mt], op.c[mt], xold);
+}
+
+template <int NT>
+struct OpS {
+    double a;
+    d2 c;
+    d2 m[NT];
+};
+template <int NT>
+__device__ __forceinline__ void t4s_load(OpS<NT>& op, const double* mat)
+{
+    const int lane = threadIdx.x & 63;
+    const d4* cf = t4q_c<NT>(mat, lane);
+    op.a = t4q_a(mat, lane)[0];
+    op.c = t4s_c01(cf);
+#pragma unroll
+    for (int mt = 0; mt < NT; ++mt) op.m[mt] = t4s_c23(cf, mt);
+}
+template <int NT>
+__device__ __forceinline__ void mm_t4s_regs(Arr<NT>& D, const Arr<NT>& C, const OpS<NT>& op, const Arr<NT>& x)
+{
+    double xold = 0.0;
+#pragma unroll
+    for (int mt = 0; mt < NT; ++mt)
+        t4q_block<NT, false, JQ_T4_DIAG | JQ_T4_RTERMS | JQ_T4_MTERMS>(D, C, x, mt, op.a, t4s_c(op.c, op.m[mt]), xold);
+}
+template <int NT, bool ZEROC>
+__device__ __forceinline__ void mm_t4s(Arr<NT>& D, const Arr<NT>& C, const double* mat, const Arr<NT>& x)
+{
+    const int lane = threadIdx.x & 63;
+    const d4* cf = t4q_c<NT>(mat, lane);
+    const double a = t4q_a(mat, lane)[0];
+    const d2 c01 = t4s_c01(cf);
+    d2 m_cur = t4s_c23(cf, 0);
+    double xold = 0.0;
+#pragma unroll
+    for (int mt = 0; mt < NT; ++mt) {
+        const d2 m = m_cur;
+        if (mt + 1 < NT) m_cur = t4s_c23(cf, mt + 1);
+        t4q_block<NT, ZEROC, JQ_T4_DIAG | JQ_T4_RTERMS | JQ_T4_MTERMS>(D, C, x, mt, a, t4s_c(c01, m), xold);
+    }
 }
 
 template <int NT, int BW, bool ZEROC, bool SD = false>
@@ -1322,7 +1379,7 @@
     for (int i = 0; i < NT; ++i) out.t[i] = (bpa.t[i] - A.t[i]) + (in_a ? Ya.t[i] : Yb.t[i]);
 }
 
-template <int NT, int BW, bool JAC, bool REGOP = true>
+template <int NT, int BW, bool JAC, bool REGOP = true, bool SC = false>
 __device__ __forceinline__ void horner_add(Arr<NT>& out, const Arr<NT>& bpa, const Arr<NT>& A, const double* S, int m,
                                            Arr<NT>& Ya, Arr<NT>& Yb, double jacobi_tol2, int ncol, int jac_wg = -1)
 {
@@ -1335,6 +1392,23 @@
         return;
     }
     int rem = m - 1;
+    if constexpr (SC) {
+        static_assert(!SC || (BW == JQ_BW_T4Q && !JAC), "SC: quad layout, Neumann solver");
+        if (rem == 0) {
+            mm_t4s<NT, false>(out, bpa, S, A);
+            return;
+        }
+        OpS<NT> op;
+        t4s_load(op, S);
+        mm_t4s_regs(Ya, A, op, A);
+        for (--rem; rem >= 2; rem -= 2) {
+            mm_t4s_regs(Ya, A, op, Ya);
+            mm_t4s_regs(Ya, A, op, Ya);
+        }
+        if (rem > 0) mm_t4s_regs(Ya, A, op, Ya);
+        mm_t4s_regs(out, bpa, op, Ya);
+        return;
+    }
     if (rem == 0) {
         mm_c<NT, BW>(out, bpa, S, A);
         return;
@@ -1443,21 +1517,22 @@
 #ifndef JQ_BWD3_NOOPQ_STATE
 #define JQ_BWD3_NOOPQ_STATE 0
 #endif
-template <int NT, int BW, bool JAC, int FUSE = 0, bool FOLD = false, bool REGOP = true, bool TERMS = false, typename RING = RingT<BW == JQ_BW_T4Q>>
+template <int NT, int BW, bool JAC, int FUSE = 0, bool FOLD = false, bool REGOP = true, bool TERMS = false, typename RING = RingT<BW == JQ_BW_T4Q>, bool SC = false>
 __device__ __forceinline__ void sv_state(RING& p, const PropArgs& a, bool active, double ceps, const double* ws, int g,
                                          const Arr<NT>& u, Arr<NT>& v, Arr<NT>& unew, Arr<NT>& vN, Arr<NT>& A, Arr<NT>& Ya,
                                          Arr<NT>& Yb)
 {
+    static_assert(!SC || (BW == JQ_BW_T4Q && !JAC && FUSE == 3 && REGOP), "SC: the fused quad-layout step");
     if constexpr (BW == JQ_BW_T4Q && !JAC && FUSE != 0) {
         const double* M0 = p.template next_ks<0, 1>();
         const double* M1 = p.template next_ks<1, 0>();
         if (active) {
             if constexpr (FOLD) {
                 static_assert(!FOLD || (FUSE & 3) == 3 || FUSE == 0, "FOLD: fused or generic path");
-                mm_t4q2<NT, true, false, 1>(A, A, M0, unew, u, M1, u, ceps, 0.0, ws + g);
+                mm_t4q2<NT, true, false, 1, SC ? 2 : 0>(A, A, M0, unew, u, M1, u, ceps, 0.0, ws + g);
             } else {
             if constexpr (FUSE & 1) {
-                mm_t4q2<NT, true, false>(A, A, M0, unew, u, M1, u);
+                mm_t4q2<NT, true, false, 0, SC ? 2 : 0>(A, A, M0, unew, u, M1, u);
             } else {
                 mm_z<NT, BW>(A, M0, u);
                 mm_c<NT, BW>(unew, u, M1, u);
@@ -1467,18 +1542,19 @@
         }
         M0 = p.template next_ks<1, 1>();
         if (active) {
-            mm_c<NT, BW>(A, A, M0, v);
+            if constexpr (SC) mm_t4s<NT, false>(A, A, M0, v);
+            else mm_c<NT, BW>(A, A, M0, v);
             a_add(v, A);
-            horner_add<NT, BW, JAC, REGOP>(v, v, A, M0, a.m, Ya, Yb, a.jacobi_tol2, a.N, a.jac_wg_lds);
+            horner_add<NT, BW, JAC, REGOP, SC>(v, v, A, M0, a.m, Ya, Yb, a.jacobi_tol2, a.N, a.jac_wg_lds);
         }
         M1 = p.template next_ks<0, 0>();
         const double* M2 = p.template next_ks<0, 2>();
         if (active) {
             if constexpr (FOLD) {
-                mm_t4q3<NT, false, false, true, 6>(vN, v, M0, unew, unew, M1, A, A, M2, v, 0.0, -ceps, -ceps, ws + g);
+                mm_t4q3<NT, false, false, true, 6, SC ? 1 : 0>(vN, v, M0, unew, unew, M1, A, A, M2, v, 0.0, -ceps, -ceps, ws + g);
             } else {
             if constexpr (FUSE & 2) {
-                mm_t4q3<NT, false, false, true>(vN, v, M0, unew, unew, M1, A, A, M2, v);
+                mm_t4q3<NT, false, false, true, 0, SC ? 1 : 0>(vN, v, M0, unew, unew, M1, A, A, M2, v);
             } else {
                 mm_c<NT, BW>(vN, v, M0, v);
                 mm_c<NT, BW>(unew, unew, M1, v);
@@ -1492,9 +1568,10 @@
         }
         M0 = p.template next_ks<1, 2>();
         if (active) {
-            mm_c<NT, BW>(A, A, M0, unew);
+            if constexpr (SC) mm_t4s<NT, false>(A, A, M0, unew);
+            else mm_c<NT, BW>(A, A, M0, unew);
             a_add(unew, A);
-            horner_add<NT, BW, JAC, REGOP>(unew, unew, A, M0, a.m, Ya, Yb, a.jacobi_tol2, a.N, a.jac_wg_lds);
+            horner_add<NT, BW, JAC, REGOP, SC>(unew, unew, A, M0, a.m, Ya, Yb, a.jacobi_tol2, a.N, a.jac_wg_lds);
         }
         return;
     }
@@ -1547,9 +1624,10 @@
 
 template <int BW, bool JAC, bool WLRT>
 constexpr bool jq_wlr_on() { return WLRT; }
-template <int NT, int BW, int MINW, bool JAC, bool WLRT = false, bool UNI = false>
+template <int NT, int BW, int MINW, bool JAC, bool WLRT = false, bool UNI = false, bool SC = false>
 __global__ __launch_bounds__((BW == JQ_BW_T4Q) ? 256 * MINW : 256, (BW == JQ_BW_T4Q) ? 1 : MINW) void k_forward(PropArgs a)
 {
+    static_assert(!SC || (BW == JQ_BW_T4Q && MINW == 3 && !JAC && !WLRT), "SC: a variant of the three-slab quad-layout kernel");
     extern __shared__ __attribute__((aligned(16))) char smem[];
     constexpr int KT = 4 * NT;
     const int lane_ = threadIdx.x & 63;
@@ -1591,7 +1669,7 @@
     {                                                                                                            \
         p.begin_step(NSTEP);                                                                                     \
         if (active) leak += a_wsq(wd, g, U);                   \
-        sv_state<NT, BW, JAC, JQ_FWD_FUSE, UNI>(p, a, active, ceps, ws, g, U, V, UN, VN, A, Ya, Yb);                  \
+        sv_state<NT, BW, JAC, JQ_FWD_FUSE, UNI, true, false, RingT<QUAD>, SC>(p, a, active, ceps, ws, g, U, V, UN, VN, A, Ya, Yb); \
                                                 \
         const double* M6 = p.template next_ks<0, 1>();                                                                             \
         if (active) {                                                                                            \
@@ -1653,10 +1731,11 @@
     }
 }
 
-template <int NT, int BW, int MINW, bool JAC, bool WLRT = false, bool UNI = false, bool ORD = false>
+template <int NT, int BW, int MINW, bool JAC, bool WLRT = false, bool UNI = false, bool ORD = false, bool SC = false>
 __global__ __launch_bounds__((BW == JQ_BW_T4Q) ? 256 * MINW : 256, (BW == JQ_BW_T4Q) ? 1 : MINW) void k_backward(PropArgs a)
 {
     static_assert(!ORD || (UNI && BW == JQ_BW_T4Q && !JAC), "ORD: a variant of the UNI quad-layout kernel");
+    static_assert(!SC || (ORD && MINW == 3 && !WLRT && !JQ_BWD3_NOOPQ && !JQ_BWD3_NOOPQ_STATE), "SC: a variant of the ORD three-slab kernel");
     extern __shared__ __attribute__((aligned(16))) char smem[];
     constexpr int KT = 4 * NT;
     const int lane_ = threadIdx.x & 63;
@@ -1759,7 +1838,7 @@
     for (int n = 0; n < a.nsteps_chunk; ++n) {
         p.begin_step(n);
         if (active) a_park(mu, P0);
-        sv_state<NT, BW, JAC, (MINW >= 3 ? (UNI ? 3 : JQ_BWD_FUSE3) : JQ_BWD_FUSE), UNI, !(QUAD && MINW >= 3 && JQ_BWD3_NOOPQ_STATE), jq_bwd_terms(NT, BW, JAC)>(p, a, active, ceps, ws, g, u, v, un, vN, mu, Ya, Yb);
+        sv_state<NT, BW, JAC, (MINW >= 3 ? (UNI ? 3 : JQ_BWD_FUSE3) : JQ_BWD_FUSE), UNI, !(QUAD && MINW >= 3 && JQ_BWD3_NOOPQ_STATE), jq_bwd_terms(NT, BW, JAC), RingT<QUAD>, SC>(p, a, active, ceps, ws, g, u, v, un, vN, mu, Ya, Yb);
         if (n > 0) flush_traces(n - 1);
         const double* M = p.template next_ks<0, 1>();
         if (active) {
@@ -1778,7 +1857,8 @@
         }
         M = p.template next_ks<1, 0>();
         if (active) {
-            mm_c<NT, BW>(L, L, M, mu);
+            if constexpr (SC) mm_t4s<NT, false>(L, L, M, mu);
+            else mm_c<NT, BW>(L, L, M, mu);
             a_axpy_rows1<NT, false>(L, wd, g, u);
             if constexpr (WLR)
                 if (wforce)
@@ -1791,7 +1871,7 @@
                     }
             a_add(mu, L);
             if constexpr (jq_bwd_terms(NT, BW, JAC)) neumann_terms_add<NT, BW>(mu, L, M, a.m, Ya);
-            else horner_add<NT, BW, JAC, BREG>(mu, mu, L, M, a.m, Ya, Yb, a.jacobi_tol2, a.N, a.jac_wg_lds);
+            else horner_add<NT, BW, JAC, BREG, SC>(mu, mu, L, M, a.m, Ya, Yb, a.jacobi_tol2, a.N, a.jac_wg_lds);
         }
         double o_p4 = 0.0;
         for (int q = 0; q < Nc; ++q) {
@@ -1837,7 +1917,8 @@
         }
         M = p.template next_ks<1, 1>();
         if (active) {
-            mm_z<NT, BW>(Ya, M, nb);
+            if constexpr (SC) mm_t4s<NT, true>(Ya, Ya, M, nb);
+            else mm_z<NT, BW>(Ya, M, nb);
             a_axpy_rows1<NT, true>(Ya, wd, g, v);
             if constexpr (WLR)
                 if (wforce)
@@ -1852,11 +1933,12 @@
                     }
             a_add(L, Ya);
             a_add(vN, Ya);
-            mm_c<NT, BW>(vN, vN, M, L);
+            if constexpr (SC) mm_t4s<NT, false>(vN, vN, M, L);
+            else mm_c<NT, BW>(vN, vN, M, L);
             a_add(L, nb);
             a_add(L, vN);
             if constexpr (jq_bwd_terms(NT, BW, JAC)) neumann_terms_add<NT, BW>(L, vN, M, a.m, Ya);
-            else horner_add<NT, BW, JAC, BREG>(L, L, vN, M, a.m, Ya, Yb, a.jacobi_tol2, a.N, a.jac_wg_lds);
+            else horner_add<NT, BW, JAC, BREG, SC>(L, L, vN, M, a.m, Ya, Yb, a.jacobi_tol2, a.N, a.jac_wg_lds);
             a_add(nb, L);
         }
         M = p.template next_ks<0, 1>();
@@ -1877,7 +1959,8 @@
         }
         M = p.template next_ks<1, 2>();
         if (active) {
-            mm_c<NT, BW>(vN, vN, M, mu);
+            if constexpr (SC) mm_t4s<NT, false>(vN, vN, M, mu);
+            else mm_c<NT, BW>(vN, vN, M, mu);
             a_axpy_rows1<NT, false>(vN, wd, g, un);
             if constexpr (WLR)
                 if (wforce)
diff --git a/juqbox.jl_amd/csrc/jq_options.h b/juqbox.jl_amd/csrc/jq_options.h
--- a/juqbox.jl_amd/csrc/jq_options.h
+++ b/juqbox.jl_amd/csrc/jq_options.h
@@ -7,7 +7,7 @@
 enum JqOpt {
     O_T4, O_OD, O_T4BIG, O_FORCE_DENSE, O_WINDOW, O_LANE, O_LANE_MIN, O_LANE_MAX, O_ROWLANE_MAX, O_COOP_MAX, O_QUAD, O_CQ, O_EMBED,
     O_STREAM_BYTES, O_CHUNK_STEPS, O_BATCH,
-    O_DQ, O_NOSPLIT, O_QUAD8, O_CQ_W, O_IMR_CQ, O_IMR_CQ2, O_CQ_FWD2, O_CQ3, O_QSPLIT, O_RL_SPLIT, O_JAC_WG, O_TRACE_BYTES, O_NO_UNI, O_NO_ORD,
+    O_DQ, O_NOSPLIT, O_QUAD8, O_CQ_W, O_IMR_CQ, O_IMR_CQ2, O_CQ_FWD2, O_CQ3, O_QSPLIT, O_RL_SPLIT, O_JAC_WG, O_TRACE_BYTES, O_NO_UNI, O_NO_ORD, O_S_COMPACT,
     O_QS_RIDE, O_CQ_GENERIC_TRACES, O_WLR_SC, O_RCCL_SELFCHECK, O_MULTI_SAME_DEVICE, O_CQ3_RDV_US, O_CQ3_WAIT_MS,
     O_DEBUG, O_CQ3_FAULT,
     O_COUNT
@@ -56,6 +56,7 @@
     {"trace_bytes", JQ_OPT_UNSET, 0, "bytes of the per-step trace records of one backward chunk (default 4 GiB): smaller = more, shorter chunks"},
     {"no_uni", 0, 0, "1: three-slab quad-layout backward sweep on the generic kernel (tests compare)"},
     {"no_ord", 0, 0, "1: no single-subsystem-control specialisation of the quad-layout backward kernels (tests compare)"},
+    {"s_compact", 1, 0, "0: three-slab quad-layout kernels read the full S operand of every block even when the S images are uniform (plan info s_uniform; bit-identical)"},
     {"qs_ride", JQ_OPT_UNSET, 0, "split quad-layout backward kernel: trace products as separate passes (0) / riding along also at four quads per workgroup (1)"},
     {"cq_generic_traces", 0, 0, "1: cooperative-quad backward sweep with full trace products even when every control acts on one subsystem"},
     {"wlr_sc", 0, JQ_OPT_EXP, "1: full weights, quad layout: carry the column dots of a step in LDS (measured slower)"},
diff --git a/juqbox.jl_amd/csrc/juqbox_hip.hip b/juqbox.jl_amd/csrc/juqbox_hip.hip
--- a/juqbox.jl_amd/csrc/juqbox_hip.hip
+++ b/juqbox.jl_amd/csrc/juqbox_hip.hip
@@ -62,6 +62,7 @@
     int BWc = 0;
     int NcK = 0;
     std::vector<int> bw_trace;
+    bool s_uniform = false;
     long long mat_elems = 0;
     long long mat_elems_c = 0;
     bool coop_ok = false;
```

New measurement: 3065, median of 6. 3.6% higher.
